# zhangxiaochen95/uav_bs_ctrl

Hardware: AMD Instinct MI355X
Metric: env-steps/sec (MADRQN, 8 UBS x 80 GT) (higher is better)
Workload: dtype f32

## Files before the change

include/uavgnn.h:

```cpp
#ifndef UAVGNN_H
#define UAVGNN_H

#include <stddef.h>
#include <stdint.h>

#ifdef __cplusplus
extern "C" {
#endif

#define UAVGNN_VERSION 100

#define UAVGNN_EINVAL (-1000)
#define UAVGNN_EUNSUPPORTED (-1001)
#define UAVGNN_EWORKSPACE (-1002)

typedef void* uavgnn_stream_t;

int uavgnn_version(void);

const char* uavgnn_strerror(int code);

int uavgnn_gatv2_fwd(const float* x_src, int E, int F_src, const float* x_dst, int F_dst, const int32_t* seg_off,
                     const int32_t* dst_order, int N, const float* W_s, const float* b_s, const float* W_d, const float* b_d, const float* attn,
                     const float* W_r, const float* b_r, int nh, int D, float slope, float* out, int ld_out,
// ... 40 lines not shown
                     const float* attn_save, float* dW_s, float* db_s, float* dW_d, float* db_d, float* dattn,
                     float* dW_r, float* db_r, void* workspace, size_t workspace_bytes, uavgnn_stream_t stream);
int uavgnn_gatv2_bwd_generic(const float* x_src, int E, int F_src, const float* x_dst, int F_dst, const int32_t* seg_off,
                     const int32_t* dst_order, int N, const float* W_s, const float* b_s, const float* W_d, const float* b_d, const float* attn,
                     int nh, int D, float slope, const float* out, const float* d_out, int ld_out,
                     const float* attn_save, float* dW_s, float* db_s, float* dW_d, float* db_d, float* dattn,
                     float* dW_r, float* db_r, void* workspace, size_t workspace_bytes, uavgnn_stream_t stream);

int uavgnn_talk_attn_fwd(const float* s, int ld_s, const float* q, int ld_q, const float* v, int ld_v, int K, int M,
                         const int32_t* talk_off, const int32_t* talk_src, int N, float scale, float* c, int ld_c,
                         float* a_save, const float* x_copy, int ld_x, int n_copy, uavgnn_stream_t stream);

int uavgnn_talk_attn_bwd(const float* s, int ld_s, const float* q, int ld_q, const float* v, int ld_v, int K, int M,
                         const int32_t* talk_off, const int32_t* talk_src, const int32_t* t_off, const int32_t* t_dst,
                         const int32_t* t_pos, int N, float scale, const float* a_save, const float* d_c, int ld_dc,
                         float* d_s, int ld_ds, float* d_q, int ld_dq, float* d_v, int ld_dv, float* de_tmp,
                         uavgnn_stream_t stream);

int uavgnn_gru_gates_fwd(const float* gi, const float* gh, const float* h, int N, int H, float* h_out,
                         uavgnn_stream_t stream);
int uavgnn_gru_gates_bwd(const float* gi, const float* gh, const float* h, const float* d_hout, int N, int H,
                         float* d_gi, float* d_gh, float* d_h, uavgnn_stream_t stream);

int uavgnn_disc_comm_fwd(const float* logits, int ld, const float* gumbel, const long long* rng, int msg,
                         const int32_t* talk_off, const int32_t* talk_src, int N, float inv_tau, float* c, int ld_c,
                         float* y0_save, int32_t* sel, uavgnn_stream_t stream);
int uavgnn_gumbel_noise(const long long* rng, long long E, int msg, float* out, uavgnn_stream_t stream);
int uavgnn_disc_comm_bwd(const float* d_c, int ld_dc, const float* y0_save, const int32_t* sel, int msg,
                         const int32_t* t_off, const int32_t* t_dst, const int32_t* t_pos, int N, float inv_tau,
                         float* d_logits, int ld_dl, uavgnn_stream_t stream);

int uavgnn_obs_degrees(const float* gt, int M, int Fg, const float* ubs, int U, int Fu, int N, int32_t* deg_seen,
                       int32_t* deg_near, uavgnn_stream_t stream);
int uavgnn_obs_compact(const float* gt, int M, int Fg, const float* ubs, int U, int Fu, int N, const int32_t* seen_off,
                       const int32_t* near_off, float* x_gt, float* x_ubs, uavgnn_stream_t stream);
int uavgnn_talk_degrees(const float* d_u2u, int n, int B, float r_comm, int32_t* deg_in, int32_t* env_edges,
                        uavgnn_stream_t stream);
int uavgnn_talk_compact(const float* d_u2u, int n, int B, float r_comm, const int32_t* talk_off,
                        const int32_t* env_base, int32_t* talk_src, int32_t* talk_eid, uavgnn_stream_t stream);
int uavgnn_offsets_scan4(const int32_t* d0, int n0, int32_t* o0, const int32_t* d1, int n1, int32_t* o1, const int32_t* d2,
                         int n2, int32_t* o2, const int32_t* d3, int n3, int32_t* o3, uavgnn_stream_t stream);

int uavgnn_eps_greedy(const float* q, int ld_q, int N, int A, int n_agents, const float* u_team, const float* u_agent,
                      float eps, long long* acts, uavgnn_stream_t stream);
int uavgnn_eps_greedy_dev(const float* q, int ld_q, int N, int A, int n_agents, const float* u_team, const float* u_agent,
                          const float* eps_dev, long long* acts, uavgnn_stream_t stream);

int uavgnn_colsum_acc(const float* x, long long ld, int N, int C, float* acc, int S, uavgnn_stream_t stream);
int uavgnn_gemm_h2_supported(int M, int N, int K);
long long uavgnn_split_h2_bytes(int n_out, int K);
int uavgnn_split_h2(const float* W, int ld, int R, int C, int transpose, void* planes, uavgnn_stream_t stream);
int uavgnn_gemm_nt_h2(const float* X, int ldx, int K1, const float* X2, int ldx2, int M, int K, const float* rowmax, const float* rowmax2,
                      const void* planes, int N, const float* bias, float* Y, int ldy, int epilogue, uavgnn_stream_t stream);
int uavgnn_gemm_nt_h2_rm2(const float* X, int ldx, int K1, const float* X2, int ldx2, int M, int K, const float* rowmax, float* rowmax2_out,
                          const void* planes, int N, const float* bias, float* Y, int ldy, int epilogue, uavgnn_stream_t stream);
int uavgnn_gemm_nt_h2_n64(const float* X, int ldx, int M, int K, const float* rowmax, const void* planes, int N, float* Y, int ldy,
                          uavgnn_stream_t stream);
int uavgnn_gru_gates_bwd_fused_sums_rowmax(const float* pre, const float* h, const float* d_hout, const float* dq, int n_out,
                                           const float* W_out, int N, int H, float* d_gi, float* d_gh, float* d_h, float* col_sums,
                                           float* row_absmax, uavgnn_stream_t stream);
int uavgnn_relu_bwd_colsum_rowmax(const float* dy, long long ld, const float* y, long long ldy, float* out, long long ldo, int N, int C,
                                  float* acc, int S, float* row_absmax, uavgnn_stream_t stream);
int uavgnn_relu_bwd_colsum(const float* dy, long long ld, const float* y, long long ldy, float* out, long long ldo, int N, int C,
                           float* acc, int S, uavgnn_stream_t stream);

int uavgnn_flat_obs_supported(int H_out, int F);
int uavgnn_flat_obs_fwd(const float* agent, long long ld_a, int F_a, const float* gt, long long ld_g, int K_g, const float* ubs,
                        long long ld_u, int K_u, int rows, const float* W, const float* b, int H_out, float* y, long long ld_y,
                        uavgnn_stream_t stream);
int uavgnn_flat_obs_wgrad_chunks(long long rows, int H_out, int F);
int uavgnn_flat_obs_wgrad(const float* dy, long long ld_dy, int H_out, const float* agent, long long ld_a, int F_a, const float* gt,
                          long long ld_g, int K_g, const float* ubs, long long ld_u, int K_u, int rows, float* partials, int S,
                          int accumulate, uavgnn_stream_t stream);

int uavgnn_talk_attn_env_supported(int n_max, int M, int K);
int uavgnn_talk_attn_env_fwd(const float* s, int ld_s, const float* q, int ld_q, const float* v, int ld_v, int K, int M,
                             const int32_t* talk_off, const int32_t* talk_src, const int32_t* graph_off, int B,
                             int n_max, float scale, float* c, int ld_c, float* a_save, const float* x_copy, int ld_x,
                             int n_copy, uavgnn_stream_t stream);
int uavgnn_talk_attn_env_bwd(const float* s, int ld_s, const float* q, int ld_q, const float* v, int ld_v, int K, int M,
                             const int32_t* talk_off, const int32_t* talk_src, const int32_t* graph_off, int B,
                             int n_max, float scale, const float* a_save, const float* d_c, int ld_dc, float* d_s,
                             int ld_ds, float* d_q, int ld_dq, float* d_v, int ld_dv, uavgnn_stream_t stream);

int uavgnn_tarmac_msg_supported(int H, int M, int K, int n_ag);
long long uavgnn_tarmac_msg_weight_bytes(int H, int M, int K);
long long uavgnn_tarmac_msg_planes_bytes(int N, int H, int M);
int uavgnn_tarmac_msg_prepare(const float* Wp, int ld, int H, int M, int K, void* tiles, uavgnn_stream_t stream);
int uavgnn_tarmac_msg_fwd(const float* x, int ld_x, const float* h, int ld_h, int N, int H, int n_ag, const void* tiles,
                          const float* bias, int M, int K, const int32_t* talk_off, const int32_t* talk_src, float scale,
                          float* c_out, int ld_c, float* a_save, float* proj_out, int ld_p, float* x_copy, int ld_xc,
                          void* planes_out, uavgnn_stream_t stream);
int uavgnn_tarmac_msg_rowmax_supported(int H, int M, int K, int n_ag);
int uavgnn_tarmac_msg_fwd_rowmax(const float* x, int ld_x, const float* h, int ld_h, int N, int H, int n_ag, const void* tiles,
                                 const float* bias, int M, int K, const int32_t* talk_off, const int32_t* talk_src, float scale,
                                 float* c_out, int ld_c, float* a_save, float* proj_out, int ld_p, float* x_copy, int ld_xc,
                                 float* row_absmax, uavgnn_stream_t stream);

size_t uavgnn_degree_order_workspace_bytes(int N);
int uavgnn_degree_order(const int32_t* seg_off, int N, int32_t* order, void* workspace, size_t workspace_bytes,
                        uavgnn_stream_t stream);
size_t uavgnn_csc_transpose_workspace_bytes(int N);
int uavgnn_csc_transpose(const int32_t* talk_off, const int32_t* talk_src, int N, int E, int32_t* t_off,
                         int32_t* t_dst, int32_t* t_pos, void* workspace, size_t workspace_bytes,
                         uavgnn_stream_t stream);
int uavgnn_csc_transpose_env(const int32_t* talk_off, const int32_t* talk_src, const int32_t* graph_off, int B, int N,
                             int32_t* t_off, int32_t* t_dst, int32_t* t_pos, uavgnn_stream_t stream);

int uavgnn_adamw_polyak(float* p, float* g, float* exp_avg, float* exp_avg_sq, float* p_targ, long long n,
                        long long n_clip, const float* hyper, double beta1, double beta2, float eps, float weight_decay,
                        float clip, float polyak, uavgnn_stream_t stream);

int uavgnn_env_state_dim(int n_ubs, int n_gts, int fair_service);
int uavgnn_env_step(const int32_t* int_consts, const double* f64_consts, int B, const long long* actions,
                    const double* avail_moves, double* pos_ubs, const float* pos_gts, int32_t* prior, float* avg_rate,
                    int32_t* t, float* run_f32, double* n_colls, float* d_u2g, float* d_u2u, int32_t* gt_ubs,
                    int32_t* gt_rb, float* rate_per_gt, double* rate_per_ubs, int32_t* mask_collision, double* reward,
                    float* done, float* obs_gt, float* obs_ubs, float* obs_agent, float* state, uavgnn_stream_t stream);

int uavgnn_build_graph_small_max_agents(void);
int uavgnn_build_graph_small(const float* gt, int M, int Fg, const float* ubs, int U, int Fu, const float* d_u2u, int n, int B,
                             float r_comm, int32_t* seen_off, int32_t* near_off, int32_t* talk_off, float* x_gt, float* x_ubs,
                             int32_t* talk_src, int32_t* talk_eid, int32_t* graph_off, uavgnn_stream_t stream);

int uavgnn_gru_cell_supported(int K_in, int H);
int uavgnn_gru_cell_fwd(const float* inp, int ld_inp, int K_in, const float* h, int N, int H, const float* W_ih,
                        const float* b_ih, const float* W_hh, const float* b_hh, float* h_out, float* pre_save,
                        uavgnn_stream_t stream);
int uavgnn_gru_cell_x3_supported(int K_in, int H);
long long uavgnn_gru_cell_x3_workspace_bytes(int K_in, int H);
int uavgnn_gru_split_weights(const float* W_ih, int K_in, const float* W_hh, int H, void* planes, uavgnn_stream_t stream);
int uavgnn_gru_cell_fwd_x3(const float* inp, int ld_inp, int K_in, const float* h, int N, int H, const void* planes,
                           const float* b_ih, const float* b_hh, float* h_out, float* pre_save, uavgnn_stream_t stream);
int uavgnn_gru_cell_fwd_x3_cat(const float* inp, int ld_inp, int K1, const float* inp2, int ld_inp2, int K2, const float* h,
                               int N, int H, const void* planes, const float* b_ih, const float* b_hh, float* h_out,
                               float* pre_save, uavgnn_stream_t stream);
#define UAVGNN_GRU_STAGING_BLOCKS 1
int uavgnn_gru_cell_fwd_x3_opts(const float* inp, int ld_inp, int K1, const float* inp2, int ld_inp2, int K2, const float* h,
                                int N, int H, const void* planes, const float* b_ih, const float* b_hh, float* h_out,
                                float* pre_save, int flags, uavgnn_stream_t stream);
int uavgnn_gru_cell_h2_supported(int K_in, int H);
long long uavgnn_gru_cell_h2_workspace_bytes(int K_in, int H);
int uavgnn_gru_split_weights_h2(const float* W_ih, int K_in, const float* W_hh, int H, void* planes, uavgnn_stream_t stream);
int uavgnn_gru_cell_fwd_h2(const float* inp, int ld_inp, int K1, const float* inp2, int ld_inp2, int K2, const float* h, int N, int H,
                           const float* row_absmax, const void* planes, const float* b_ih, const float* b_hh, float* h_out,
                           float* pre_save, uavgnn_stream_t stream);
int uavgnn_row_absmax(const float* a1, int ld1, int K1, const float* a2, int ld2, int K2, const float* a3, int ld3, int K3, int N,
                      float* out, uavgnn_stream_t stream);
int uavgnn_head_supported(int H, int A);
int uavgnn_head_fwd(const float* h, int ld_h, int N, int H, const float* W, int ld_w, const float* b, int A, float* q, int ld_q,
                    uavgnn_stream_t stream);
#define UAVGNN_GEMM_ACCUMULATE 1
#define UAVGNN_GEMM_RELU 2
#define UAVGNN_GEMM_STAGING_INTERLEAVED 4
#define UAVGNN_GEMM_TILE_128 8
#define UAVGNN_GEMM_TILE_64 16
int uavgnn_gemm_x3_supported(int M, int N, int K);
int uavgnn_split_bf16x3(const float* W, int ld, int R, int C, int transpose, void* planes, uavgnn_stream_t stream);
int uavgnn_gemm_nt_x3(const float* X, int ldx, int M, int K, const void* planes, int N, const float* bias, float* Y, int ldy,
                      int epilogue, uavgnn_stream_t stream);
int uavgnn_gemm_nt_x3_cat(const float* X, int ldx, int K1, const float* X2, int ldx2, int M, int K, const void* planes, int N,
                          const float* bias, float* Y, int ldy, int epilogue, uavgnn_stream_t stream);
int uavgnn_gemm_nt_x3_rowmax(const float* X, int ldx, int M, int K, const void* planes, int N, const float* bias, float* Y, int ldy,
                             int epilogue, float* rowmax_out, uavgnn_stream_t stream);

int uavgnn_gemm_tn_x3_chunks(long long n_rows, int Mo, int Ko);
int uavgnn_gemm_tn_x3(const float* dY, int ldy, int Mo, const float* X, int ldx, int Ko, long long n_rows, float* partials,
                      int S, int accumulate, uavgnn_stream_t stream);
int uavgnn_col_absmax(const float* x, long long ld, long long n, int C, float* out, uavgnn_stream_t stream);
int uavgnn_gemm_tn_h2_supported(long long n_rows, int Mo, int Ko);
int uavgnn_gemm_tn_h2_chunks(long long n_rows, int Mo, int Ko);
int uavgnn_gemm_tn_h2(const float* dY, long long ldy, int Mo, const float* X, long long ldx, int Ko, long long n_rows,
                      const float* colmax_y, const float* colmax_x, float* partials, int S, int accumulate, uavgnn_stream_t stream);
int uavgnn_gru_gates_bwd_fused(const float* pre, const float* h, const float* d_hout, int N, int H, float* d_gi, float* d_gh,
                               float* d_h, uavgnn_stream_t stream);
int uavgnn_gru_gates_bwd_fused_head(const float* pre, const float* h, const float* d_hout, const float* dq, int n_out,
                                    const float* W_out, int N, int H, float* d_gi, float* d_gh, float* d_h,
                                    uavgnn_stream_t stream);
int uavgnn_gru_gates_bwd_sum_rows(int N, int H);
int uavgnn_gru_gates_bwd_fused_sums(const float* pre, const float* h, const float* d_hout, const float* dq, int n_out,
                                    const float* W_out, int N, int H, float* d_gi, float* d_gh, float* d_h, float* col_sums,
                                    uavgnn_stream_t stream);

long long uavgnn_gru_cell_bwd_workspace_bytes(int K_in, int H);
int uavgnn_gru_split_weights_bwd(const float* W_ih, int K_in, const float* W_hh, int H, void* planes, uavgnn_stream_t stream);
int uavgnn_gru_cell_bwd(const float* pre, const float* h, const float* d_hout, int N, int K_in, int H, const void* planes_bwd,
                        float* d_gi, float* d_gh, float* d_inp, int ld_dinp, float* d_h, uavgnn_stream_t stream);

#define UAVGNN_WS_GATV2_BWD 1
#define UAVGNN_WS_DEGREE_ORDER 2
#define UAVGNN_WS_CSC_TRANSPOSE 3
#define UAVGNN_WS_GRU_PLANES 4
#define UAVGNN_WS_GRU_BWD_PLANES 5
#define UAVGNN_WS_GEMM_PLANES 6
#define UAVGNN_WS_GEMM_TN_PARTIALS 7
#define UAVGNN_WS_K1_IMAGE 8
long long uavgnn_workspace_bytes(int kind, long long a, long long b, long long c);

#ifdef __cplusplus
// ... 4 lines not shown
```

uav_bs_ctrl_amd/_lib.py:

```python
from __future__ import annotations

import ctypes
import os

import torch as th

_HERE = os.path.dirname(os.path.abspath(__file__))
LIB_PATH = os.environ.get("UAVGNN_LIB") or os.path.join(_HERE, "csrc", "libuavgnn.so")

_c_fp = ctypes.c_void_p
_c_ip = ctypes.c_void_p
_c_int = ctypes.c_int
_c_f32 = ctypes.c_float
_c_st = ctypes.c_void_p

SIGNATURES = {
    "uavgnn_version": (_c_int, []),
    "uavgnn_strerror": (ctypes.c_char_p, [_c_int]),
    "uavgnn_gatv2_fwd": (_c_int, [_c_fp, _c_int, _c_int, _c_fp, _c_int, _c_ip, _c_ip, _c_int, _c_fp, _c_fp, _c_fp, _c_fp, _c_fp,
                                  _c_fp, _c_fp, _c_int, _c_int, _c_f32, _c_fp, _c_int, _c_fp, _c_st]),
    "uavgnn_gatv2_fwd_valu": (_c_int, [_c_fp, _c_int, _c_int, _c_fp, _c_int, _c_ip, _c_ip, _c_int, _c_fp, _c_fp, _c_fp, _c_fp, _c_fp,
                                       _c_fp, _c_fp, _c_int, _c_int, _c_f32, _c_fp, _c_int, _c_fp, _c_st]),
    "uavgnn_gatv2_fwd_mfma": (_c_int, [_c_fp, _c_int, _c_int, _c_fp, _c_int, _c_ip, _c_ip, _c_int, _c_fp, _c_fp, _c_fp, _c_fp, _c_fp,
                                       _c_fp, _c_fp, _c_int, _c_int, _c_f32, _c_fp, _c_int, _c_fp, _c_st]),
# ... 38 lines not shown
    "uavgnn_talk_compact": (_c_int, [_c_fp, _c_int, _c_int, _c_f32, _c_ip, _c_ip, _c_ip, _c_ip, _c_st]),
    "uavgnn_build_graph_small_max_agents": (_c_int, []),
    "uavgnn_build_graph_small": (_c_int, [_c_fp, _c_int, _c_int, _c_fp, _c_int, _c_int, _c_fp, _c_int, _c_int, _c_f32, _c_ip, _c_ip,
                                          _c_ip, _c_fp, _c_fp, _c_ip, _c_ip, _c_ip, _c_st]),
    "uavgnn_degree_order_workspace_bytes": (ctypes.c_size_t, [_c_int]),
    "uavgnn_degree_order": (_c_int, [_c_ip, _c_int, _c_ip, ctypes.c_void_p, ctypes.c_size_t, _c_st]),
    "uavgnn_csc_transpose_workspace_bytes": (ctypes.c_size_t, [_c_int]),
    "uavgnn_csc_transpose": (_c_int, [_c_ip, _c_ip, _c_int, _c_int, _c_ip, _c_ip, _c_ip, ctypes.c_void_p,
                                      ctypes.c_size_t, _c_st]),
    "uavgnn_csc_transpose_env": (_c_int, [_c_ip, _c_ip, _c_ip, _c_int, _c_int, _c_ip, _c_ip, _c_ip, _c_st]),
    "uavgnn_talk_attn_env_supported": (_c_int, [_c_int, _c_int, _c_int]),
    "uavgnn_tarmac_msg_supported": (_c_int, [_c_int, _c_int, _c_int, _c_int]),
    "uavgnn_tarmac_msg_weight_bytes": (ctypes.c_longlong, [_c_int, _c_int, _c_int]),
    "uavgnn_tarmac_msg_planes_bytes": (ctypes.c_longlong, [_c_int, _c_int, _c_int]),
    "uavgnn_tarmac_msg_prepare": (_c_int, [_c_fp, _c_int, _c_int, _c_int, _c_int, ctypes.c_void_p, _c_st]),
    "uavgnn_tarmac_msg_fwd_dbg": (_c_int, [_c_fp, _c_int, _c_fp, _c_int, _c_int, _c_int, _c_int, ctypes.c_void_p, _c_fp, _c_int, _c_int,
                                           _c_ip, _c_ip, _c_f32, _c_fp, _c_int, _c_fp, _c_fp, _c_int, _c_fp, _c_int, ctypes.c_void_p,
                                           _c_int, _c_st]),
    "uavgnn_tarmac_msg_fwd": (_c_int, [_c_fp, _c_int, _c_fp, _c_int, _c_int, _c_int, _c_int, ctypes.c_void_p, _c_fp, _c_int, _c_int,
                                       _c_ip, _c_ip, _c_f32, _c_fp, _c_int, _c_fp, _c_fp, _c_int, _c_fp, _c_int, ctypes.c_void_p,
                                       _c_st]),
    "uavgnn_talk_attn_env_fwd": (_c_int, [_c_fp, _c_int, _c_fp, _c_int, _c_fp, _c_int, _c_int, _c_int, _c_ip, _c_ip,
                                          _c_ip, _c_int, _c_int, _c_f32, _c_fp, _c_int, _c_fp, _c_fp, _c_int, _c_int,
                                          _c_st]),
    "uavgnn_talk_attn_env_bwd": (_c_int, [_c_fp, _c_int, _c_fp, _c_int, _c_fp, _c_int, _c_int, _c_int, _c_ip, _c_ip,
                                          _c_ip, _c_int, _c_int, _c_f32, _c_fp, _c_fp, _c_int, _c_fp, _c_int, _c_fp,
                                          _c_int, _c_fp, _c_int, _c_st]),
    "uavgnn_eps_greedy": (_c_int, [_c_fp, _c_int, _c_int, _c_int, _c_int, _c_fp, _c_fp, _c_f32, ctypes.c_void_p, _c_st]),
    "uavgnn_eps_greedy_dev": (_c_int, [_c_fp, _c_int, _c_int, _c_int, _c_int, _c_fp, _c_fp, _c_fp, ctypes.c_void_p, _c_st]),
    "uavgnn_colsum_acc": (_c_int, [_c_fp, ctypes.c_longlong, _c_int, _c_int, _c_fp, _c_int, _c_st]),
    "uavgnn_relu_bwd_colsum": (_c_int, [_c_fp, ctypes.c_longlong, _c_fp, ctypes.c_longlong, _c_fp, ctypes.c_longlong, _c_int, _c_int, _c_fp,
                               _c_int, _c_st]),
    "uavgnn_relu_bwd_colsum_rowmax": (_c_int, [_c_fp, ctypes.c_longlong, _c_fp, ctypes.c_longlong, _c_fp, ctypes.c_longlong, _c_int, _c_int,
                                               _c_fp, _c_int, _c_fp, _c_st]),
    "uavgnn_flat_obs_supported": (_c_int, [_c_int, _c_int]),
    "uavgnn_flat_obs_fwd": (_c_int, [_c_fp, ctypes.c_longlong, _c_int, _c_fp, ctypes.c_longlong, _c_int, _c_fp, ctypes.c_longlong, _c_int,
                                     _c_int, _c_fp, _c_fp, _c_int, _c_fp, ctypes.c_longlong, _c_st]),
    "uavgnn_flat_obs_wgrad_chunks": (_c_int, [ctypes.c_longlong, _c_int, _c_int]),
    "uavgnn_flat_obs_wgrad": (_c_int, [_c_fp, ctypes.c_longlong, _c_int, _c_fp, ctypes.c_longlong, _c_int, _c_fp, ctypes.c_longlong, _c_int,
                                       _c_fp, ctypes.c_longlong, _c_int, _c_int, _c_fp, _c_int, _c_int, _c_st]),
    "uavgnn_gemm_nt_x3_rowmax": (_c_int, [_c_fp, _c_int, _c_int, _c_int, ctypes.c_void_p, _c_int, _c_fp, _c_fp, _c_int, _c_int, _c_fp, _c_st]),
    "uavgnn_col_absmax": (_c_int, [_c_fp, ctypes.c_longlong, ctypes.c_longlong, _c_int, _c_fp, _c_st]),
    "uavgnn_gemm_tn_h2_supported": (_c_int, [ctypes.c_longlong, _c_int, _c_int]),
    "uavgnn_gemm_tn_h2_chunks": (_c_int, [ctypes.c_longlong, _c_int, _c_int]),
    "uavgnn_gemm_tn_h2": (_c_int, [_c_fp, ctypes.c_longlong, _c_int, _c_fp, ctypes.c_longlong, _c_int, ctypes.c_longlong, _c_fp, _c_fp, _c_fp,
                                   _c_int, _c_int, _c_st]),
    "uavgnn_gemm_h2_supported": (_c_int, [_c_int, _c_int, _c_int]),
    "uavgnn_split_h2_bytes": (ctypes.c_longlong, [_c_int, _c_int]),
    "uavgnn_split_h2": (_c_int, [_c_fp, _c_int, _c_int, _c_int, _c_int, ctypes.c_void_p, _c_st]),
    "uavgnn_gemm_nt_h2": (_c_int, [_c_fp, _c_int, _c_int, _c_fp, _c_int, _c_int, _c_int, _c_fp, _c_fp, ctypes.c_void_p, _c_int, _c_fp, _c_fp,
                                   _c_int, _c_int, _c_st]),
    "uavgnn_gemm_nt_h2_rm2": (_c_int, [_c_fp, _c_int, _c_int, _c_fp, _c_int, _c_int, _c_int, _c_fp, _c_fp, ctypes.c_void_p, _c_int, _c_fp, _c_fp,
                                       _c_int, _c_int, _c_st]),
    "uavgnn_gemm_nt_h2_n64": (_c_int, [_c_fp, _c_int, _c_int, _c_int, _c_fp, ctypes.c_void_p, _c_int, _c_fp, _c_int, _c_st]),
    "uavgnn_env_state_dim": (_c_int, [_c_int, _c_int, _c_int]),
    "uavgnn_env_step": (_c_int, [ctypes.POINTER(ctypes.c_int32), ctypes.POINTER(ctypes.c_double), _c_int] + [_c_fp] * 22 + [_c_st]),
    "uavgnn_adamw_polyak": (_c_int, [_c_fp, _c_fp, _c_fp, _c_fp, _c_fp, ctypes.c_longlong, ctypes.c_longlong, _c_fp, ctypes.c_double,
                                     ctypes.c_double, _c_f32, _c_f32, _c_f32, _c_f32, _c_st]),
    "uavgnn_gru_cell_supported": (_c_int, [_c_int, _c_int]),
    "uavgnn_gru_cell_fwd": (_c_int, [_c_fp, _c_int, _c_int, _c_fp, _c_int, _c_int, _c_fp, _c_fp, _c_fp, _c_fp, _c_fp, _c_fp, _c_st]),
    "uavgnn_gru_cell_x3_supported": (_c_int, [_c_int, _c_int]),
    "uavgnn_gru_cell_x3_workspace_bytes": (ctypes.c_longlong, [_c_int, _c_int]),
    "uavgnn_gru_split_weights": (_c_int, [_c_fp, _c_int, _c_fp, _c_int, ctypes.c_void_p, _c_st]),
    "uavgnn_gru_cell_fwd_x3": (_c_int, [_c_fp, _c_int, _c_int, _c_fp, _c_int, _c_int, ctypes.c_void_p, _c_fp, _c_fp, _c_fp, _c_fp, _c_st]),
    "uavgnn_gru_cell_fwd_x3_cat": (_c_int, [_c_fp, _c_int, _c_int, _c_fp, _c_int, _c_int, _c_fp, _c_int, _c_int, ctypes.c_void_p, _c_fp, _c_fp,
                                            _c_fp, _c_fp, _c_st]),
    "uavgnn_gru_cell_fwd_x3_opts": (_c_int, [_c_fp, _c_int, _c_int, _c_fp, _c_int, _c_int, _c_fp, _c_int, _c_int, ctypes.c_void_p, _c_fp, _c_fp,
                                             _c_fp, _c_fp, _c_int, _c_st]),
    "uavgnn_gru_cell_h2_supported": (_c_int, [_c_int, _c_int]),
    "uavgnn_gru_cell_h2_workspace_bytes": (ctypes.c_longlong, [_c_int, _c_int]),
    "uavgnn_gru_split_weights_h2": (_c_int, [_c_fp, _c_int, _c_fp, _c_int, ctypes.c_void_p, _c_st]),
    "uavgnn_gru_cell_fwd_h2": (_c_int, [_c_fp, _c_int, _c_int, _c_fp, _c_int, _c_int, _c_fp, _c_int, _c_int, _c_fp, ctypes.c_void_p, _c_fp,
                                        _c_fp, _c_fp, _c_fp, _c_st]),
    "uavgnn_row_absmax": (_c_int, [_c_fp, _c_int, _c_int, _c_fp, _c_int, _c_int, _c_fp, _c_int, _c_int, _c_int, _c_fp, _c_st]),
    "uavgnn_tarmac_msg_rowmax_supported": (_c_int, [_c_int, _c_int, _c_int, _c_int]),
    "uavgnn_tarmac_msg_fwd_rowmax": (_c_int, [_c_fp, _c_int, _c_fp, _c_int, _c_int, _c_int, _c_int, ctypes.c_void_p, _c_fp, _c_int, _c_int,
                                              _c_ip, _c_ip, _c_f32, _c_fp, _c_int, _c_fp, _c_fp, _c_int, _c_fp, _c_int, _c_fp, _c_st]),
    "uavgnn_gru_weight_tiles_bytes": (ctypes.c_longlong, [_c_int, _c_int]),
    "uavgnn_gru_split_weight_tiles": (_c_int, [_c_fp, _c_int, _c_fp, _c_int, ctypes.c_void_p, _c_st]),
    "uavgnn_gru_cell_fwd_planes": (_c_int, [ctypes.c_void_p, _c_int, _c_fp, _c_int, _c_int, ctypes.c_void_p, _c_fp, _c_fp, _c_fp, _c_fp,
                                            _c_st]),
    "uavgnn_gru_cell_fwd_planes_opts": (_c_int, [ctypes.c_void_p, _c_int, _c_fp, _c_int, _c_int, ctypes.c_void_p, _c_fp, _c_fp, _c_fp,
                                                 _c_fp, _c_int, _c_st]),
    "uavgnn_gru_cell_bwd_workspace_bytes": (ctypes.c_longlong, [_c_int, _c_int]),
    "uavgnn_gru_split_weights_bwd": (_c_int, [_c_fp, _c_int, _c_fp, _c_int, ctypes.c_void_p, _c_st]),
    "uavgnn_gru_cell_bwd": (_c_int, [_c_fp, _c_fp, _c_fp, _c_int, _c_int, _c_int, ctypes.c_void_p, _c_fp, _c_fp, _c_fp, _c_int, _c_fp,
                                     _c_st]),
    "uavgnn_workspace_bytes": (ctypes.c_longlong, [_c_int, ctypes.c_longlong, ctypes.c_longlong, ctypes.c_longlong]),
    "uavgnn_gemm_tn_x3_chunks": (_c_int, [ctypes.c_longlong, _c_int, _c_int]),
    "uavgnn_gemm_tn_x3": (_c_int, [_c_fp, _c_int, _c_int, _c_fp, _c_int, _c_int, ctypes.c_longlong, _c_fp, _c_int, _c_int, _c_st]),
    "uavgnn_gemm_x3_supported": (_c_int, [_c_int, _c_int, _c_int]),
    "uavgnn_head_supported": (_c_int, [_c_int, _c_int]),
    "uavgnn_head_fwd": (_c_int, [_c_fp, _c_int, _c_int, _c_int, _c_fp, _c_int, _c_fp, _c_int, _c_fp, _c_int, _c_st]),
    "uavgnn_split_bf16x3": (_c_int, [_c_fp, _c_int, _c_int, _c_int, _c_int, ctypes.c_void_p, _c_st]),
    "uavgnn_gemm_nt_x3": (_c_int, [_c_fp, _c_int, _c_int, _c_int, ctypes.c_void_p, _c_int, _c_fp, _c_fp, _c_int, _c_int, _c_st]),
    "uavgnn_gemm_nt_x3_cat": (_c_int, [_c_fp, _c_int, _c_int, _c_fp, _c_int, _c_int, _c_int, ctypes.c_void_p, _c_int, _c_fp, _c_fp, _c_int,
                              _c_int, _c_st]),
    "uavgnn_gru_gates_bwd_fused": (_c_int, [_c_fp, _c_fp, _c_fp, _c_int, _c_int, _c_fp, _c_fp, _c_fp, _c_st]),
    "uavgnn_gru_gates_bwd_fused_head": (_c_int, [_c_fp, _c_fp, _c_fp, _c_fp, _c_int, _c_fp, _c_int, _c_int, _c_fp, _c_fp, _c_fp,
                                                 _c_st]),
    "uavgnn_gru_gates_bwd_sum_rows": (_c_int, [_c_int, _c_int]),
    "uavgnn_gru_gates_bwd_fused_sums": (_c_int, [_c_fp, _c_fp, _c_fp, _c_fp, _c_int, _c_fp, _c_int, _c_int, _c_fp, _c_fp, _c_fp, _c_fp,
                                                 _c_st]),
    "uavgnn_gru_gates_bwd_fused_sums_rowmax": (_c_int, [_c_fp, _c_fp, _c_fp, _c_fp, _c_int, _c_fp, _c_int, _c_int, _c_fp, _c_fp, _c_fp, _c_fp,
                                                        _c_fp, _c_st]),
    "uavgnn_gru_gates_fwd": (_c_int, [_c_fp, _c_fp, _c_fp, _c_int, _c_int, _c_fp, _c_st]),
    "uavgnn_gru_gates_bwd": (_c_int, [_c_fp, _c_fp, _c_fp, _c_fp, _c_int, _c_int, _c_fp, _c_fp, _c_fp, _c_st]),
}

_LIB = None
UAVGNN_EINVAL = -1000
UAVGNN_EUNSUPPORTED = -1001


class UavGnnError(RuntimeError):
    pass


def lib() -> ctypes.CDLL:
    global _LIB
    if _LIB is None:
        if not os.path.exists(LIB_PATH):
            raise UavGnnError(f"{LIB_PATH} is missing - build it with `python -c 'import __graft_entry__ as g; "
                              f"g.build()'`.  uav_bs_ctrl_amd has no CPU / eager fallback.")
        handle = ctypes.CDLL(LIB_PATH)
        for name, (res, args) in SIGNATURES.items():
            fn = getattr(handle, name)
            fn.restype, fn.argtypes = res, args
        _LIB = handle
        if os.environ.get("UAVGNN_TUNED_GEMM", "0") == "1":
# ... 42 lines not shown
```

uav_bs_ctrl_amd/csrc/gemm_h2.hip:

```cpp
#include "common.h"
#include "f16x2.h"

namespace uavgnn {
namespace {

using namespace h2;

constexpr int BN = 128, BK = 32, BM8 = 256, NT = 512;
constexpr int PA = BM8 * 4, PB = BN * 4;
constexpr int BUF = 2 * PA + 2 * PB;

__global__ __launch_bounds__(256) void split_h2_kernel(const float* __restrict__ W, int ld, int R, int C, int transpose,
                                                       unsigned short* __restrict__ planes, float* __restrict__ winv) {
  __shared__ float red[4];
  const int orow = blockIdx.x, tid = threadIdx.x;
  const int ocol_n = transpose ? R : C;
  const size_t n = static_cast<size_t>(transpose ? C : R) * ocol_n;
  auto at = [&](int j) { return transpose ? W[static_cast<size_t>(j) * ld + orow] : W[static_cast<size_t>(orow) * ld + j]; };
  float m = 0.f;
  for (int j = tid; j < ocol_n; j += 256) m = fmaxf(m, fabsf(at(j)));
  m = wave_max(m);
  if ((tid & 63) == 0) red[tid >> 6] = m;
  __syncthreads();
  m = fmaxf(fmaxf(red[0], red[1]), fmaxf(red[2], red[3]));
  const int se = scale_exp(m);
  const float s = pow2f(se);
  for (int j = 2 * tid; j < ocol_n; j += 512) {
    const Split2 sp = split_pair(at(j) * s, at(j + 1) * s);
    *reinterpret_cast<unsigned*>(planes + static_cast<size_t>(orow) * ocol_n + j) = sp.hi;
    *reinterpret_cast<unsigned*>(planes + n + static_cast<size_t>(orow) * ocol_n + j) = sp.lo;
  }
  if (tid == 0) winv[orow] = pow2f(-se);
}

template <bool ACC, bool RELU, bool IL>
__global__ __launch_bounds__(NT) void gemm_nt_h2w8_kernel(const float* __restrict__ X, int ldx, int M, int K,
                                                          const unsigned short* __restrict__ Bp, int N, const float* __restrict__ winv,
                                                          const float* __restrict__ bias, float* __restrict__ Y, int ldy,
                                                          int row_blocks, int col_blocks, const float* __restrict__ X2, int ldx2,
                                                          int ns1, const float* __restrict__ rm1, const float* __restrict__ rm2,
                                                          float* __restrict__ rm2_out) {
  constexpr int kTileChunks = BM8 * (BN + 4) / 4;
#ifndef UAVGNN_GEMM_H2_TILE_STORE
#define UAVGNN_GEMM_H2_TILE_STORE 1
#endif
  constexpr bool kTileStore = ACC || UAVGNN_GEMM_H2_TILE_STORE;
  __shared__ u32x4 smem[(kTileStore && kTileChunks > 2 * BUF) ? kTileChunks : 2 * BUF];
  __shared__ float sInv[BM8];
  __shared__ float sRow2[BM8];
  const int tid = threadIdx.x, lane = tid & 63, wave = tid >> 6;
  const int l32 = lane & 31, lh = lane >> 5, sw = swz32(l32);
  const int wm = (wave >> 1) * 64, wn = (wave & 1) * 64;
  const int xcd = blockIdx.x & 7, slot = blockIdx.x >> 3;
  const int rb = (slot / col_blocks) * 8 + xcd, cb = slot - (slot / col_blocks) * col_blocks;
  if (rb >= row_blocks) return;
  const int m0 = rb * BM8, n0 = cb * BN;

  f32x16 acc[2][2];
#pragma unroll
  for (int a = 0; a < 2; ++a)
#pragma unroll
    for (int b = 0; b < 2; ++b)
#pragma unroll
      for (int i = 0; i < 16; ++i) acc[a][b][i] = 0.f;

  const int lr = tid >> 3, c4 = tid & 7;
  unsigned xo[4], xo2[4];
  float sca[4];
  auto bound = [&](int row) {
    const float a = rm1[row];
    return rm2 != nullptr ? fmaxf(a, rm2[row]) : a;
  };
  const bool own2 = rm2_out != nullptr;
  float m2[4] = {0.f, 0.f, 0.f, 0.f};
#pragma unroll
  for (int i = 0; i < 4; ++i) {
    const int row = min(m0 + lr + 64 * i, M - 1);
    xo[i] = static_cast<unsigned>(row) * ldx + 4 * c4;
    xo2[i] = static_cast<unsigned>(row) * ldx2 + 4 * c4;
  }
  if (own2) {
    const int nq = (K - ns1 * BK) / 4;
    bool bad[4] = {false, false, false, false};
#pragma unroll
    for (int i = 0; i < 4; ++i)
      for (int q = c4; q < nq; q += 8) {
        const float4 v = *reinterpret_cast<const float4*>(X2 + xo2[i] + 4 * (q - c4));
        const float a0 = fabsf(v.x), a1 = fabsf(v.y), a2 = fabsf(v.z), a3 = fabsf(v.w);
        bad[i] |= !(a0 <= 3.4028234663852886e38f) | !(a1 <= 3.4028234663852886e38f) | !(a2 <= 3.4028234663852886e38f) |
                  !(a3 <= 3.4028234663852886e38f);
        m2[i] = fmaxf(fmaxf(m2[i], fmaxf(a0, a1)), fmaxf(a2, a3));
      }
#pragma unroll
    for (int i = 0; i < 4; ++i) {
// ... 133 lines not shown
      }
      __builtin_amdgcn_sched_barrier(0);
      UAVGNN_H2_MFMA(f0)
      __builtin_amdgcn_sched_barrier(0);
      if (!early) {
        lstore((t + 1) & 1);
        gload(min(t + 2, ns - 1));
      }
      __syncthreads();
      UAVGNN_H2_READ(f0, (t + 1) & 1, 0)
      __builtin_amdgcn_sched_barrier(0);
      UAVGNN_H2_MFMA(f1)
      __builtin_amdgcn_sched_barrier(0);
    }
  }
#undef UAVGNN_H2_MFMA
#undef UAVGNN_H2_TERM
#undef UAVGNN_H2_READ
  if constexpr (kTileStore) {
  if ((ldy & 3) == 0 && (reinterpret_cast<uintptr_t>(Y) & 15) == 0 && n0 + BN <= N) {
    constexpr int LDT = BN + 4;
    float* sT = reinterpret_cast<float*>(smem);
    static_assert(BM8 * LDT * 4 <= static_cast<int>(sizeof(smem)), "the output tile fits the LDS array");
    __syncthreads();
#pragma unroll
    for (int a = 0; a < 2; ++a)
#pragma unroll
      for (int b = 0; b < 2; ++b) {
        const int col = n0 + wn + b * 32 + l32;
        const float bv = bias != nullptr ? bias[col] : 0.f, ci = winv[col];
#pragma unroll
        for (int i = 0; i < 16; ++i) {
          const int lrow = wm + a * 32 + 8 * (i >> 2) + 4 * lh + (i & 3);
          sT[lrow * LDT + wn + b * 32 + l32] = acc[a][b][i] * ci * sInv[lrow] + bv;
        }
      }
    float4 yv[16];
    if constexpr (ACC) {
#pragma unroll
      for (int q = 0; q < 16; ++q) {
        const int idx = tid + NT * q, row = idx >> 5, cc = idx & 31;
        yv[q] = *reinterpret_cast<const float4*>(Y + static_cast<size_t>(min(m0 + row, M - 1)) * ldy + n0 + 4 * cc);
      }
    }
    __syncthreads();
#pragma unroll
    for (int q = 0; q < 16; ++q) {
      const int idx = tid + NT * q, row = idx >> 5, cc = idx & 31;
      const float4 t = *reinterpret_cast<const float4*>(sT + row * LDT + 4 * cc);
      float4 o = t;
      if constexpr (ACC) o = {yv[q].x + t.x, yv[q].y + t.y, yv[q].z + t.z, yv[q].w + t.w};
      if (RELU) o = {fmaxf(o.x, 0.f), fmaxf(o.y, 0.f), fmaxf(o.z, 0.f), fmaxf(o.w, 0.f)};
      if (m0 + row < M) *reinterpret_cast<float4*>(Y + static_cast<size_t>(m0 + row) * ldy + n0 + 4 * cc) = o;
    }
    return;
  }
  }
#pragma unroll
  for (int b = 0; b < 2; ++b) {
    const int col = n0 + wn + b * 32 + l32;
    if (col >= N) continue;
    const float bv = bias != nullptr ? bias[col] : 0.f, ci = winv[col];
#pragma unroll
    for (int a = 0; a < 2; ++a)
#pragma unroll
      for (int i = 0; i < 16; ++i) {
        const int lrow = wm + a * 32 + 8 * (i >> 2) + 4 * lh + (i & 3);
        const int row = m0 + lrow;
        if (row < M) {
          float* p = Y + static_cast<size_t>(row) * ldy + col;
          float v = acc[a][b][i] * ci * sInv[lrow] + bv;
          if (ACC) v += *p;
          if (RELU) v = fmaxf(v, 0.f);
          *p = v;
        }
      }
  }
}

constexpr int BM6 = 128, BN6 = 64;
constexpr int PA6 = BM6 * 4, PB6 = BN6 * 4;
constexpr int SUB6 = 2 * PA6 + 2 * PB6;
constexpr int BUF6 = 2 * SUB6;

__global__ __launch_bounds__(NT) void gemm_nt_h2n64_kernel(const float* __restrict__ X, int ldx, int M, int K,
                                                           const unsigned short* __restrict__ Bp, int N, const float* __restrict__ winv,
                                                           float* __restrict__ Y, int ldy, int col_blocks, const float* __restrict__ rm1) {
  constexpr int LDT = BN6 + 4;
  static_assert(BM6 * LDT * 4 <= 2 * BUF6 * 16, "the output tile fits the staging buffers");
  __shared__ u32x4 smem[2 * BUF6];
  __shared__ float sInv[BM6];
  const int tid = threadIdx.x, lane = tid & 63, wave = tid >> 6;
  const int l32 = lane & 31, lh = lane >> 5, sw = swz32(l32);
  const int wm = (wave >> 1) * 32, wn = (wave & 1) * 32;
  const int rb = blockIdx.x / col_blocks, cb = blockIdx.x - rb * col_blocks;
  const int m0 = rb * BM6, n0 = cb * BN6;

  f32x16 acc;
#pragma unroll
  for (int i = 0; i < 16; ++i) acc[i] = 0.f;

  const int lr = tid >> 3, c4 = tid & 7;
  unsigned xo[2];
  float sca[2];
#pragma unroll
  for (int i = 0; i < 2; ++i) {
// ... 68 lines not shown
    __builtin_amdgcn_sched_barrier(0);
    UAVGNN_N64_MFMA(f3)
    __builtin_amdgcn_sched_barrier(0);
  }
#undef UAVGNN_N64_MFMA
#undef UAVGNN_N64_READ
  float* sT = reinterpret_cast<float*>(smem);
  __syncthreads();
  {
    const float ci = winv[n0 + wn + l32];
#pragma unroll
    for (int i = 0; i < 16; ++i) {
      const int lrow = wm + 8 * (i >> 2) + 4 * lh + (i & 3);
      sT[lrow * LDT + wn + l32] = acc[i] * ci * sInv[lrow];
    }
  }
  __syncthreads();
#pragma unroll
  for (int q = 0; q < 4; ++q) {
    const int idx = tid + NT * q, row = idx >> 4, cc = idx & 15;
    if (m0 + row < M)
      *reinterpret_cast<float4*>(Y + static_cast<size_t>(m0 + row) * ldy + n0 + 4 * cc) =
          *reinterpret_cast<const float4*>(sT + row * LDT + 4 * cc);
  }
}

}
}

using namespace uavgnn;

extern "C" int uavgnn_gemm_h2_supported(int M, int N, int K) {
  return (M > 0 && N > 0 && K >= BK && K % BK == 0 && static_cast<long long>(M) * K < (1LL << 31) &&
          2LL * N * K < (1LL << 31)) ? 1 : 0;
}

extern "C" long long uavgnn_split_h2_bytes(int n_out, int K) {
  if (n_out <= 0 || K <= 0) return 0;
  return 4LL * n_out * K + 4LL * n_out;
}

extern "C" int uavgnn_split_h2(const float* W, int ld, int R, int C, int transpose, void* planes, uavgnn_stream_t stream) {
  if (!W || !planes || R <= 0 || C <= 0 || ld < C) return UAVGNN_EINVAL;
  const int n_out = transpose ? C : R, K = transpose ? R : C;
  if ((K & 1) || (reinterpret_cast<uintptr_t>(planes) & 15)) return UAVGNN_EUNSUPPORTED;
  unsigned short* p = static_cast<unsigned short*>(planes);
  float* winv = reinterpret_cast<float*>(p + 2LL * n_out * K);
  hipLaunchKernelGGL(split_h2_kernel, dim3(n_out), dim3(256), 0, static_cast<hipStream_t>(stream), W, ld, R, C, transpose, p, winv);
  return launch_status();
}

static int gemm_nt_h2_launch(const float* X, int ldx, int K1, const float* X2, int ldx2, int M, int K, const float* rowmax,
                             const float* rowmax2, float* rowmax2_out, const void* planes, int N, const float* bias, float* Y, int ldy,
                             int epilogue, uavgnn_stream_t stream) {
  if (M < 0 || !X || !planes || !Y || !rowmax || ldx < K1 || ldy < N || K1 <= 0 || K1 > K || (X2 == nullptr) != (K1 == K) ||
      (X2 != nullptr && ldx2 < K - K1) || (rowmax2_out != nullptr && (X2 == nullptr || rowmax2 != nullptr)))
    return UAVGNN_EINVAL;
  if (M == 0) return 0;
  if (!uavgnn_gemm_h2_supported(M, N, K) || (ldx & 3) || static_cast<long long>(M) * ldx >= (1LL << 31) ||
      ((reinterpret_cast<uintptr_t>(X) | reinterpret_cast<uintptr_t>(planes)) & 15) ||
      (epilogue & (UAVGNN_GEMM_TILE_128 | UAVGNN_GEMM_TILE_64)))
    return UAVGNN_EUNSUPPORTED;
  if (X2 != nullptr && ((K1 % BK) || (ldx2 & 3) || static_cast<long long>(M) * ldx2 >= (1LL << 31) || (reinterpret_cast<uintptr_t>(X2) & 15)))
    return UAVGNN_EUNSUPPORTED;
  const int ns1 = K1 / BK;
  hipStream_t st = static_cast<hipStream_t>(stream);
  const unsigned short* bp = static_cast<const unsigned short*>(planes);
  const float* winv = reinterpret_cast<const float*>(bp + 2LL * N * K);
  const bool acc = (epilogue & UAVGNN_GEMM_ACCUMULATE) != 0, relu = (epilogue & UAVGNN_GEMM_RELU) != 0;
  const int col_blocks = (N + BN - 1) / BN, row_blocks = (M + BM8 - 1) / BM8;
  const dim3 grid(((row_blocks + 7) / 8) * 8 * col_blocks), block(NT);
#define UAVGNN_H2_GEMM(ACC, RELU, IL)                                                                                              \
  hipLaunchKernelGGL((gemm_nt_h2w8_kernel<ACC, RELU, IL>), grid, block, 0, st, X, ldx, M, K, bp, N, winv, bias, Y, ldy, row_blocks, \
                     col_blocks, X2, ldx2, ns1, rowmax, rowmax2, rowmax2_out)
#define UAVGNN_H2_GEMM_IL(IL)                         \
  if (acc && relu) UAVGNN_H2_GEMM(true, true, IL);    \
  else if (acc) UAVGNN_H2_GEMM(true, false, IL);      \
  else if (relu) UAVGNN_H2_GEMM(false, true, IL);     \
  else UAVGNN_H2_GEMM(false, false, IL);
  if (epilogue & UAVGNN_GEMM_STAGING_INTERLEAVED) { UAVGNN_H2_GEMM_IL(true) }
  else { UAVGNN_H2_GEMM_IL(false) }
#undef UAVGNN_H2_GEMM_IL
#undef UAVGNN_H2_GEMM
  return launch_status();
}

extern "C" int uavgnn_gemm_nt_h2(const float* X, int ldx, int K1, const float* X2, int ldx2, int M, int K, const float* rowmax,
                                 const float* rowmax2, const void* planes, int N, const float* bias, float* Y, int ldy, int epilogue,
                                 uavgnn_stream_t stream) {
  return gemm_nt_h2_launch(X, ldx, K1, X2, ldx2, M, K, rowmax, rowmax2, nullptr, planes, N, bias, Y, ldy, epilogue, stream);
}

extern "C" int uavgnn_gemm_nt_h2_rm2(const float* X, int ldx, int K1, const float* X2, int ldx2, int M, int K, const float* rowmax,
                                     float* rowmax2_out, const void* planes, int N, const float* bias, float* Y, int ldy, int epilogue,
                                     uavgnn_stream_t stream) {
  if (!rowmax2_out) return UAVGNN_EINVAL;
  return gemm_nt_h2_launch(X, ldx, K1, X2, ldx2, M, K, rowmax, nullptr, rowmax2_out, planes, N, bias, Y, ldy, epilogue, stream);
}

extern "C" int uavgnn_gemm_nt_h2_n64(const float* X, int ldx, int M, int K, const float* rowmax, const void* planes, int N, float* Y,
                                     int ldy, uavgnn_stream_t stream) {
  if (M < 0 || !X || !planes || !Y || !rowmax || K <= 0 || N <= 0 || ldx < K || ldy < N) return UAVGNN_EINVAL;
  if (M == 0) return 0;
  if (!uavgnn_gemm_h2_supported(M, N, K) || (N % BN6) || (K % (2 * BK)) || (ldx & 3) || (ldy & 3) || static_cast<long long>(M) * ldx >= (1LL << 31) ||
      ((reinterpret_cast<uintptr_t>(X) | reinterpret_cast<uintptr_t>(planes) | reinterpret_cast<uintptr_t>(Y)) & 15))
    return UAVGNN_EUNSUPPORTED;
  const unsigned short* bp = static_cast<const unsigned short*>(planes);
  const float* winv = reinterpret_cast<const float*>(bp + 2LL * N * K);
  const int col_blocks = N / BN6, row_blocks = (M + BM6 - 1) / BM6;
  hipLaunchKernelGGL(gemm_nt_h2n64_kernel, dim3(row_blocks * col_blocks), dim3(NT), 0, static_cast<hipStream_t>(stream), X, ldx, M, K, bp,
                     N, winv, Y, ldy, col_blocks, rowmax);
  return launch_status();
}
```

uav_bs_ctrl_amd/csrc/gru_h2.hip:

```cpp
#include <type_traits>

#include "common.h"
#include "f16x2.h"
#include "gru_gates.h"

namespace uavgnn {
namespace {

using namespace h2;

constexpr int BM = 128, BK = 32, BJ = 64, NT = 512, ST = 68;
constexpr int PA = BM * 4, PB = 3 * BJ * 4;
constexpr int BUF = 2 * PA + 2 * PB;

__global__ __launch_bounds__(256) void split_planes_h2_kernel(const float* __restrict__ W_ih, int K_in, const float* __restrict__ W_hh,
                                                              int H, unsigned short* __restrict__ p_ih,
                                                              unsigned short* __restrict__ p_hh, float* __restrict__ winv) {
  __shared__ float red[4];
  const int row = blockIdx.x, tid = threadIdx.x;
  const float* a = W_ih + static_cast<size_t>(row) * K_in;
  const float* b = W_hh + static_cast<size_t>(row) * H;
  float m = 0.f;
  for (int i = tid; i < K_in; i += 256) m = fmaxf(m, fabsf(a[i]));
  for (int i = tid; i < H; i += 256) m = fmaxf(m, fabsf(b[i]));
  m = wave_max(m);
  if ((tid & 63) == 0) red[tid >> 6] = m;
  __syncthreads();
  m = fmaxf(fmaxf(red[0], red[1]), fmaxf(red[2], red[3]));
  const int se = scale_exp(m);
  const float s = pow2f(se);
  const size_t n_ih = static_cast<size_t>(3) * H * K_in, n_hh = static_cast<size_t>(3) * H * H;
  for (int i = 2 * tid; i < K_in; i += 512) {
    const Split2 sp = split_pair(a[i] * s, a[i + 1] * s);
    *reinterpret_cast<unsigned*>(p_ih + static_cast<size_t>(row) * K_in + i) = sp.hi;
    *reinterpret_cast<unsigned*>(p_ih + n_ih + static_cast<size_t>(row) * K_in + i) = sp.lo;
  }
  for (int i = 2 * tid; i < H; i += 512) {
    const Split2 sp = split_pair(b[i] * s, b[i + 1] * s);
    *reinterpret_cast<unsigned*>(p_hh + static_cast<size_t>(row) * H + i) = sp.hi;
    *reinterpret_cast<unsigned*>(p_hh + n_hh + static_cast<size_t>(row) * H + i) = sp.lo;
  }
  if (tid == 0) winv[row] = pow2f(-se);
}

template <bool SAVE>
__global__ __launch_bounds__(NT) void gru_cell_fwd_h2_kernel(
    const float* __restrict__ inp, int ld_inp, int K1, const float* __restrict__ inp2, int ld_inp2, int K2,
    const float* __restrict__ h, int N, int H, const float* __restrict__ row_absmax,
    const unsigned short* __restrict__ Wih_p, const float* __restrict__ b_ih, const unsigned short* __restrict__ Whh_p,
    const float* __restrict__ b_hh, const float* __restrict__ winv, float* __restrict__ h_out, float* __restrict__ pre, int row_blocks) {
  __shared__ u32x4 smem[2 * BUF];
  __shared__ float sInv[BM];
  const int tid = threadIdx.x, lane = tid & 63, wave = tid >> 6;
  const int wm = (wave >> 1) * 32, wc = (wave & 1) * 32;
  const int CB = H / BJ;
  const int xcd = blockIdx.x & 7, slot = blockIdx.x >> 3;
  const int rb = (slot / CB) * 8 + xcd, cb = slot - (slot / CB) * CB;
  if (rb >= row_blocks) return;
  const int m0 = rb * BM, j0 = cb * BJ;

  f32x16 acc[4];
#pragma unroll
  for (int s = 0; s < 4; ++s)
#pragma unroll
    for (int i = 0; i < 16; ++i) acc[s][i] = 0.f;
  const int l32 = lane & 31, lh = lane >> 5, sw = swz32(l32);
  const int lr = tid >> 3, c4 = tid & 7;
  const int sa_w = lr * 32 + (((c4 >> 1) ^ swz32(lr)) * 8) + (c4 & 1) * 4;
  unsigned rowa[2], wrow[3];
  float sca[2];
  int sbw[3];
#pragma unroll
  for (int i = 0; i < 2; ++i) {
    rowa[i] = static_cast<unsigned>(min(m0 + lr + 64 * i, N - 1));
    sca[i] = pow2f(scale_exp(row_absmax[rowa[i]]));
  }
  if (tid < BM) sInv[tid] = pow2f(-scale_exp(row_absmax[min(m0 + tid, N - 1)]));
#pragma unroll
  for (int i = 0; i < 3; ++i) {
    const int q = tid + NT * i, pl = q / PB, rem = q - pl * PB, row = rem >> 2, c = rem & 3;
    wrow[i] = static_cast<unsigned>(pl * 3 * H + (row >> 6) * H + j0 + (row & 63));
    sbw[i] = 2 * PA + pl * PB + row * 4 + (c ^ swz32(row));
  }
  const unsigned wc8 = 16u * (tid & 3);
  const int n1 = K1 / BK, n12 = n1 + K2 / BK, ns = n12 + H / BK;
  float4 ra[2][2];
  u32x4 rw[2][3];
  unsigned oa[2], ow[3];
  const char* __restrict__ Ab = reinterpret_cast<const char*>(inp);
  const char* __restrict__ Wb = reinterpret_cast<const char*>(Wih_p);
  int lt = 0;
  auto set_a = [&](const float* base, int ld) {
    Ab = reinterpret_cast<const char*>(base);
#pragma unroll
    for (int i = 0; i < 2; ++i) oa[i] = 4u * (rowa[i] * static_cast<unsigned>(ld) + 4u * c4);
  };
  auto set_w = [&](const unsigned short* base, int K) {
    Wb = reinterpret_cast<const char*>(base);
#pragma unroll
    for (int i = 0; i < 3; ++i) ow[i] = 2u * wrow[i] * static_cast<unsigned>(K) + wc8;
  };
  set_a(inp, ld_inp);
  set_w(Wih_p, K1 + K2);
// ... 128 lines not shown
    UAVGNN_H2_STEP(2, Set1)
    ++t;
    UAVGNN_H2_STEP(3, Set0)
    ++t;
  }
  for (; t + 1 < ns; ++t) {
    UAVGNN_H2_STEP(3, Set1)
    ++t;
    UAVGNN_H2_STEP(3, Set0)
  }
  if (t < ns) {
    UAVGNN_H2_STEP(3, Set1)
    ++t;
  }
#undef UAVGNN_H2_STEP
#undef UAVGNN_H2_MFMA
#undef UAVGNN_H2_READ
#undef UAVGNN_H2_TERM
  __syncthreads();
  float* sH = reinterpret_cast<float*>(smem);
#pragma unroll
  for (int q = 0; q < 4; ++q) {
    const int idx = tid + NT * q, row = idx >> 4, cc = idx & 15;
    *reinterpret_cast<float4*>(sH + row * ST + 4 * cc) =
        *reinterpret_cast<const float4*>(h + static_cast<size_t>(min(m0 + row, N - 1)) * H + j0 + 4 * cc);
  }
  __syncthreads();
  const int c = j0 + wc + l32;
  const float b_r = b_ih[c] + b_hh[c], b_z = b_ih[H + c] + b_hh[H + c], b_in = b_ih[2 * H + c], b_hn = b_hh[2 * H + c];
  const float ci_r = winv[c], ci_z = winv[H + c], ci_n = winv[2 * H + c];
#pragma unroll
  for (int i = 0; i < 16; ++i) {
    const int lrow = wm + 8 * (i >> 2) + 4 * lh + (i & 3);
    const int row = m0 + lrow;
    const float ri = sInv[lrow];
    const float pr = acc[0][i] * ri * ci_r + b_r, pz = acc[1][i] * ri * ci_z + b_z;
    const float gin = acc[2][i] * ri * ci_n + b_in, ghn = acc[3][i] * ri * ci_n + b_hn;
    const float rr = fast_sigmoid(pr), zz = fast_sigmoid(pz);
    const float nn = fast_tanh(fmaf(rr, ghn, gin));
    float* hp = sH + lrow * ST + wc + l32;
    *hp = fmaf(zz, *hp - nn, nn);
    if (SAVE && row < N) {
      float* p = pre + static_cast<size_t>(row) * 4 * H + c;
      p[0] = pr;
      p[H] = pz;
      p[2 * H] = gin;
      p[3 * H] = ghn;
    }
  }
  __syncthreads();
#pragma unroll
  for (int q = 0; q < 4; ++q) {
    const int idx = tid + NT * q, row = idx >> 4, cc = idx & 15;
    if (m0 + row < N)
      *reinterpret_cast<float4*>(h_out + static_cast<size_t>(m0 + row) * H + j0 + 4 * cc) =
          *reinterpret_cast<const float4*>(sH + row * ST + 4 * cc);
  }
}

}
}

using namespace uavgnn;

extern "C" int uavgnn_gru_cell_h2_supported(int K_in, int H) {
  return (K_in >= BK && K_in % BK == 0 && H >= BJ && H % BJ == 0) ? 1 : 0;
}

extern "C" long long uavgnn_gru_cell_h2_workspace_bytes(int K_in, int H) {
  if (K_in <= 0 || H <= 0) return 0;
  return 2LL * 3 * H * (static_cast<long long>(K_in) + H) * 2 + 4LL * 3 * H;
}

extern "C" int uavgnn_gru_split_weights_h2(const float* W_ih, int K_in, const float* W_hh, int H, void* planes,
                                           uavgnn_stream_t stream) {
  if (!W_ih || !W_hh || !planes || K_in <= 0 || H <= 0) return UAVGNN_EINVAL;
  if ((K_in & 1) || (H & 1) || ((reinterpret_cast<uintptr_t>(W_ih) | reinterpret_cast<uintptr_t>(W_hh)) & 7) ||
      (reinterpret_cast<uintptr_t>(planes) & 15))
    return UAVGNN_EUNSUPPORTED;
  unsigned short* p0 = static_cast<unsigned short*>(planes);
  unsigned short* p1 = p0 + 6LL * H * K_in;
  float* winv = reinterpret_cast<float*>(p1 + 6LL * H * H);
  hipLaunchKernelGGL(split_planes_h2_kernel, dim3(3 * H), dim3(256), 0, static_cast<hipStream_t>(stream), W_ih, K_in, W_hh, H, p0, p1,
                     winv);
  return launch_status();
}

extern "C" int uavgnn_gru_cell_fwd_h2(const float* inp, int ld_inp, int K1, const float* inp2, int ld_inp2, int K2, const float* h,
                                      int N, int H, const float* row_absmax, const void* planes, const float* b_ih,
                                      const float* b_hh, float* h_out, float* pre_save, uavgnn_stream_t stream) {
  const int K_in = K1 + K2;
  if (N < 0 || !inp || !h || !planes || !b_ih || !b_hh || !h_out || !row_absmax || ld_inp < K1 || K2 < 0 ||
      (K2 > 0 && (!inp2 || ld_inp2 < K2)))
    return UAVGNN_EINVAL;
  if (K2 == 0) {
    inp2 = inp;
    ld_inp2 = ld_inp;
  }
  if (!uavgnn_gru_cell_h2_supported(K_in, H) || K1 < BK || (K1 % BK) || (K2 % BK) || (ld_inp & 3) || (ld_inp2 & 3) ||
      ((reinterpret_cast<uintptr_t>(inp) | reinterpret_cast<uintptr_t>(inp2) | reinterpret_cast<uintptr_t>(h) |
        reinterpret_cast<uintptr_t>(planes) | reinterpret_cast<uintptr_t>(h_out)) & 15))
    return UAVGNN_EUNSUPPORTED;
  const long long ld_max = ld_inp > ld_inp2 ? (ld_inp > H ? ld_inp : H) : (ld_inp2 > H ? ld_inp2 : H);
  if (4LL * N * ld_max >= (1LL << 32) || 12LL * H * (K_in > H ? K_in : H) >= (1LL << 32)) return UAVGNN_EUNSUPPORTED;
  if (N == 0) return 0;
  const unsigned short* p0 = static_cast<const unsigned short*>(planes);
  const unsigned short* p1 = p0 + 6LL * H * K_in;
  const float* winv = reinterpret_cast<const float*>(p1 + 6LL * H * H);
  const int row_blocks = (N + BM - 1) / BM, rb8 = ((row_blocks + 7) / 8) * 8;
  hipStream_t st = static_cast<hipStream_t>(stream);
  const dim3 grid(rb8 * (H / BJ)), block(NT);
  if (pre_save != nullptr)
    hipLaunchKernelGGL(gru_cell_fwd_h2_kernel<true>, grid, block, 0, st, inp, ld_inp, K1, inp2, ld_inp2, K2, h, N, H, row_absmax, p0, b_ih,
                       p1, b_hh, winv, h_out, pre_save, row_blocks);
  else
    hipLaunchKernelGGL(gru_cell_fwd_h2_kernel<false>, grid, block, 0, st, inp, ld_inp, K1, inp2, ld_inp2, K2, h, N, H, row_absmax, p0, b_ih,
                       p1, b_hh, winv, h_out, pre_save, row_blocks);
  return launch_status();
}

namespace uavgnn {
namespace {
__global__ __launch_bounds__(256) void row_absmax_kernel(const float* __restrict__ a1, int ld1, int K1, const float* __restrict__ a2,
                                                         int ld2, int K2, const float* __restrict__ a3, int ld3, int K3, int N,
                                                         float* __restrict__ out) {
  const int row = blockIdx.x * 4 + (threadIdx.x >> 6), lane = threadIdx.x & 63;
  if (row >= N) return;
  float m = 0.f;
  bool bad = false;
  auto piece = [&](const float* a, int ld, int K) {
    if (a == nullptr) return;
    const float* r = a + static_cast<size_t>(row) * ld;
    for (int i = lane; i < K; i += 64) {
      const float v = fabsf(r[i]);
      bad |= !(v <= 3.4028234663852886e38f);
      m = fmaxf(m, v);
    }
  };
  piece(a1, ld1, K1);
  piece(a2, ld2, K2);
  piece(a3, ld3, K3);
  m = wave_max(m);
  if (__any(bad)) m = INFINITY;
  if (lane == 0) out[row] = m;
}
}
}

extern "C" int uavgnn_row_absmax(const float* a1, int ld1, int K1, const float* a2, int ld2, int K2, const float* a3, int ld3, int K3,
                                 int N, float* out, uavgnn_stream_t stream) {
  if (N < 0 || !a1 || !out || K1 <= 0 || ld1 < K1 || (a2 && (K2 <= 0 || ld2 < K2)) || (a3 && (K3 <= 0 || ld3 < K3))) return UAVGNN_EINVAL;
  if (N == 0) return 0;
  hipLaunchKernelGGL(row_absmax_kernel, dim3((N + 3) / 4), dim3(256), 0, static_cast<hipStream_t>(stream), a1, ld1, K1, a2, ld2, K2, a3,
                     ld3, K3, N, out);
  return launch_status();
}
```

uav_bs_ctrl_amd/csrc/tarmac_msg.hip:

```cpp
#include <math.h>

#include "bf16x3.h"
#include "common.h"
#include "uavgnn_probe.h"

namespace uavgnn {
namespace {

using namespace x3;

constexpr int kMsgWaves = 4;
constexpr int kMsgRows = 16 * kMsgWaves;
constexpr int kMsgThreads = kWave * kMsgWaves;
constexpr int kMaxCols = 128;

__device__ __forceinline__ bf16x8 frag_of(unsigned a, unsigned b, unsigned c, unsigned d) {
  return __builtin_bit_cast(bf16x8, u32x4{a, b, c, d});
}

__device__ __forceinline__ void lds_barrier() {
  __builtin_amdgcn_fence(__ATOMIC_RELEASE, "workgroup", "local");
  __builtin_amdgcn_s_barrier();
  __builtin_amdgcn_fence(__ATOMIC_ACQUIRE, "workgroup", "local");
}

struct Planes8 {
  u32x4 p[3];
};

__device__ __forceinline__ Planes8 split8(const float4 lo, const float4 hi) {
  const Split3 a = split_pair(lo.x, lo.y), b = split_pair(lo.z, lo.w), c = split_pair(hi.x, hi.y), d = split_pair(hi.z, hi.w);
  Planes8 r;
  r.p[0] = u32x4{a.h1, b.h1, c.h1, d.h1};
  r.p[1] = u32x4{a.h2, b.h2, c.h2, d.h2};
  r.p[2] = u32x4{a.h3, b.h3, c.h3, d.h3};
  return r;
}

__global__ __launch_bounds__(256) void tarmac_msg_prepare_kernel(const float* __restrict__ W, int ld, int R, int RP, int KK,
                                                                 u32x4* __restrict__ tiles) {
  const int idx = blockIdx.x * 256 + threadIdx.x;
  const int per_slice = RP * 4, nsl = KK / 32;
  if (idx >= nsl * per_slice) return;
  const int s = idx / per_slice, rem = idx - s * per_slice, r = rem >> 2, c = rem & 3;
  Planes8 pl;
  if (r < R) {
    const float* src = W + static_cast<size_t>(r) * ld + 32 * s + 4 * c;
    pl = split8(*reinterpret_cast<const float4*>(src), *reinterpret_cast<const float4*>(src + 16));
  } else {
    pl.p[0] = pl.p[1] = pl.p[2] = u32x4{0u, 0u, 0u, 0u};
  }
  u32x4* dst = tiles + static_cast<size_t>(s) * 3 * per_slice + r * 4 + (c ^ swz(r));
#pragma unroll
  for (int p = 0; p < 3; ++p) dst[p * per_slice] = pl.p[p];
}

__device__ __forceinline__ void msg_scatter(float* __restrict__ Mx, int nmax, const float* __restrict__ VAL,
                                            const int* __restrict__ SRC, const int* __restrict__ DST,
                                            const int* __restrict__ OFF, int E, int lane) {
  for (int e = lane; e < E; e += kWave) {
    const int d = DST[e], sidx = SRC[e];
    const int j0 = OFF[d], j1 = OFF[d + 1];
    bool first = true;
    for (int jx = j0; jx < e; ++jx) first = first && (SRC[jx] != sidx);
    if (first) {
      float acc = VAL[e];
      for (int jx = e + 1; jx < j1; ++jx)
        if (SRC[jx] == sidx) acc += VAL[jx];
      Mx[d * nmax + sidx] = acc;
    }
  }
}

template <int CT, bool TRAIN, bool PLANES>
__global__ __launch_bounds__(kMsgThreads, CT == 8 ? 2 : 3) void tarmac_msg_fwd_kernel(
    const float* __restrict__ x, int ld_x, const float* __restrict__ h, int ld_h, int N, int H, int n_ag,
    const u32x4* __restrict__ Wt, const float* __restrict__ bias, int M, int K, const int32_t* __restrict__ talk_off,
    const int32_t* __restrict__ talk_src, float scale, float* __restrict__ c_out, int ld_c, float* __restrict__ a_save,
    float* __restrict__ proj_out, int ld_p, float* __restrict__ x_copy, int ld_xc, u32x4* __restrict__ planes_out, int dbg) {
  constexpr int RP = 16 * CT;
  constexpr int BCH = 3 * RP * 4;
  constexpr int BPT = (BCH + kMsgThreads - 1) / kMsgThreads;
  constexpr int LDP = RP + 1;
  constexpr int NA = 16, EMAX = NA * NA;
  constexpr int kScratch = (NA + 4) + 5 * EMAX;
  constexpr int kLoopBytes = 2 * BCH * 16, kTailBytes = kMsgWaves * (16 * LDP + kScratch) * 4;
  __shared__ __attribute__((aligned(16))) unsigned char smem_raw[kLoopBytes > kTailBytes ? kLoopBytes : kTailBytes];
  u32x4(*sB)[BCH] = reinterpret_cast<u32x4(*)[BCH]>(smem_raw);

  const int tid = threadIdx.x, lane = tid & 63;
  const int wave = __builtin_amdgcn_readfirstlane(tid >> 6);
  const int j = lane & 15, g = lane >> 4;
  const int row0 = blockIdx.x * kMsgRows + wave * 16;
  const int row = row0 + j, rowc = min(row, N - 1);
  const int nsx = H / 32, ns = 2 * nsx;
  const float* __restrict__ xr = x + static_cast<size_t>(rowc) * ld_x + 4 * g;
  const float* __restrict__ hr = h + static_cast<size_t>(rowc) * ld_h + 4 * g;

  f32x4 acc[CT];
#pragma unroll
  for (int ct = 0; ct < CT; ++ct) acc[ct] = f32x4{0.f, 0.f, 0.f, 0.f};

  auto a_src = [&](int s) {
    s = min(s, ns - 1);
    return s < nsx ? xr + 32 * s : hr + 32 * (s - nsx);
  };
  u32x4 rb[BPT];
  auto load_b = [&](int s) {
    const u32x4* src = Wt + static_cast<size_t>(min(s, ns - 1)) * BCH;
#pragma unroll
    for (int i = 0; i < BPT; ++i) rb[i] = src[min(tid + kMsgThreads * i, BCH - 1)];
  };
  auto store_b = [&](int buf) {
#pragma unroll
    for (int i = 0; i < BPT; ++i) sB[buf][min(tid + kMsgThreads * i, BCH - 1)] = rb[i];
  };
  const int nsl_cell = nsx + (M + 31) / 32 + nsx;
  const int r128 = row & 127;
  u32x2* const pl_base = PLANES ? reinterpret_cast<u32x2*>(planes_out + (static_cast<size_t>(row >> 7) * nsl_cell * 3) * 512 + r128 * 4) +
                                      (g & 1)
                                : nullptr;
  const int pl_q0 = 2 * ((g >> 1) ^ swz32(r128)), pl_q1 = 2 * ((2 + (g >> 1)) ^ swz32(r128));
  auto store_planes = [&](int cell_slice, const Planes8& pl) {
    if (PLANES && row < N) {
// ... 270 lines not shown
      amax = fmaxf(fmaxf(amax, fabsf(HI.z)), fabsf(HI.w));                                           \
    }                                                                                                \
    if (TRAIN && half == 0 && x_copy != nullptr && row < N) {           \
      float* d = x_copy + static_cast<size_t>(row) * ld_xc + 32 * t_ + 4 * g;                        \
      *reinterpret_cast<float4*>(d) = LO;                                                            \
      *reinterpret_cast<float4*>(d + 16) = HI;                                                       \
    }                                                                                                \
    UAVGNN_MSG_LOAD_A(LO, HI, t_ + 2)                                                                \
    const bf16x8 fa0 = as_frag(pa.p[0]), fa1 = as_frag(pa.p[1]), fa2 = as_frag(pa.p[2]);            \
    const u32x4* sb = sB[t_ & 1] + half * BCH;                                                       \
    _Pragma("unroll") for (int cp = 0; cp < CT; cp += 2) {                                           \
      UAVGNN_MSG_TERM(fa0, 2) UAVGNN_MSG_TERM(fa2, 0) UAVGNN_MSG_TERM(fa1, 1) UAVGNN_MSG_TERM(fa0, 1) \
      UAVGNN_MSG_TERM(fa1, 0) UAVGNN_MSG_TERM(fa0, 0)                                                \
    }                                                                                                \
    store_b((t_ + 1) & 1);                    \
    load_b(t_ + 2);                                                                                  \
    lds_barrier();                                                                                   \
  }
  for (int t = 0; t < nsx; t += 2) {
    UAVGNN_MSG_STEP(a0_lo, a0_hi, t)
    UAVGNN_MSG_STEP(a1_lo, a1_hi, t + 1)
  }
#undef UAVGNN_MSG_STEP
#undef UAVGNN_MSG_TERM
#undef UAVGNN_MSG_LOAD_A

  float* __restrict__ P = reinterpret_cast<float*>(smem_raw) + tile * (16 * LDP + kScratch);
  const int ncol = M + 2 * K;
  if (RM) load_fsrc();
  if (RM) {
    amax = fmaxf(amax, __shfl_xor(amax, 16));
    amax = fmaxf(amax, __shfl_xor(amax, 32));
    if (g == 0) sRowMax[tile][half][j] = amax;
  }
  if (half == 0) {
#pragma unroll
    for (int ct = 0; ct < CT; ++ct) {
      const int col = ct * 16 + j;
      const float b = col < ncol ? bias[col] : 0.f;
#pragma unroll
      for (int i = 0; i < 4; ++i) P[(4 * g + i) * LDP + col] = acc[ct][i] + b;
    }
  }
  lds_barrier();
  if (half == 1) {
#pragma unroll
    for (int ct = 0; ct < CT; ++ct) {
      const int col = ct * 16 + j;
#pragma unroll
      for (int i = 0; i < 4; ++i) P[(4 * g + i) * LDP + col] += acc[ct][i];
    }
  }
  lds_barrier();
  int* __restrict__ OFF = reinterpret_cast<int*>(P + 16 * LDP);
  float* __restrict__ SC = reinterpret_cast<float*>(OFF + NA + 4);
  float* __restrict__ AD = SC + EMAX;
  int* __restrict__ SRC = reinterpret_cast<int*>(AD + EMAX);
  int* __restrict__ DST = SRC + EMAX;
  float* __restrict__ AV = reinterpret_cast<float*>(DST + EMAX);
  if (half == 1) {
    if (TRAIN && proj_out != nullptr) {
      for (int r = 0; r < 16; ++r) {
        if (row0 + r >= N) break;
        float* d = proj_out + static_cast<size_t>(row0 + r) * ld_p;
        for (int col = lane; col < ncol; col += kWave) d[col] = P[r * LDP + col];
      }
    }
    lds_barrier();
    return;
  }
  bool poison = !ok;
  if (ok) {
    for (int i = lane; i < EMAX; i += kWave) AD[i] = 0.f;
    if (lane <= 16) OFF[lane] = toff - e_lo;
    wave_sync_lds();
    bool bad = false;
#pragma unroll
    for (int i = 0; i < 4; ++i) {
      const int e = lane + kWave * i;
      if (e < E) {
        const int u = fsrc[i] - row0;
        bad |= (u < 0) | (u >= 16);
        SRC[e] = u < 0 ? 0 : (u >= 16 ? 15 : u);
        int d = 0;
#pragma unroll
        for (int jj = 1; jj < 16; ++jj) d += e >= OFF[jj];
        DST[e] = d;
      }
    }
    poison = __any(bad);
    wave_sync_lds();
    if (!poison) {
      for (int e = lane; e < E; e += kWave) {
        const float* __restrict__ sr = P + SRC[e] * LDP + M;
        const float* __restrict__ qr = P + DST[e] * LDP + M + K;
        float a = 0.f;
#pragma unroll 4
        for (int k = 0; k < K; ++k) a = fmaf(sr[k], qr[k], a);
        SC[e] = a * scale;
      }
      wave_sync_lds();
      for (int e = lane; e < E; e += kWave) {
        const int d = DST[e];
        const int j0 = OFF[d], j1 = OFF[d + 1];
        float m = -INFINITY;
#pragma unroll 2
        for (int jj = j0; jj < j1; ++jj) m = fmaxf(m, SC[jj]);
        float den = 0.f;
#pragma unroll 2
        for (int jj = j0; jj < j1; ++jj) den += expf(SC[jj] - m);
        const float a = expf(SC[e] - m) / den;
        if (TRAIN && a_save != nullptr) a_save[e_lo + e] = a;
        AV[e] = a;
      }
      wave_sync_lds();
      msg_scatter(AD, NA, AV, SRC, DST, OFF, E, lane);
      wave_sync_lds();
    }
  }
  lds_barrier();
  if (poison) {
    for (int i = 0; i < 16; ++i)
      for (int ch = lane; ch < M; ch += kWave) P[i * LDP + ch] = NAN;
  } else {
    for (int c0 = 0; c0 < M; c0 += kWave) {
      const int ch = c0 + lane, chc = ch < M ? ch : M - 1;
      float v[NA];
#pragma unroll
      for (int t = 0; t < NA; ++t) v[t] = P[t * LDP + chc];
#pragma unroll 4
      for (int r = 0; r < NA; ++r) {
        float a = 0.f;
#pragma unroll
        for (int t = 0; t < NA; t += 4) {
          const float4 q = *reinterpret_cast<const float4*>(AD + r * NA + t);
          a = fmaf(q.x, v[t], a);
          a = fmaf(q.y, v[t + 1], a);
          a = fmaf(q.z, v[t + 2], a);
          a = fmaf(q.w, v[t + 3], a);
        }
        if (ch < M) P[r * LDP + ch] = a;
      }
    }
  }
  wave_sync_lds();
  for (int r = 0; r < 16; ++r) {
    if (row0 + r >= N) break;
    float* d = c_out + static_cast<size_t>(row0 + r) * ld_c;
    for (int ch = lane; ch < M; ch += kWave) d[ch] = P[r * LDP + ch];
  }
  if (RM) {
    float cm = 0.f;
    for (int ch = g; ch < M; ch += 4) cm = fmaxf(cm, fabsf(P[j * LDP + ch]));
    cm = fmaxf(cm, __shfl_xor(cm, 16));
    cm = fmaxf(cm, __shfl_xor(cm, 32));
    if (g == 0 && row < N) row_absmax[row] = fmaxf(cm, fmaxf(sRowMax[tile][0][j], sRowMax[tile][1][j]));
  }
}

}
}

using namespace uavgnn;

extern "C" int uavgnn_tarmac_msg_supported(int H, int M, int K, int n_ag) {
  if (H < 32 || (H % 32) || M < 1 || K < 1 || K > 64 || M + 2 * K > kMaxCols) return 0;
  if (n_ag < 1 || n_ag > 16 || (16 % n_ag)) return 0;
  return 1;
}

static int msg_rows_padded(int M, int K) {
  const int ct = (M + 2 * K + 15) / 16;
  return 16 * (ct <= 4 ? 4 : ct <= 6 ? 6 : 8);
}

extern "C" long long uavgnn_tarmac_msg_weight_bytes(int H, int M, int K) {
  if (H <= 0 || M <= 0 || K <= 0 || M + 2 * K > kMaxCols) return 0;
  return static_cast<long long>(2 * H / 32) * 3 * msg_rows_padded(M, K) * 64;
}

extern "C" long long uavgnn_tarmac_msg_planes_bytes(int N, int H, int M) {
  if (N <= 0 || H <= 0 || M <= 0) return 0;
  const long long nsl = 2 * (H / 32) + (M + 31) / 32;
  return ((static_cast<long long>(N) + 127) / 128) * nsl * 3 * 8192;
}

extern "C" int uavgnn_tarmac_msg_prepare(const float* Wp, int ld, int H, int M, int K, void* tiles, uavgnn_stream_t stream) {
  if (!Wp || !tiles || H <= 0 || M <= 0 || K <= 0 || ld < 2 * H) return UAVGNN_EINVAL;
  if ((H % 32) || (ld & 3) || (reinterpret_cast<uintptr_t>(Wp) & 15) || (reinterpret_cast<uintptr_t>(tiles) & 15) || M + 2 * K > kMaxCols)
    return UAVGNN_EUNSUPPORTED;
  const int R = M + 2 * K, RP = msg_rows_padded(M, K), KK = 2 * H;
  const int total = (KK / 32) * RP * 4;
  hipLaunchKernelGGL(tarmac_msg_prepare_kernel, dim3((total + 255) / 256), dim3(256), 0, static_cast<hipStream_t>(stream), Wp, ld,
                     R, RP, KK, static_cast<u32x4*>(tiles));
  return launch_status();
}

static int msg_launch(const float* x, int ld_x, const float* h, int ld_h, int N, int H, int n_ag, const void* tiles, const float* bias, int M,
                      int K, const int32_t* talk_off, const int32_t* talk_src, float scale, float* c_out, int ld_c, float* a_save,
                      float* proj_out, int ld_p, float* x_copy, int ld_xc, void* planes_out, float* row_absmax, int dbg,
                      uavgnn_stream_t stream);

extern "C" int uavgnn_tarmac_msg_fwd_dbg(const float* x, int ld_x, const float* h, int ld_h, int N, int H, int n_ag, const void* tiles,
                                         const float* bias, int M, int K, const int32_t* talk_off, const int32_t* talk_src,
                                         float scale, float* c_out, int ld_c, float* a_save, float* proj_out, int ld_p,
                                         float* x_copy, int ld_xc, void* planes_out, int dbg, uavgnn_stream_t stream) {
  return msg_launch(x, ld_x, h, ld_h, N, H, n_ag, tiles, bias, M, K, talk_off, talk_src, scale, c_out, ld_c, a_save, proj_out, ld_p, x_copy,
                    ld_xc, planes_out, nullptr, dbg, stream);
}

// ... 85 lines not shown
```

uav_bs_ctrl_amd/ops.py:

```python
from __future__ import annotations

import os
import torch as th

from . import _lib as L

NEG_SLOPE = 0.2
K1_IMAGE = os.environ.get("UAVGNN_K1_IMAGE", "1") != "0"
HETERO_FUSED = True
K1_BF16Z = os.environ.get("UAVGNN_K1_BF16Z", "1") != "0"
K1_ROWMAX = os.environ.get("UAVGNN_K1_ROWMAX", "1") != "0"
K1_ROWMAX_MIN_ROWS = 1 << 17
K1_ROWMAX_DENSE_DEG = int(os.environ.get("UAVGNN_K1_ROWMAX_DENSE_DEG", "16"))
K1_ROWMAX_DENSE_MIN_ROWS = 16384


class _KernelTimer:

    def __init__(self):
        self.enabled = False
        self.only = None
        self._spans = {}

    def reset(self, enabled=True, only=None):
        self._spans = {}
        self.enabled = enabled
        self.only = None if only is None else frozenset(only)

    class _Span:
        def __init__(self, timer, name, work=None):
            self.t, self.name, self.work = timer, name, work

        def __enter__(self):
            self.on = self.t.enabled and (self.t.only is None or self.name in self.t.only)
            if self.on:
                self.e0 = th.cuda.Event(enable_timing=True)
                self.e1 = th.cuda.Event(enable_timing=True)
                self.e0.record()
            return self

        def __exit__(self, *exc):
            if self.on:
                self.e1.record()
                self.t._spans.setdefault(self.name, []).append((self.e0, self.e1, self.work))
            return False

    def span(self, name, work=None):
        return _KernelTimer._Span(self, name, work)

    def summary(self):
        th.cuda.synchronize()
        out = {}
        for name, pairs in self._spans.items():
            ms = [a.elapsed_time(b) for a, b, _ in pairs]
            out[name] = dict(count=len(ms), avg_ms=sum(ms) / len(ms), total_ms=sum(ms), ms=ms,
# ... 79 lines not shown
            has_order.append(order is not None)
            meta.append((FS, need, has_br, has_order[-1]))
        ctx.nh, ctx.meta, ctx.H = nh, meta, H
        ctx.save_for_backward(*saved, out)
        return out

    @staticmethod
    def backward(ctx, d_out):
        saved = ctx.saved_tensors
        x_dst, out = saved[0], saved[-1]
        nh, H = ctx.nh, ctx.H
        R = len(ctx.meta)
        N, dev = x_dst.shape[0], x_dst.device
        d_out = L.f32c(d_out)
        grads = [None, None, None]
        for i, (FS, need, has_br, has_ord) in enumerate(ctx.meta):
            x_src, seg_off, order, W_s, b_s, W_d, b_d, attn, W_r, a_save = saved[1 + i * 10: 1 + (i + 1) * 10]
            if not need or N == 0:
                grads += [None] * 10
                continue
            g = [th.empty_like(W_s), th.empty_like(b_s), th.empty_like(W_d), th.empty_like(b_d),
                 th.empty_like(attn), th.empty_like(W_r), th.empty(H, dtype=th.float32, device=dev)]
            ws_bytes = L.lib().uavgnn_gatv2_bwd_workspace_bytes(FS, H)
            ws = th.empty(ws_bytes // 4, dtype=th.float32, device=dev)
            with KERNEL_TIMER.span(f"gatv2_bwd[F={FS}]"):
                rc = L.lib().uavgnn_gatv2_bwd(L.ptr(x_src), x_src.shape[0], FS, L.ptr(x_dst), x_dst.shape[1], L.ptr(seg_off),
                                              L.ptr(order) if has_ord else None, N, L.ptr(W_s), L.ptr(b_s), L.ptr(W_d), L.ptr(b_d), L.ptr(attn), nh, H // nh,
                                              NEG_SLOPE, out.data_ptr() + 4 * i * H, d_out.data_ptr() + 4 * i * H,
                                              R * H, L.ptr(a_save), *[L.ptr(t) for t in g], ws.data_ptr(), ws_bytes,
                                              L.stream())
            L.check(rc, "uavgnn_gatv2_bwd")
            dW_s, db_s, dW_d, db_d, dattn, dW_r, db_r = g
            grads += [None, None, None, dattn, dW_s, db_s, dW_d, db_d, dW_r, db_r if has_br else None]
        return tuple(grads)


def hetero_gatv2(x_dst, nh, relations):
    flat = []
    for x_src, seg_off, order, conv in relations:
        flat += [x_src, seg_off, order, conv.attn, conv.fc_src.weight, conv.fc_src.bias, conv.fc_dst.weight,
                 conv.fc_dst.bias, conv.res_fc.weight, conv.res_fc.bias]
    _HeteroGATv2.last_rowmax = None
    out = _HeteroGATv2.apply(x_dst, nh, th.is_grad_enabled(), *flat)
    rm, _HeteroGATv2.last_rowmax = _HeteroGATv2.last_rowmax, None
    if rm is not None and rm[0] == out.data_ptr():
        out._uavgnn_rowmax = (rm[1], rm[2], _version_of(out))
    return out


def _version_of(t):
    return None if t.is_inference() else t._version


def _talk_transpose_if_needed(g, *tensors):
    if th.is_grad_enabled() and any(t is not None and t.requires_grad for t in tensors):
        return g.talk_transpose()
    return None, None, None


def _talk_env(g, M, K):
    go, n_max = g.graph_off, g.hints.get("max_graph_agents")
    if go is None or not go.is_cuda or n_max is None or n_max < 1:
        return None
    if not L.lib().uavgnn_talk_attn_env_supported(int(n_max), int(M), int(K)):
        return None
    return go, go.numel() - 1, int(n_max)


def _launch_talk_fwd(env, s, ld_s, q, ld_q, v, ld_v, K, M, talk_off, talk_src, N, scale, c, ld_c, a_save, x_copy, ld_x,
                     n_copy):
    with KERNEL_TIMER.span("talk_attn_fwd"):
        if env is not None:
            go, B, n_max = env
            rc = L.lib().uavgnn_talk_attn_env_fwd(s, ld_s, q, ld_q, v, ld_v, K, M, L.ptr(talk_off), L.ptr(talk_src),
                                                  go.data_ptr(), B, n_max, scale, c, ld_c, a_save, x_copy, ld_x, n_copy,
                                                  L.stream())
        else:
            rc = L.lib().uavgnn_talk_attn_fwd(s, ld_s, q, ld_q, v, ld_v, K, M, L.ptr(talk_off), L.ptr(talk_src), N,
                                              scale, c, ld_c, a_save, x_copy, ld_x, n_copy, L.stream())
    L.check(rc, "uavgnn_talk_attn_fwd")


def _launch_talk_bwd(env, s, ld_s, q, ld_q, v, ld_v, K, M, talk_off, talk_src, transpose, N, scale, a_save, d_c, ld_dc,
                     d_s, ld_ds, d_q, ld_dq, d_v, ld_dv):
    with KERNEL_TIMER.span("talk_attn_bwd"):
        if env is not None:
            go, B, n_max = env
            rc = L.lib().uavgnn_talk_attn_env_bwd(s, ld_s, q, ld_q, v, ld_v, K, M, L.ptr(talk_off), L.ptr(talk_src),
                                                  go.data_ptr(), B, n_max, scale, a_save.data_ptr(), d_c, ld_dc, d_s,
                                                  ld_ds, d_q, ld_dq, d_v, ld_dv, L.stream())
        else:
            t_off, t_dst, t_pos = transpose
            de = th.empty_like(a_save) if s is not None else None
            rc = L.lib().uavgnn_talk_attn_bwd(s, ld_s, q, ld_q, v, ld_v, K, M, L.ptr(talk_off), L.ptr(talk_src),
                                              L.ptr(t_off), L.ptr(t_dst), L.ptr(t_pos), N, scale, a_save.data_ptr(),
                                              d_c, ld_dc, d_s, ld_ds, d_q, ld_dq, d_v, ld_dv, L.ptr(de), L.stream())
    L.check(rc, "uavgnn_talk_attn_bwd")


class _TalkAttention(th.autograd.Function):

    @staticmethod
    def forward(ctx, s, q, v, talk_off, talk_src, t_off, t_dst, t_pos, scale, env=None):
        L.require_gpu(v, talk_off, talk_src, s, q)
        N, M = v.shape
        K = 0 if s is None else s.shape[1]
# ... 92 lines not shown
_PLANES_MAX = 128


class frozen_weights:

    def __init__(self, store=None):
        self.store = store

    def __enter__(self):
        global _PLANES
        self.prev = _PLANES
        if self.store is not None:
            _PLANES = self.store
        elif _PLANES is None:
            _PLANES = {}
        return self

    def __exit__(self, *exc):
        global _PLANES
        _PLANES = self.prev
        return False


def _cached_planes(key, nbytes, device, build, keep=()):
    if _PLANES is not None:
        hit = _PLANES.pop(key, None)
        if hit is not None:
            _PLANES[key] = hit
            return hit[0]
    planes = th.empty(nbytes, dtype=th.uint8, device=device)
    build(planes)
    if _PLANES is not None:
        while len(_PLANES) >= _PLANES_MAX:
            victim = next((k for k in _PLANES if k[0] != "k1img"), None)
            if victim is None:
                break
            del _PLANES[victim]
        _PLANES[key] = (planes, tuple(keep))
    return planes


def gru_cell_two_piece_supported(x, c, h) -> bool:
    K1, K2, H = x.shape[1], c.shape[1], h.shape[1]
    return bool(GRU_X3 and K1 >= 32 and K1 % 32 == 0 and K2 % 32 == 0 and _mc_operand(x) and _mc_operand(c)
                and L.lib().uavgnn_gru_cell_x3_supported(K1 + K2, H)
                and 4 * x.shape[0] * max(x.stride(0), c.stride(0), H) < 2 ** 32)


def gru_cell_h2_supported(K_in, H, N, ld_max) -> bool:
    return bool(GRU_H2 and GRU_X3 and N >= GRU_FUSED_MIN_ROWS and L.lib().uavgnn_gru_cell_h2_supported(K_in, H)
                and 4 * N * max(ld_max, H) < 2 ** 32)


def _gru_cell_launch(inp, h, W_ih, b_ih, W_hh, b_hh, save, inp2=None, h2_out=None, rowmax=None):
    N, H = h.shape
    h2 = th.empty_like(h) if h2_out is None else h2_out
    pre = th.empty((N, 4 * H), dtype=th.float32, device=h.device) if save else None
    if rowmax is not None:
        lib, K1, K2 = L.lib(), inp.shape[1], (0 if inp2 is None else inp2.shape[1])
        K_in = K1 + K2
        with KERNEL_TIMER.span("gru_cell_fwd", (N, K_in, H, "f16x2")):
            planes = _cached_planes(("gruh2", W_ih.data_ptr(), W_hh.data_ptr(), W_ih._version, W_hh._version, K_in, H),
                                    lib.uavgnn_gru_cell_h2_workspace_bytes(K_in, H), h.device,
                                    lambda p: L.check(lib.uavgnn_gru_split_weights_h2(W_ih.data_ptr(), K_in, W_hh.data_ptr(), H,
                                                                                      p.data_ptr(), L.stream()),
                                                      "uavgnn_gru_split_weights_h2"), keep=(W_ih, W_hh))
            rc = lib.uavgnn_gru_cell_fwd_h2(inp.data_ptr(), inp.stride(0), K1, L.ptr(inp2), 0 if inp2 is None else inp2.stride(0), K2,
                                            h.data_ptr(), N, H, rowmax.data_ptr(), planes.data_ptr(), b_ih.data_ptr(), b_hh.data_ptr(),
                                            h2.data_ptr(), L.ptr(pre), L.stream())
        L.check(rc, "uavgnn_gru_cell_fwd_h2")
        return h2, pre
    if inp2 is not None or (GRU_X3 and L.lib().uavgnn_gru_cell_x3_supported(inp.shape[1], H)
                            and 4 * N * max(inp.stride(0), H) < 2 ** 32):
        lib, K1, K2 = L.lib(), inp.shape[1], (0 if inp2 is None else inp2.shape[1])
        K_in = K1 + K2
        with KERNEL_TIMER.span("gru_cell_fwd", (N, K_in, H, "bf16x3")):
            planes = _cached_planes(("gru", W_ih.data_ptr(), W_hh.data_ptr(), W_ih._version, W_hh._version, K_in, H),
                                    lib.uavgnn_gru_cell_x3_workspace_bytes(K_in, H), h.device,
                                    lambda p: L.check(lib.uavgnn_gru_split_weights(W_ih.data_ptr(), K_in, W_hh.data_ptr(), H,
                                                                                   p.data_ptr(), L.stream()),
                                                      "uavgnn_gru_split_weights"), keep=(W_ih, W_hh))
            rc = lib.uavgnn_gru_cell_fwd_x3_opts(inp.data_ptr(), inp.stride(0), K1, L.ptr(inp2),
                                                 0 if inp2 is None else inp2.stride(0), K2, h.data_ptr(), N, H, planes.data_ptr(),
                                                 b_ih.data_ptr(), b_hh.data_ptr(), h2.data_ptr(), L.ptr(pre), GRU_X3_FLAGS,
                                                 L.stream())
        L.check(rc, "uavgnn_gru_cell_fwd_x3_opts")
        return h2, pre
    with KERNEL_TIMER.span("gru_cell_fwd", (N, inp.shape[1], H, "f32")):
        rc = L.lib().uavgnn_gru_cell_fwd(inp.data_ptr(), inp.stride(0), inp.shape[1], h.data_ptr(), N, H, W_ih.data_ptr(),
                                         b_ih.data_ptr(), W_hh.data_ptr(), b_hh.data_ptr(), h2.data_ptr(), L.ptr(pre),
                                         L.stream())
    L.check(rc, "uavgnn_gru_cell_fwd")
    return h2, pre


def _gru_gates_bwd_from_pre(pre, h, d_hout, d_gi=None, d_gh=None, head=None, sums=None, rowmax=None):
    N, H = h.shape
    if d_gi is None:
        d_gi = th.empty((N, 3 * H), dtype=th.float32, device=h.device)
    if d_gh is None:
        d_gh = th.empty_like(d_gi)
    dh = th.empty_like(h)
    with KERNEL_TIMER.span("gru_gates_bwd"):
        if sums is not None and rowmax is not None:
            dq, W_out = head if head is not None else (None, None)
            rc = L.lib().uavgnn_gru_gates_bwd_fused_sums_rowmax(pre.data_ptr(), h.data_ptr(), L.ptr(d_hout), L.ptr(dq),
                                                                0 if dq is None else dq.shape[1], L.ptr(W_out), N, H, d_gi.data_ptr(),
                                                                d_gh.data_ptr(), dh.data_ptr(), sums.data_ptr(), rowmax.data_ptr(),
                                                                L.stream())
        elif sums is not None:
            dq, W_out = head if head is not None else (None, None)
            rc = L.lib().uavgnn_gru_gates_bwd_fused_sums(pre.data_ptr(), h.data_ptr(), L.ptr(d_hout), L.ptr(dq),
                                                         0 if dq is None else dq.shape[1], L.ptr(W_out), N, H, d_gi.data_ptr(),
                                                         d_gh.data_ptr(), dh.data_ptr(), sums.data_ptr(), L.stream())
        elif head is not None:
            dq, W_out = head
            rc = L.lib().uavgnn_gru_gates_bwd_fused_head(pre.data_ptr(), h.data_ptr(), L.ptr(d_hout), dq.data_ptr(), dq.shape[1],
                                                         W_out.data_ptr(), N, H, d_gi.data_ptr(), d_gh.data_ptr(), dh.data_ptr(),
                                                         L.stream())
        else:
            rc = L.lib().uavgnn_gru_gates_bwd_fused(pre.data_ptr(), h.data_ptr(), d_hout.data_ptr(), N, H, d_gi.data_ptr(),
                                                    d_gh.data_ptr(), dh.data_ptr(), L.stream())
# ... 126 lines not shown
    if relu:
        return th._addmm_activation(b, x, W.t())
    return th.addmm(b, x, W.t()) if b is not None else th.mm(x, W.t())


def _mm_nn(dy, W, out=None, accumulate=False, rowmax=None):
    if rowmax is not None and gemm_h2_supported(dy, W.shape[1], W.shape[0]) and W.stride(1) == 1 and \
            (out is None or (out.stride(1) == 1 and out.dtype == th.float32)):
        return gemm_h2(dy, W, rowmax, True, out=out, accumulate=accumulate)
    if gemm_x3_supported(dy, W.shape[1], W.shape[0]) and W.stride(1) == 1 and \
            (out is None or (out.stride(1) == 1 and out.dtype == th.float32)):
        return gemm_x3(dy, W, True, out=out, accumulate=accumulate)
    if out is None:
        return th.mm(dy, W)
    return out.addmm_(dy, W) if accumulate else th.mm(dy, W, out=out)


def gemm_x3_cat_supported(a1, a2, n_out) -> bool:
    K1, K2 = a1.shape[1], a2.shape[1]
    return bool(a2.is_cuda and a2.dtype == th.float32 and a2.dim() == 2 and a2.shape[0] == a1.shape[0] and K1 % 32 == 0
                and K2 % 32 == 0 and _mc_operand(a2)
                and a2.shape[0] * a2.stride(0) < 2 ** 31 and gemm_x3_supported(a1, n_out, K1 + K2)
                and ((a1.shape[0] + 255) // 256) * ((n_out + 127) // 128) >= GEMM_X3_SMALL_GRID and not (GEMM_X3_FLAGS & 8))


def gemm_x3_cat(a1, a2, W1, W2, out):
    lib = L.lib()
    M, K1 = a1.shape
    K2, n_out = a2.shape[1], W1.shape[1]
    K = K1 + K2
    assert W1.shape[0] == K1 and W2.shape == (K2, n_out) and W1.stride(1) == 1 and W2.stride(1) == 1

    def build(p):
        Wc = th.cat((W1, W2), 0)
        L.check(lib.uavgnn_split_bf16x3(Wc.data_ptr(), n_out, K, n_out, 1, p.data_ptr(), L.stream()), "uavgnn_split_bf16x3")
    with KERNEL_TIMER.span("gemm_x3", (M, n_out, K)):
        planes = _cached_planes(("matcat", W1.data_ptr(), W1._version, W1.stride(0), W2.data_ptr(), W2._version, W2.stride(0), K1, K2,
                                 n_out), 6 * K * n_out, a1.device, build, keep=(W1, W2))
        rc = lib.uavgnn_gemm_nt_x3_cat(a1.data_ptr(), a1.stride(0), K1, a2.data_ptr(), a2.stride(0), M, K, planes.data_ptr(), n_out,
                                       None, out.data_ptr(), out.stride(0), GEMM_X3_FLAGS & 4, L.stream())
    L.check(rc, "uavgnn_gemm_nt_x3_cat")
    return out


GEMM_H2 = os.environ.get("UAVGNN_GEMM_H2", "1") != "0"


def gemm_h2_supported(a, n_out, k) -> bool:
    return bool(GEMM_H2 and gemm_x3_supported(a, n_out, k) and L.lib().uavgnn_gemm_h2_supported(a.shape[0], n_out, k)
                and ((a.shape[0] + 255) // 256) * ((n_out + 127) // 128) >= GEMM_X3_SMALL_GRID)


def gemm_h2(a, W, rowmax, transpose_w=False, bias=None, out=None, accumulate=False, relu=False, a2=None, W2=None, rowmax2=None,
            rowmax2_out=None):
    lib = L.lib()
    M, K1 = a.shape
    if a2 is not None:
        assert transpose_w and W2 is not None and W.stride(1) == 1 and W2.stride(1) == 1
        K2, n_out = a2.shape[1], W.shape[1]
        K = K1 + K2
        key = ("h2cat", W.data_ptr(), W._version, W.stride(0), W2.data_ptr(), W2._version, W2.stride(0), K1, K2, n_out)

        def build(p):
            Wc = th.cat((W, W2), 0)
            L.check(lib.uavgnn_split_h2(Wc.data_ptr(), n_out, K, n_out, 1, p.data_ptr(), L.stream()), "uavgnn_split_h2")
        keep = (W, W2)
    else:
        R, C = W.shape
        n_out, K = (C, R) if transpose_w else (R, C)
        assert K == K1 and W.stride(1) == 1
        key = ("h2mat", W.data_ptr(), W._version, W.stride(0), R, C, bool(transpose_w))

        def build(p):
            L.check(lib.uavgnn_split_h2(W.data_ptr(), W.stride(0), R, C, int(transpose_w), p.data_ptr(), L.stream()), "uavgnn_split_h2")
        keep = (W,)
    if out is None:
        out = th.empty((M, n_out), dtype=th.float32, device=a.device)
    with KERNEL_TIMER.span("gemm_h2", (M, n_out, K)):
        planes = _cached_planes(key, lib.uavgnn_split_h2_bytes(n_out, K), a.device, build, keep=keep)
        fn, rm2 = (lib.uavgnn_gemm_nt_h2, rowmax2) if rowmax2_out is None else (lib.uavgnn_gemm_nt_h2_rm2, rowmax2_out)
        rc = fn(a.data_ptr(), a.stride(0), K1, L.ptr(a2), 0 if a2 is None else a2.stride(0), M, K, rowmax.data_ptr(),
                L.ptr(rm2), planes.data_ptr(), n_out, L.ptr(bias), out.data_ptr(), out.stride(0),
                (1 if accumulate else 0) | (2 if relu else 0) | (GEMM_X3_FLAGS & 4), L.stream())
    L.check(rc, "uavgnn_gemm_nt_h2")
    return out


G4 = os.environ.get("UAVGNN_G4", "1") != "0"
DC_H2 = os.environ.get("UAVGNN_DC_H2", "1") != "0"
GEMM_H2_N64_MIN_GRID = 128


def gemm_h2_n64_supported(a, n_out, k) -> bool:
    return bool(DC_H2 and GEMM_H2 and a.is_cuda and a.dtype == th.float32 and a.dim() == 2 and _mc_operand(a) and a.shape[1] == k
                and n_out % 64 == 0 and k % 64 == 0 and a.shape[0] * a.stride(0) < 2 ** 31
                and L.lib().uavgnn_gemm_h2_supported(a.shape[0], n_out, k)
                and ((a.shape[0] + 127) // 128) * (n_out // 64) >= GEMM_H2_N64_MIN_GRID)


def gemm_h2_n64(a, W, rowmax, out=None):
    lib = L.lib()
    M, K = a.shape
    R, n_out = W.shape
    assert R == K and W.stride(1) == 1
    if out is None:
        out = th.empty((M, n_out), dtype=th.float32, device=a.device)
    with KERNEL_TIMER.span("gemm_h2_n64", (M, n_out, K)):
        planes = _cached_planes(("h2mat", W.data_ptr(), W._version, W.stride(0), R, n_out, True), lib.uavgnn_split_h2_bytes(n_out, K),
                                a.device, lambda p: L.check(lib.uavgnn_split_h2(W.data_ptr(), W.stride(0), R, n_out, 1, p.data_ptr(),
                                                                                 L.stream()), "uavgnn_split_h2"), keep=(W,))
        rc = lib.uavgnn_gemm_nt_h2_n64(a.data_ptr(), a.stride(0), M, K, rowmax.data_ptr(), planes.data_ptr(), n_out, out.data_ptr(),
                                       out.stride(0), L.stream())
    L.check(rc, "uavgnn_gemm_nt_h2_n64")
    return out


GEMM_TN_MIN_ROWS = 1 << 18
GEMM_TN_H2 = os.environ.get("UAVGNN_GEMM_TN_H2", "1") != "0"


def _max_two_stage(t):
    n = t.numel()
    S = 1
    while S < 1024 and n % (2 * S) == 0 and n // (2 * S) >= 256:
        S *= 2
    return t.reshape(S, n // S).max(1).values.max()


def gemm_tn_h2_supported(dy, x, min_in=128) -> bool:
    return bool(GEMM_X3 and GEMM_H2 and GEMM_TN_H2 and dy.is_cuda and dy.dtype == th.float32 and x.dtype == th.float32 and dy.dim() == 2
                and x.dim() == 2 and dy.shape[0] == x.shape[0] and dy.shape[0] >= GEMM_TN_MIN_ROWS and _mc_operand(dy) and _mc_operand(x)
                and dy.shape[1] >= 256 and x.shape[1] >= min_in
                and L.lib().uavgnn_gemm_tn_h2_supported(dy.shape[0], dy.shape[1], x.shape[1]))


def gemm_tn_x3_supported(dy, x) -> bool:
# ... 19 lines not shown

    @staticmethod
    def forward(ctx, x, W, b):
        ctx.save_for_backward(x, W)
        ctx.has_bias = b is not None
        return _mm_nt(x, W, b)

    @staticmethod
    def backward(ctx, dy):
        x, W = ctx.saved_tensors
        return _LinearSplitK._grads(ctx, x, W, dy, ctx.has_bias)

    @staticmethod
    def _grads(ctx, x, W, dy, has_bias, rowmax=None, x_rowmax=None):
        dy = dy.contiguous()
        dx = dW = db = None
        if ctx.needs_input_grad[0]:
            dx = _mm_nn(dy, W, rowmax=rowmax)
        if ctx.needs_input_grad[1] and rowmax is not None and x_rowmax is not None and gemm_tn_h2_supported(dy, x):
            lib = L.lib()
            n, Mo, Ko = dy.shape[0], dy.shape[1], x.shape[1]
            S = lib.uavgnn_gemm_tn_h2_chunks(n, Mo, Ko)
            part = th.empty((S, Mo, Ko), dtype=th.float32, device=x.device)
            cy, cx = _max_two_stage(rowmax).expand(Mo).contiguous(), _max_two_stage(x_rowmax).expand(Ko).contiguous()
            with KERNEL_TIMER.span("gemm_tn_h2", (n, Mo, Ko)):
                rc = lib.uavgnn_gemm_tn_h2(dy.data_ptr(), dy.stride(0), Mo, x.data_ptr(), x.stride(0), Ko, n, cy.data_ptr(), cx.data_ptr(),
                                           part.data_ptr(), S, 0, L.stream())
            L.check(rc, "uavgnn_gemm_tn_h2")
            dW = part.sum(0)
        elif ctx.needs_input_grad[1] and gemm_tn_x3_supported(dy, x):
            dW = gemm_tn_x3(dy, x).sum(0)
        elif ctx.needs_input_grad[1]:
            n, S = x.shape[0], WeightGradSink._chunks(x.shape[0])
            if S > 1:
                xc = x if x.is_contiguous() else x.contiguous()
                part = th.bmm(dy.view(S, n // S, -1).transpose(1, 2), xc.view(S, n // S, -1))
                dW = part.sum(0)
            else:
                dW = th.mm(dy.t(), x)
        if has_bias and ctx.needs_input_grad[2]:
            db = _colsum(dy)
        return dx, dW, db


def linear(x, W, b=None):
    return _LinearSplitK.apply(x, W, b)


RELU_BWD_FUSED = os.environ.get("UAVGNN_RELU_BWD_FUSED", "1") != "0"


class _LinearReLU(th.autograd.Function):

    @staticmethod
    def forward(ctx, x, W, b, rm_a=None, rm_b=None, train=True):
        ctx.x_rowmax = None
        ctx.n_extra = 0 if rm_a is None else 3
        n_out = W.shape[0]
        rm = None if rm_a is None else (rm_a, rm_b)
        if (rm is not None and b is not None and b.is_contiguous() and W.stride(1) == 1 and gemm_h2_supported(x, n_out, W.shape[1])):
            y = gemm_h2(x, W, rm[0], False, bias=b, relu=True, rowmax2=rm[1])
            if ctx.needs_input_grad[1] and train:
                ctx.x_rowmax = th.maximum(rm[0], rm[1])
            ctx.save_for_backward(x, W, y)
            return y
        if (ctx.needs_input_grad[1] and n_out % 4 == 0 and gemm_x3_supported(x, n_out, W.shape[1]) and W.stride(1) == 1 and b is not None
                and b.is_contiguous() and x.shape[0] >= GEMM_TN_MIN_ROWS and GEMM_TN_H2 and GEMM_H2 and n_out >= 256 and x.shape[1] >= 128
                and L.lib().uavgnn_gemm_tn_h2_supported(x.shape[0], n_out, x.shape[1])):
            ctx.x_rowmax = th.empty(x.shape[0], dtype=th.float32, device=x.device)
            y = gemm_x3(x, W, False, bias=b, relu=True, rowmax_out=ctx.x_rowmax)
        else:
            y = _mm_nt(x, W, b, relu=True)
        ctx.save_for_backward(x, W, y)
        return y

    @staticmethod
    def backward(ctx, dy):
        x, W, y = ctx.saved_tensors
        n, C = dy.shape
        if (RELU_BWD_FUSED and ctx.needs_input_grad[2] and dy.is_cuda and dy.dtype == th.float32 and y.dtype == th.float32 and n > 0
                and C % 4 == 0 and _mc_operand(dy) and _mc_operand(y)
                and dy.stride(0) >= C and y.stride(0) >= C):
            S = _row_blocks(n)
            dym = th.empty((n, C), dtype=th.float32, device=dy.device)
            part = th.zeros((S, C), dtype=th.float32, device=dy.device)
            rowmax = None
            if C == 256 and ctx.needs_input_grad[0] and gemm_h2_supported(dym, W.shape[1], C) and W.stride(1) == 1:
                rowmax = th.empty(n, dtype=th.float32, device=dy.device)
                L.check(L.lib().uavgnn_relu_bwd_colsum_rowmax(dy.data_ptr(), dy.stride(0), y.data_ptr(), y.stride(0), dym.data_ptr(), C, n,
                                                              C, part.data_ptr(), S, rowmax.data_ptr(), L.stream()),
                        "uavgnn_relu_bwd_colsum_rowmax")
            else:
                L.check(L.lib().uavgnn_relu_bwd_colsum(dy.data_ptr(), dy.stride(0), y.data_ptr(), y.stride(0), dym.data_ptr(), C, n, C,
                                                       part.data_ptr(), S, L.stream()), "uavgnn_relu_bwd_colsum")
            dx, dW, _ = _LinearSplitK._grads(ctx, x, W, dym, False, rowmax=rowmax, x_rowmax=ctx.x_rowmax)
            return (dx, dW, part.sum(0)) + (None,) * ctx.n_extra
        dy = th.ops.aten.threshold_backward(dy, y, 0.0)
        return tuple(_LinearSplitK._grads(ctx, x, W, dy, True)) + (None,) * ctx.n_extra


def linear_relu(x, W, b):
    rm = getattr(x, "_uavgnn_rowmax", None)
    if rm is not None and rm[2] == _version_of(x):
        return _LinearReLU.apply(x, W, b, rm[0], rm[1], th.is_grad_enabled())
    return _LinearReLU.apply(x, W, b)


FLAT_OBS_FUSED = os.environ.get("UAVGNN_FLAT_OBS_FUSED", "auto")
FLAT_OBS_AUTO_MAX_ROWS = 1 << 15
FLAT_OBS_AUTO_MAX_F = 64


def flat_obs_supported(parts, W, needs_grad=False) -> bool:
    F = sum(p.shape[1] for p in parts)
    rows = parts[0].shape[0]
    mode = str(FLAT_OBS_FUSED)
    if mode == "0" or (mode != "1" and (needs_grad or rows > FLAT_OBS_AUTO_MAX_ROWS or F > FLAT_OBS_AUTO_MAX_F)):
        return False
    return bool(W.is_cuda and W.dtype == th.float32 and W.is_contiguous() and W.shape[1] == F
                and all(p.is_cuda and p.dtype == th.float32 and p.dim() == 2 and p.shape[0] == rows
                        and (p.stride(1) == 1 or p.shape[1] <= 1) and (rows <= 1 or p.stride(0) >= p.shape[1]) for p in parts)
                and rows < 2 ** 31 and L.lib().uavgnn_flat_obs_supported(W.shape[0], F))


def _flat_src(parts):
    out = []
    for p in parts:
        out += [p.data_ptr() if p.shape[1] else None, p.stride(0) if p.shape[0] > 1 else p.shape[1], p.shape[1]]
    return out


class _FlatLinearReLU(th.autograd.Function):

    @staticmethod
    def forward(ctx, W, b, agent, gt, ubs):
        parts = (agent, gt, ubs)
        rows, H = agent.shape[0], W.shape[0]
        y = th.empty((rows, H), dtype=th.float32, device=W.device)
        with KERNEL_TIMER.span("flat_obs_fwd", (rows, H, W.shape[1])):
            rc = L.lib().uavgnn_flat_obs_fwd(*_flat_src(parts), rows, W.data_ptr(), L.ptr(b), H, y.data_ptr(), y.stride(0), L.stream())
        L.check(rc, "uavgnn_flat_obs_fwd")
        ctx.has_bias = b is not None
        ctx.save_for_backward(y, agent, gt, ubs)
        return y

    @staticmethod
    def backward(ctx, dy):
        y, agent, gt, ubs = ctx.saved_tensors
        parts = (agent, gt, ubs)
        n, H = dy.shape
        F = sum(p.shape[1] for p in parts)
        lib = L.lib()
        if dy.stride(1) != 1 or dy.stride(0) < H or dy.stride(0) % 4 or dy.data_ptr() % 16:
            dy = dy.contiguous()
        S = _row_blocks(n)
        dym = th.empty((n, H), dtype=th.float32, device=dy.device)
        db_part = th.zeros((S, H), dtype=th.float32, device=dy.device)
# ... 195 lines not shown
    n, S = x.shape[0], WeightGradSink._chunks(x.shape[0])
    if S == 1:
        return th.mm(dy.t(), x)
    return th.bmm(dy.view(S, n // S, -1).transpose(1, 2), x.view(S, n // S, -1)).sum(0)


GRAD_SINK = None
SEQ_STAGING = os.environ.get("UAVGNN_SEQ_STAGING", "1") != "0"


def _add_grad(p, g):
    if p.grad is None:
        p.grad = g.clone()
    else:
        p.grad.add_(g)


def _add_grad_cols(p, g, start):
    if p.grad is None:
        p.grad = th.zeros_like(p)
    p.grad[start:start + g.shape[0]].add_(g)


class _TimeSplit(th.autograd.Function):

    @staticmethod
    def forward(ctx, x_all, T1, holder):
        N = x_all.shape[0] // T1
        buf = th.empty((T1, N, x_all.shape[1]), dtype=x_all.dtype, device=x_all.device)
        holder.append(buf)
        ctx.buf = buf
        return tuple(x_all.detach().view(T1, N, -1).unbind(0))

    @staticmethod
    def backward(ctx, *grads):
        buf = ctx.buf
        for t, g in enumerate(grads):
            if g is None:
                buf[t].zero_()
            elif g.data_ptr() != buf[t].data_ptr() or g.stride() != buf[t].stride():
                buf[t].copy_(g)
        return buf.view(-1, buf.shape[2]), None, None


def time_split(x_all, T1):
    if not (th.is_grad_enabled() and x_all.requires_grad):
        return x_all.view(T1, x_all.shape[0] // T1, -1).unbind(0), [None] * T1
    holder = []
    xs = _TimeSplit.apply(x_all, T1, holder)
    return xs, list(holder[0].unbind(0))


MSG_FUSED = os.environ.get("UAVGNN_MSG_FUSED", "1") != "0"


def _tarmac_msg_plan(x, h, Wp, bp, M, K, env, N, H):
    if not MSG_FUSED or env is None or N == 0:
        return None
    _, B, n_ag = env
    if N != B * n_ag or (H + M) % 4 or not L.lib().uavgnn_tarmac_msg_supported(H, M, K, n_ag):
        return None
    if (Wp.shape != (M + 2 * K, 2 * H) or not Wp.is_contiguous() or Wp.data_ptr() % 16 or not bp.is_contiguous()
            or x.data_ptr() % 16 or h.data_ptr() % 16 or x.dtype != th.float32 or Wp.dtype != th.float32):
        return None
    lib = L.lib()
    tiles = _cached_planes(("msgw", Wp.data_ptr(), Wp._version, H, M, K), lib.uavgnn_tarmac_msg_weight_bytes(H, M, K), x.device,
                           lambda buf: L.check(lib.uavgnn_tarmac_msg_prepare(Wp.data_ptr(), Wp.stride(0), H, M, K, buf.data_ptr(),
                                                                            L.stream()), "uavgnn_tarmac_msg_prepare"),
                           keep=(Wp,))
    return tiles, n_ag


def _launch_tarmac_msg(msg, x, h, bp, M, K, talk_off, talk_src, N, H, c_ptr, ld_c, a_save, proj, ld_p, x_copy, ld_xc, planes=None,
                       rowmax=None):
    tiles, n_ag = msg
    if rowmax is not None:
        with KERNEL_TIMER.span("tarmac_msg_fwd", (N, H, M, K, int(proj is not None), int(x_copy is not None))):
            rc = L.lib().uavgnn_tarmac_msg_fwd_rowmax(x.data_ptr(), x.stride(0), h.data_ptr(), h.stride(0), N, H, n_ag, tiles.data_ptr(),
                                                      bp.data_ptr(), M, K, L.ptr(talk_off), L.ptr(talk_src), 1.0 / K, c_ptr, ld_c, a_save,
                                                      proj, ld_p, x_copy, ld_xc, rowmax.data_ptr(), L.stream())
        L.check(rc, "uavgnn_tarmac_msg_fwd_rowmax")
        return
    with KERNEL_TIMER.span("tarmac_msg_fwd", (N, H, M, K, int(proj is not None), int(x_copy is not None))):
        rc = L.lib().uavgnn_tarmac_msg_fwd(x.data_ptr(), x.stride(0), h.data_ptr(), h.stride(0), N, H, n_ag, tiles.data_ptr(),
                                           bp.data_ptr(), M, K, L.ptr(talk_off), L.ptr(talk_src), 1.0 / K, c_ptr, ld_c, a_save, proj,
                                           ld_p, x_copy, ld_xc, L.ptr(planes), L.stream())
    L.check(rc, "uavgnn_tarmac_msg_fwd")


def head_fwd(h, W_out, b_out):
    N, H = h.shape
    A = W_out.shape[0]
    if (h.is_cuda and h.dtype == th.float32 and N > 0 and _mc_operand(h) and _mc_operand(W_out)
            and b_out.is_contiguous() and L.lib().uavgnn_head_supported(H, A)):
        q = th.empty((N, A), dtype=th.float32, device=h.device)
        with KERNEL_TIMER.span("head_fwd", (N, H, A)):
            rc = L.lib().uavgnn_head_fwd(h.data_ptr(), h.stride(0), N, H, W_out.data_ptr(), W_out.stride(0), b_out.data_ptr(), A,
                                         q.data_ptr(), A, L.stream())
        L.check(rc, "uavgnn_head_fwd")
        return q
    return th.addmm(b_out, h, W_out.t())


class _TarmacStep(th.autograd.Function):

    @staticmethod
    def forward(ctx, x, h, Wp, bp, W_ih, b_ih, W_hh, b_hh, W_out, b_out, M, K, talk_off, talk_src, t_off, t_dst, t_pos,
                split, env=None, dx_out=None, train=True):
        L.require_gpu(x, h, Wp, W_ih, talk_off)
        N, H = x.shape
        x, h = L.f32c(x), L.f32c(h)
        msg = _tarmac_msg_plan(x, h, Wp, bp, M, K, env, N, H)
        if msg is not None:
            proj = None
        elif gemm_x3_supported(x, Wp.shape[0], H) and gemm_x3_supported(h, Wp.shape[0], H) and bp.is_contiguous():
            proj = gemm_x3(x, Wp[:, :H], bias=bp)
            gemm_x3(h, Wp[:, H:], out=proj, accumulate=True)
        else:
            proj = th.addmm(bp, x, Wp[:, :H].t())
            proj.addmm_(h, Wp[:, H:].t())
        E = talk_src.shape[0]
        a_save = th.empty(max(E, 1), dtype=th.float32, device=x.device)
        ld = M + 2 * K
        ctx.seq = ctx.seq_t = None
        aligned = all(t.is_contiguous() and t.data_ptr() % 16 == 0 for t in (W_ih, W_hh))
        rowmax = None
        if (msg is not None and aligned and GRU_FUSED and gru_cell_h2_supported(H + M, H, N, max(x.stride(0), H + M))
                and H % 32 == 0 and M % 32 == 0 and L.lib().uavgnn_tarmac_msg_rowmax_supported(H, M, K, msg[1])):
            rowmax = th.empty(N, dtype=th.float32, device=x.device)
        c_only = None
        if not train and aligned and h.shape[0] >= GRU_FUSED_MIN_ROWS and GRU_FUSED:
            c_only = th.empty((N, M), dtype=th.float32, device=x.device)
            if not gru_cell_two_piece_supported(x, c_only, h):
                c_only = None
        if c_only is not None:
            if msg is not None:
                _launch_tarmac_msg(msg, x, h, bp, M, K, talk_off, talk_src, N, H, c_only.data_ptr(), M, None, None, 0, None, 0,
                                   rowmax=rowmax)
            else:
                _launch_talk_fwd(env, proj.data_ptr() + 4 * M, ld, proj.data_ptr() + 4 * (M + K), ld, proj.data_ptr(), ld, K, M,
                                 talk_off, talk_src, N, 1.0 / K, c_only.data_ptr(), M, a_save.data_ptr(), None, 0, 0)
            h2, _ = _gru_cell_launch(x, h, W_ih, b_ih, W_hh, b_hh, save=False, inp2=c_only, rowmax=rowmax)
            inp, fused = c_only, True
            gi = gh = h2
        else:
            seq = GRAD_SINK.seq if (train and GRAD_SINK is not None) else None
            if seq is not None and (seq.t_fwd >= seq.T1 or N != seq.N or seq.x_all.shape[1] != H or
                                    x.data_ptr() != seq.x_all.data_ptr() + 4 * H * N * seq.t_fwd):
                seq = None
            if seq is not None and seq.t_fwd > 0 and h.data_ptr() != seq.slot("h", seq.t_fwd, H, extra=1).data_ptr():
                seq = None
            if seq is not None:
                seq_t = seq.t_fwd
                seq.t_fwd += 1
                seq.steps[seq_t] = _StepRecord()
                inp = seq.slot("inp", seq_t, H + M)
                if seq_t == 0:
                    seq.slot("h", 0, H, extra=1).copy_(h)
            else:
                inp = th.empty((N, H + M), dtype=th.float32, device=x.device)
            if seq is not None and rowmax is not None:
                rowmax = seq.slot("rowmax", seq_t, 1).view(N)
                seq.steps[seq_t].rowmax = True
            if msg is not None:
                proj = th.empty((N, ld), dtype=th.float32, device=x.device)
                _launch_tarmac_msg(msg, x, h, bp, M, K, talk_off, talk_src, N, H, inp.data_ptr() + 4 * H, H + M, a_save.data_ptr(),
                                   proj.data_ptr(), ld, inp.data_ptr(), H + M, rowmax=rowmax)
            else:
                _launch_talk_fwd(env, proj.data_ptr() + 4 * M, ld, proj.data_ptr() + 4 * (M + K), ld, proj.data_ptr(), ld, K, M,
                                 talk_off, talk_src, N, 1.0 / K, inp.data_ptr() + 4 * H, H + M, a_save.data_ptr(), x.data_ptr(),
                                 x.stride(0), H)
            fused = gru_cell_supported(inp, h) and aligned
            if fused:
                h2, pre = _gru_cell_launch(inp, h, W_ih, b_ih, W_hh, b_hh, save=bool(train),
                                           h2_out=None if seq is None else seq.slot("h", seq_t + 1, H, extra=1), rowmax=rowmax)
                if seq is not None and pre is not None:
                    ctx.seq, ctx.seq_t = seq, seq_t
                gi = gh = pre if pre is not None else h2
            else:
                gi = th.addmm(b_ih, inp, W_ih.t())
                gh = th.addmm(b_hh, h, W_hh.t())
                h2 = th.empty_like(h)
                with KERNEL_TIMER.span("gru_gates_fwd"):
                    rc = L.lib().uavgnn_gru_gates_fwd(gi.data_ptr(), gh.data_ptr(), h.data_ptr(), N, H, h2.data_ptr(), L.stream())
                L.check(rc, "uavgnn_gru_gates_fwd")
        q = head_fwd(h2, W_out, b_out)
        if proj is None:
            proj = h2
        ctx.dims = (M, K)
        ctx.split, ctx.env, ctx.dx_out, ctx.fused_gru = split, env, dx_out, fused
        ctx.have_pre = bool(train) or not fused
        ctx.save_for_backward(x, h, proj, inp, gi, gh, h2, a_save, Wp, W_ih, W_hh, W_out, talk_off, talk_src, t_off,
                              t_dst, t_pos)
        return q, h2

    @staticmethod
    def backward(ctx, dq, dh2):
        (x, h, proj, inp, gi, gh, h2, a_save, Wp, W_ih, W_hh, W_out, talk_off, talk_src, t_off, t_dst,
         t_pos) = ctx.saved_tensors
        N, H = x.shape
        if not ctx.have_pre:
            raise L.UavGnnError("tarmac_step: backward through a forward that saved no pre-activations (train=False)")
        sink = GRAD_SINK
        dq = L.f32c(dq) if dq is not None else th.zeros((N, W_out.shape[0]), dtype=th.float32, device=x.device)
        seq = ctx.seq if (sink is not None and ctx.seq is not None and sink.seq is ctx.seq) else None
        head, dh2_tot = _step_dh2(ctx.fused_gru, sink, dq, dh2, W_out, N, H)
        d_gi, d_gh, dh, rm_g, g4 = _step_gate_grads(seq, ctx.seq_t, ctx.fused_gru, gi, gh, h, dh2_tot, head, W_hh)
        dx, d_proj = _step_input_grads(seq, ctx.seq_t, sink, ctx.dims, ctx.env, ctx.dx_out, proj, a_save, Wp, W_ih, W_hh,
                                       (talk_off, talk_src, (t_off, t_dst, t_pos)), d_gi, d_gh, dh, rm_g, g4)
        gWp = gbp = gWih = gbih = gWhh = gbhh = gWo = gbo = None
        ids = {"Wp": id(Wp), "W_ih": id(W_ih), "W_hh": id(W_hh), "W_out": id(W_out)}
        if seq is not None:
            seq.steps[ctx.seq_t].dq = dq
            seq.bwd_steps.append(ctx.seq_t)
            seq.split, seq.H, seq.ids = ctx.split, H, ids
        elif sink is not None:
            sink.step_grads(ctx.split, ids, H, x, h, h2, inp, d_proj, d_gi, d_gh, dq)
        else:
            gWp = th.cat((_wgrad(d_proj, x), _wgrad(d_proj, h)), 1)
            gbp = _colsum(d_proj)
            gWih, gbih = _wgrad(d_gi, inp), _colsum(d_gi)
            gWhh, gbhh = _wgrad(d_gh, h), th.cat((gbih[:2 * H], _colsum(d_gh[:, 2 * H:])))
            gWo, gbo = _wgrad(dq, h2), _colsum(dq)
        return (dx, dh, gWp, gbp, gWih, gbih, gWhh, gbhh, gWo, gbo) + (None,) * 11


def _step_dh2(fused_gru, sink, dq, dh2, W_out, N, H):
    if (fused_gru and H % 4 == 0 and W_out.shape[0] <= 64 and W_out.is_contiguous()
            and W_out.dtype == th.float32 and W_out.data_ptr() % 16 == 0
            and (dh2 is None or (dh2.is_contiguous() and dh2.dtype == th.float32 and dh2.shape == (N, H)))):
        if sink is not None:
            sink.owned.clear()
        return (dq, W_out.detach()), dh2
    if dh2 is None:
        return None, th.mm(dq, W_out)
    if (sink is not None and dh2.is_contiguous() and dh2.dtype == th.float32 and dh2.shape == (N, H)
            and sink.owned.get(dh2.data_ptr()) is not None):
        sink.owned.clear()
# ... 68 lines not shown
            rm_p = seq.slot("rm_p", t, 1).view(N)
            seq.steps[t].rm_p = True
        else:
            rm_p = th.empty(N, dtype=th.float32, device=d_gi.device)
        gemm_h2(d_gi, W_ih[:, :H], rm_g, True, out=dx, a2=d_proj, W2=Wp[:, :H], rowmax2_out=rm_p)
    elif dx_cat:
        gemm_x3_cat(d_gi, d_proj, W_ih[:, :H], Wp[:, :H], dx)
    elif split_dinp:
        dx.addmm_(d_proj, Wp[:, :H])
    elif dx_out is not None:
        dx = th.addmm(d_inp[:, :H], d_proj, Wp[:, :H], out=dx_out)
    else:
        dx = th.addmm(d_inp[:, :H], d_proj, Wp[:, :H])
    return dx, d_proj


def tarmac_step(x, h, g, comm, f_out, stacked=None, dx_out=None):
    M, K = comm._msg_size, comm._key_size
    Wp, bp = stacked if stacked is not None else comm.fused_projection()
    off, src = g.talk_csc()
    cell = comm.f_udt
    env = _talk_env(g, M, K)
    t_off, t_dst, t_pos = ((None, None, None) if env is not None else
                           _talk_transpose_if_needed(g, x, h, Wp, cell.weight_ih, f_out.weight))
    H = cell.weight_hh.shape[1]
    params = {"W_ih": cell.weight_ih, "b_ih": cell.bias_ih, "W_hh": cell.weight_hh, "b_hh": cell.bias_hh,
              "W_out": f_out.weight, "b_out": f_out.bias}

    def split(name, grad, col0):
        if name == "Wp":
            r = 0
            for lin in (comm.f_val, comm.f_sign, comm.f_que):
                rows = lin.weight.shape[0]
                if lin.weight.grad is None:
                    lin.weight.grad = th.zeros_like(lin.weight)
                lin.weight.grad[:, col0:col0 + grad.shape[1]].add_(grad[r:r + rows])
                r += rows
        elif name == "bp":
            r = 0
            for lin in (comm.f_val, comm.f_sign, comm.f_que):
                rows = lin.bias.shape[0]
                _add_grad(lin.bias, grad[r:r + rows])
                r += rows
        elif name == "b_ih":
            _add_grad(params["b_ih"], grad)
            _add_grad_cols(params["b_hh"], grad[:2 * H], 0)
        elif name == "b_hh":
            _add_grad_cols(params["b_hh"], grad, col0)
        else:
            _add_grad(params[name], grad)

    train = th.is_grad_enabled() and any(t.requires_grad for t in (x, h, Wp, bp, cell.weight_ih, cell.bias_ih,
                                                                   cell.weight_hh, cell.bias_hh, f_out.weight, f_out.bias))
    return _TarmacStep.apply(x, h, Wp, bp, cell.weight_ih, cell.bias_ih, cell.weight_hh, cell.bias_hh, f_out.weight,
                             f_out.bias, M, K, off, src, t_off, t_dst, t_pos, split, env, dx_out, train)


class _DiscComm(th.autograd.Function):

    @staticmethod
    def forward(ctx, logits, gumbel, talk_off, talk_src, t_off, t_dst, t_pos, inv_tau, rng=None):
        L.require_gpu(logits, gumbel, talk_off, talk_src, rng)
        logits = L.f32c(logits)
        N, M2 = logits.shape
        M = M2 // 2
        E = talk_src.shape[0]
        if gumbel is not None:
            gumbel = L.f32c(gumbel)
            if gumbel.numel() != E * M2:
                raise L.UavGnnError(f"disc_comm: gumbel noise must be [E={E}, msg={M}, 2]")
        elif rng is None or rng.dtype != th.int64 or rng.numel() != 2:
            raise L.UavGnnError("disc_comm: either the Gumbel noise or a device int64 {seed, step} pair is required")
        c = th.empty((N, M2), dtype=th.float32, device=logits.device)
        y0 = th.empty((max(E, 1), M), dtype=th.float32, device=logits.device)
        sel = th.empty((N, M2), dtype=th.int32, device=logits.device)
        with KERNEL_TIMER.span("disc_comm_fwd"):
            rc = L.lib().uavgnn_disc_comm_fwd(logits.data_ptr(), M2, L.ptr(gumbel), L.ptr(rng), M, L.ptr(talk_off),
                                              L.ptr(talk_src), N, float(inv_tau), c.data_ptr(), M2, y0.data_ptr(),
                                              sel.data_ptr(), L.stream())
        L.check(rc, "uavgnn_disc_comm_fwd")
        ctx.inv_tau, ctx.M = float(inv_tau), M
        ctx.save_for_backward(y0, sel, t_off, t_dst, t_pos)
        return c

    @staticmethod
    def backward(ctx, d_c):
        y0, sel, t_off, t_dst, t_pos = ctx.saved_tensors
        d_c = L.f32c(d_c)
        N = d_c.shape[0]
        d_logits = th.empty_like(d_c)
        with KERNEL_TIMER.span("disc_comm_bwd"):
            rc = L.lib().uavgnn_disc_comm_bwd(d_c.data_ptr(), d_c.stride(0), y0.data_ptr(), sel.data_ptr(), ctx.M,
                                              L.ptr(t_off), L.ptr(t_dst), L.ptr(t_pos), N, ctx.inv_tau,
                                              d_logits.data_ptr(), d_logits.stride(0), L.stream())
        L.check(rc, "uavgnn_disc_comm_bwd")
        return d_logits, None, None, None, None, None, None, None, None


def disc_comm_aggregate(logits, gumbel, g, tau=0.5, rng=None):
    off, src = g.talk_csc()
    t_off, t_dst, t_pos = _talk_transpose_if_needed(g, logits)
    return _DiscComm.apply(logits, gumbel, off, src, t_off, t_dst, t_pos, 1.0 / tau, rng)


def gumbel_noise(rng, E, msg):
    out = th.empty((E, msg, 2), dtype=th.float32, device=rng.device)
    L.check(L.lib().uavgnn_gumbel_noise(rng.data_ptr(), E, msg, out.data_ptr(), L.stream()), "uavgnn_gumbel_noise")
    return out
# ... 1 lines not shown
```

Measured before the change: 2.647 million.

## Propagate per-row abs-max bounds from GEMM/GRU epilogues into an h2 TarMAC message kernel

Adds epilogue variants of the h2 GEMM and the GRU cell kernel that emit per-row, per-column-block abs-max values alongside their outputs. It also adds an h2 TarMAC message kernel that takes these precomputed bounds for x and h. The goal is to skip separate row-absmax passes over the activations before the split-precision message projection. The cost is extra shuffle reductions and stores in the epilogues, plus Python-side bookkeeping (a last_hmax handoff and row-bound caching) that could go stale if pointers are reused.

```diff
diff --git a/include/uavgnn.h b/include/uavgnn.h
--- a/include/uavgnn.h
+++ b/include/uavgnn.h
@@ -116,6 +116,9 @@
 int uavgnn_split_h2(const float* W, int ld, int R, int C, int transpose, void* planes, uavgnn_stream_t stream);
 int uavgnn_gemm_nt_h2(const float* X, int ldx, int K1, const float* X2, int ldx2, int M, int K, const float* rowmax, const float* rowmax2,
                       const void* planes, int N, const float* bias, float* Y, int ldy, int epilogue, uavgnn_stream_t stream);
+int uavgnn_gemm_nt_h2_ymax(const float* X, int ldx, int K1, const float* X2, int ldx2, int M, int K, const float* rowmax, const float* rowmax2,
+                           const void* planes, int N, const float* bias, float* Y, int ldy, int epilogue, float* ymax,
+                           uavgnn_stream_t stream);
 int uavgnn_gemm_nt_h2_rm2(const float* X, int ldx, int K1, const float* X2, int ldx2, int M, int K, const float* rowmax, float* rowmax2_out,
                           const void* planes, int N, const float* bias, float* Y, int ldy, int epilogue, uavgnn_stream_t stream);
 int uavgnn_gemm_nt_h2_n64(const float* X, int ldx, int M, int K, const float* rowmax, const void* planes, int N, float* Y, int ldy,
@@ -160,6 +163,13 @@
                                  const float* bias, int M, int K, const int32_t* talk_off, const int32_t* talk_src, float scale,
                                  float* c_out, int ld_c, float* a_save, float* proj_out, int ld_p, float* x_copy, int ld_xc,
                                  float* row_absmax, uavgnn_stream_t stream);
+int uavgnn_tarmac_msg_h2_supported(int H, int M, int K, int n_ag);
+long long uavgnn_tarmac_msg_weight_bytes_h2(int H, int M, int K);
+int uavgnn_tarmac_msg_prepare_h2(const float* Wp, int ld, int H, int M, int K, void* tiles, uavgnn_stream_t stream);
+int uavgnn_tarmac_msg_fwd_h2(const float* x, int ld_x, const float* h, int ld_h, int N, int H, int n_ag, const float* x_bound, int ld_xb,
+                             int n_xb, const float* h_bound, int ld_hb, int n_hb, const void* tiles, const float* bias, int M, int K,
+                             const int32_t* talk_off, const int32_t* talk_src, float scale, float* c_out, int ld_c, float* a_save,
+                             float* proj_out, int ld_p, float* x_copy, int ld_xc, float* row_absmax, uavgnn_stream_t stream);
 
 size_t uavgnn_degree_order_workspace_bytes(int N);
 int uavgnn_degree_order(const int32_t* seg_off, int N, int32_t* order, void* workspace, size_t workspace_bytes,
@@ -209,6 +219,9 @@
 int uavgnn_gru_cell_fwd_h2(const float* inp, int ld_inp, int K1, const float* inp2, int ld_inp2, int K2, const float* h, int N, int H,
                            const float* row_absmax, const void* planes, const float* b_ih, const float* b_hh, float* h_out,
                            float* pre_save, uavgnn_stream_t stream);
+int uavgnn_gru_cell_fwd_h2_hmax(const float* inp, int ld_inp, int K1, const float* inp2, int ld_inp2, int K2, const float* h, int N, int H,
+                                const float* row_absmax, const void* planes, const float* b_ih, const float* b_hh, float* h_out,
+                                float* pre_save, float* hmax, uavgnn_stream_t stream);
 int uavgnn_row_absmax(const float* a1, int ld1, int K1, const float* a2, int ld2, int K2, const float* a3, int ld3, int K3, int N,
                       float* out, uavgnn_stream_t stream);
 int uavgnn_head_supported(int H, int A);
diff --git a/uav_bs_ctrl_amd/_lib.py b/uav_bs_ctrl_amd/_lib.py
--- a/uav_bs_ctrl_amd/_lib.py
+++ b/uav_bs_ctrl_amd/_lib.py
@@ -114,6 +114,8 @@
                                    _c_int, _c_int, _c_st]),
     "uavgnn_gemm_nt_h2_rm2": (_c_int, [_c_fp, _c_int, _c_int, _c_fp, _c_int, _c_int, _c_int, _c_fp, _c_fp, ctypes.c_void_p, _c_int, _c_fp, _c_fp,
                                        _c_int, _c_int, _c_st]),
+    "uavgnn_gemm_nt_h2_ymax": (_c_int, [_c_fp, _c_int, _c_int, _c_fp, _c_int, _c_int, _c_int, _c_fp, _c_fp, ctypes.c_void_p, _c_int, _c_fp, _c_fp,
+                                        _c_int, _c_int, _c_fp, _c_st]),
     "uavgnn_gemm_nt_h2_n64": (_c_int, [_c_fp, _c_int, _c_int, _c_int, _c_fp, ctypes.c_void_p, _c_int, _c_fp, _c_int, _c_st]),
     "uavgnn_env_state_dim": (_c_int, [_c_int, _c_int, _c_int]),
     "uavgnn_env_step": (_c_int, [ctypes.POINTER(ctypes.c_int32), ctypes.POINTER(ctypes.c_double), _c_int] + [_c_fp] * 22 + [_c_st]),
@@ -134,10 +136,18 @@
     "uavgnn_gru_split_weights_h2": (_c_int, [_c_fp, _c_int, _c_fp, _c_int, ctypes.c_void_p, _c_st]),
     "uavgnn_gru_cell_fwd_h2": (_c_int, [_c_fp, _c_int, _c_int, _c_fp, _c_int, _c_int, _c_fp, _c_int, _c_int, _c_fp, ctypes.c_void_p, _c_fp,
                                         _c_fp, _c_fp, _c_fp, _c_st]),
+    "uavgnn_gru_cell_fwd_h2_hmax": (_c_int, [_c_fp, _c_int, _c_int, _c_fp, _c_int, _c_int, _c_fp, _c_int, _c_int, _c_fp, ctypes.c_void_p, _c_fp,
+                                             _c_fp, _c_fp, _c_fp, _c_fp, _c_st]),
     "uavgnn_row_absmax": (_c_int, [_c_fp, _c_int, _c_int, _c_fp, _c_int, _c_int, _c_fp, _c_int, _c_int, _c_int, _c_fp, _c_st]),
     "uavgnn_tarmac_msg_rowmax_supported": (_c_int, [_c_int, _c_int, _c_int, _c_int]),
     "uavgnn_tarmac_msg_fwd_rowmax": (_c_int, [_c_fp, _c_int, _c_fp, _c_int, _c_int, _c_int, _c_int, ctypes.c_void_p, _c_fp, _c_int, _c_int,
                                               _c_ip, _c_ip, _c_f32, _c_fp, _c_int, _c_fp, _c_fp, _c_int, _c_fp, _c_int, _c_fp, _c_st]),
+    "uavgnn_tarmac_msg_h2_supported": (_c_int, [_c_int, _c_int, _c_int, _c_int]),
+    "uavgnn_tarmac_msg_weight_bytes_h2": (ctypes.c_longlong, [_c_int, _c_int, _c_int]),
+    "uavgnn_tarmac_msg_prepare_h2": (_c_int, [_c_fp, _c_int, _c_int, _c_int, _c_int, ctypes.c_void_p, _c_st]),
+    "uavgnn_tarmac_msg_fwd_h2": (_c_int, [_c_fp, _c_int, _c_fp, _c_int, _c_int, _c_int, _c_int, _c_fp, _c_int, _c_int, _c_fp, _c_int, _c_int,
+                                          ctypes.c_void_p, _c_fp, _c_int, _c_int, _c_ip, _c_ip, _c_f32, _c_fp, _c_int, _c_fp, _c_fp, _c_int,
+                                          _c_fp, _c_int, _c_fp, _c_st]),
     "uavgnn_gru_weight_tiles_bytes": (ctypes.c_longlong, [_c_int, _c_int]),
     "uavgnn_gru_split_weight_tiles": (_c_int, [_c_fp, _c_int, _c_fp, _c_int, ctypes.c_void_p, _c_st]),
     "uavgnn_gru_cell_fwd_planes": (_c_int, [ctypes.c_void_p, _c_int, _c_fp, _c_int, _c_int, ctypes.c_void_p, _c_fp, _c_fp, _c_fp, _c_fp,
diff --git a/uav_bs_ctrl_amd/csrc/gemm_h2.hip b/uav_bs_ctrl_amd/csrc/gemm_h2.hip
--- a/uav_bs_ctrl_amd/csrc/gemm_h2.hip
+++ b/uav_bs_ctrl_amd/csrc/gemm_h2.hip
@@ -39,7 +39,7 @@
                                                           const float* __restrict__ bias, float* __restrict__ Y, int ldy,
                                                           int row_blocks, int col_blocks, const float* __restrict__ X2, int ldx2,
                                                           int ns1, const float* __restrict__ rm1, const float* __restrict__ rm2,
-                                                          float* __restrict__ rm2_out) {
+                                                          float* __restrict__ rm2_out, float* __restrict__ ymax) {
   constexpr int kTileChunks = BM8 * (BN + 4) / 4;
 #ifndef UAVGNN_GEMM_H2_TILE_STORE
 #define UAVGNN_GEMM_H2_TILE_STORE 1
@@ -279,6 +279,17 @@
       if constexpr (ACC) o = {yv[q].x + t.x, yv[q].y + t.y, yv[q].z + t.z, yv[q].w + t.w};
       if (RELU) o = {fmaxf(o.x, 0.f), fmaxf(o.y, 0.f), fmaxf(o.z, 0.f), fmaxf(o.w, 0.f)};
       if (m0 + row < M) *reinterpret_cast<float4*>(Y + static_cast<size_t>(m0 + row) * ldy + n0 + 4 * cc) = o;
+      if (ymax != nullptr) {
+        const float a0 = fabsf(o.x), a1 = fabsf(o.y), a2 = fabsf(o.z), a3 = fabsf(o.w);
+        float m = fmaxf(fmaxf(a0, a1), fmaxf(a2, a3));
+        if (!(fabsf(t.x) <= 3.4028234663852886e38f) || !(fabsf(t.y) <= 3.4028234663852886e38f) || !(fabsf(t.z) <= 3.4028234663852886e38f) ||
+            !(fabsf(t.w) <= 3.4028234663852886e38f) || !(a0 <= 3.4028234663852886e38f) || !(a1 <= 3.4028234663852886e38f) ||
+            !(a2 <= 3.4028234663852886e38f) || !(a3 <= 3.4028234663852886e38f))
+          m = INFINITY;
+#pragma unroll
+        for (int off = 1; off < 32; off <<= 1) m = fmaxf(m, __shfl_xor(m, off));
+        if (cc == 0 && m0 + row < M) ymax[static_cast<size_t>(m0 + row) * col_blocks + cb] = m;
+      }
     }
     return;
   }
@@ -453,7 +464,7 @@
 
 static int gemm_nt_h2_launch(const float* X, int ldx, int K1, const float* X2, int ldx2, int M, int K, const float* rowmax,
                              const float* rowmax2, float* rowmax2_out, const void* planes, int N, const float* bias, float* Y, int ldy,
-                             int epilogue, uavgnn_stream_t stream) {
+                             int epilogue, uavgnn_stream_t stream, float* ymax = nullptr) {
   if (M < 0 || !X || !planes || !Y || !rowmax || ldx < K1 || ldy < N || K1 <= 0 || K1 > K || (X2 == nullptr) != (K1 == K) ||
       (X2 != nullptr && ldx2 < K - K1) || (rowmax2_out != nullptr && (X2 == nullptr || rowmax2 != nullptr)))
     return UAVGNN_EINVAL;
@@ -464,6 +475,7 @@
     return UAVGNN_EUNSUPPORTED;
   if (X2 != nullptr && ((K1 % BK) || (ldx2 & 3) || static_cast<long long>(M) * ldx2 >= (1LL << 31) || (reinterpret_cast<uintptr_t>(X2) & 15)))
     return UAVGNN_EUNSUPPORTED;
+  if (ymax != nullptr && ((N % BN) || (ldy & 3) || (reinterpret_cast<uintptr_t>(Y) & 15) || !UAVGNN_GEMM_H2_TILE_STORE)) return UAVGNN_EUNSUPPORTED;
   const int ns1 = K1 / BK;
   hipStream_t st = static_cast<hipStream_t>(stream);
   const unsigned short* bp = static_cast<const unsigned short*>(planes);
@@ -473,7 +485,7 @@
   const dim3 grid(((row_blocks + 7) / 8) * 8 * col_blocks), block(NT);
 #define UAVGNN_H2_GEMM(ACC, RELU, IL)                                                                                              \
   hipLaunchKernelGGL((gemm_nt_h2w8_kernel<ACC, RELU, IL>), grid, block, 0, st, X, ldx, M, K, bp, N, winv, bias, Y, ldy, row_blocks, \
-                     col_blocks, X2, ldx2, ns1, rowmax, rowmax2, rowmax2_out)
+                     col_blocks, X2, ldx2, ns1, rowmax, rowmax2, rowmax2_out, ymax)
 #define UAVGNN_H2_GEMM_IL(IL)                         \
   if (acc && relu) UAVGNN_H2_GEMM(true, true, IL);    \
   else if (acc) UAVGNN_H2_GEMM(true, false, IL);      \
@@ -490,6 +502,13 @@
                                  const float* rowmax2, const void* planes, int N, const float* bias, float* Y, int ldy, int epilogue,
                                  uavgnn_stream_t stream) {
   return gemm_nt_h2_launch(X, ldx, K1, X2, ldx2, M, K, rowmax, rowmax2, nullptr, planes, N, bias, Y, ldy, epilogue, stream);
+}
+
+extern "C" int uavgnn_gemm_nt_h2_ymax(const float* X, int ldx, int K1, const float* X2, int ldx2, int M, int K, const float* rowmax,
+                                      const float* rowmax2, const void* planes, int N, const float* bias, float* Y, int ldy, int epilogue,
+                                      float* ymax, uavgnn_stream_t stream) {
+  if (!ymax) return UAVGNN_EINVAL;
+  return gemm_nt_h2_launch(X, ldx, K1, X2, ldx2, M, K, rowmax, rowmax2, nullptr, planes, N, bias, Y, ldy, epilogue, stream, ymax);
 }
 
 extern "C" int uavgnn_gemm_nt_h2_rm2(const float* X, int ldx, int K1, const float* X2, int ldx2, int M, int K, const float* rowmax,
diff --git a/uav_bs_ctrl_amd/csrc/gru_h2.hip b/uav_bs_ctrl_amd/csrc/gru_h2.hip
--- a/uav_bs_ctrl_amd/csrc/gru_h2.hip
+++ b/uav_bs_ctrl_amd/csrc/gru_h2.hip
@@ -48,7 +48,8 @@
     const float* __restrict__ inp, int ld_inp, int K1, const float* __restrict__ inp2, int ld_inp2, int K2,
     const float* __restrict__ h, int N, int H, const float* __restrict__ row_absmax,
     const unsigned short* __restrict__ Wih_p, const float* __restrict__ b_ih, const unsigned short* __restrict__ Whh_p,
-    const float* __restrict__ b_hh, const float* __restrict__ winv, float* __restrict__ h_out, float* __restrict__ pre, int row_blocks) {
+    const float* __restrict__ b_hh, const float* __restrict__ winv, float* __restrict__ h_out, float* __restrict__ pre, int row_blocks,
+    float* __restrict__ hmax) {
   __shared__ u32x4 smem[2 * BUF];
   __shared__ float sInv[BM];
   const int tid = threadIdx.x, lane = tid & 63, wave = tid >> 6;
@@ -283,9 +284,18 @@
 #pragma unroll
   for (int q = 0; q < 4; ++q) {
     const int idx = tid + NT * q, row = idx >> 4, cc = idx & 15;
-    if (m0 + row < N)
-      *reinterpret_cast<float4*>(h_out + static_cast<size_t>(m0 + row) * H + j0 + 4 * cc) =
-          *reinterpret_cast<const float4*>(sH + row * ST + 4 * cc);
+    const float4 v = *reinterpret_cast<const float4*>(sH + row * ST + 4 * cc);
+    if (m0 + row < N) *reinterpret_cast<float4*>(h_out + static_cast<size_t>(m0 + row) * H + j0 + 4 * cc) = v;
+    if (hmax != nullptr) {
+      const float a0 = fabsf(v.x), a1 = fabsf(v.y), a2 = fabsf(v.z), a3 = fabsf(v.w);
+      float m = fmaxf(fmaxf(a0, a1), fmaxf(a2, a3));
+      if (!(a0 <= 3.4028234663852886e38f) || !(a1 <= 3.4028234663852886e38f) || !(a2 <= 3.4028234663852886e38f) ||
+          !(a3 <= 3.4028234663852886e38f))
+        m = INFINITY;
+#pragma unroll
+      for (int o = 1; o < 16; o <<= 1) m = fmaxf(m, __shfl_xor(m, o));
+      if (cc == 0 && m0 + row < N) hmax[static_cast<size_t>(m0 + row) * CB + cb] = m;
+    }
   }
 }
 
@@ -317,9 +327,9 @@
   return launch_status();
 }
 
-extern "C" int uavgnn_gru_cell_fwd_h2(const float* inp, int ld_inp, int K1, const float* inp2, int ld_inp2, int K2, const float* h,
-                                      int N, int H, const float* row_absmax, const void* planes, const float* b_ih,
-                                      const float* b_hh, float* h_out, float* pre_save, uavgnn_stream_t stream) {
+static int gru_cell_h2_launch(const float* inp, int ld_inp, int K1, const float* inp2, int ld_inp2, int K2, const float* h, int N, int H,
+                              const float* row_absmax, const void* planes, const float* b_ih, const float* b_hh, float* h_out,
+                              float* pre_save, float* hmax, uavgnn_stream_t stream) {
   const int K_in = K1 + K2;
   if (N < 0 || !inp || !h || !planes || !b_ih || !b_hh || !h_out || !row_absmax || ld_inp < K1 || K2 < 0 ||
       (K2 > 0 && (!inp2 || ld_inp2 < K2)))
@@ -343,11 +353,24 @@
   const dim3 grid(rb8 * (H / BJ)), block(NT);
   if (pre_save != nullptr)
     hipLaunchKernelGGL(gru_cell_fwd_h2_kernel<true>, grid, block, 0, st, inp, ld_inp, K1, inp2, ld_inp2, K2, h, N, H, row_absmax, p0, b_ih,
-                       p1, b_hh, winv, h_out, pre_save, row_blocks);
+                       p1, b_hh, winv, h_out, pre_save, row_blocks, hmax);
   else
     hipLaunchKernelGGL(gru_cell_fwd_h2_kernel<false>, grid, block, 0, st, inp, ld_inp, K1, inp2, ld_inp2, K2, h, N, H, row_absmax, p0, b_ih,
-                       p1, b_hh, winv, h_out, pre_save, row_blocks);
+                       p1, b_hh, winv, h_out, pre_save, row_blocks, hmax);
   return launch_status();
+}
+
+extern "C" int uavgnn_gru_cell_fwd_h2(const float* inp, int ld_inp, int K1, const float* inp2, int ld_inp2, int K2, const float* h,
+                                      int N, int H, const float* row_absmax, const void* planes, const float* b_ih,
+                                      const float* b_hh, float* h_out, float* pre_save, uavgnn_stream_t stream) {
+  return gru_cell_h2_launch(inp, ld_inp, K1, inp2, ld_inp2, K2, h, N, H, row_absmax, planes, b_ih, b_hh, h_out, pre_save, nullptr, stream);
+}
+
+extern "C" int uavgnn_gru_cell_fwd_h2_hmax(const float* inp, int ld_inp, int K1, const float* inp2, int ld_inp2, int K2, const float* h,
+                                           int N, int H, const float* row_absmax, const void* planes, const float* b_ih,
+                                           const float* b_hh, float* h_out, float* pre_save, float* hmax, uavgnn_stream_t stream) {
+  if (!hmax) return UAVGNN_EINVAL;
+  return gru_cell_h2_launch(inp, ld_inp, K1, inp2, ld_inp2, K2, h, N, H, row_absmax, planes, b_ih, b_hh, h_out, pre_save, hmax, stream);
 }
 
 namespace uavgnn {
diff --git a/uav_bs_ctrl_amd/csrc/tarmac_msg.hip b/uav_bs_ctrl_amd/csrc/tarmac_msg.hip
--- a/uav_bs_ctrl_amd/csrc/tarmac_msg.hip
+++ b/uav_bs_ctrl_amd/csrc/tarmac_msg.hip
@@ -2,26 +2,19 @@
 
 #include "bf16x3.h"
 #include "common.h"
+#include "tarmac_msg_pair.h"
 #include "uavgnn_probe.h"
 
 namespace uavgnn {
 namespace {
 
 using namespace x3;
-
-constexpr int kMsgWaves = 4;
-constexpr int kMsgRows = 16 * kMsgWaves;
-constexpr int kMsgThreads = kWave * kMsgWaves;
+using namespace msg;
+
 constexpr int kMaxCols = 128;
 
 __device__ __forceinline__ bf16x8 frag_of(unsigned a, unsigned b, unsigned c, unsigned d) {
   return __builtin_bit_cast(bf16x8, u32x4{a, b, c, d});
-}
-
-__device__ __forceinline__ void lds_barrier() {
-  __builtin_amdgcn_fence(__ATOMIC_RELEASE, "workgroup", "local");
-  __builtin_amdgcn_s_barrier();
-  __builtin_amdgcn_fence(__ATOMIC_ACQUIRE, "workgroup", "local");
 }
 
 struct Planes8 {
@@ -53,23 +46,6 @@
   u32x4* dst = tiles + static_cast<size_t>(s) * 3 * per_slice + r * 4 + (c ^ swz(r));
 #pragma unroll
   for (int p = 0; p < 3; ++p) dst[p * per_slice] = pl.p[p];
-}
-
-__device__ __forceinline__ void msg_scatter(float* __restrict__ Mx, int nmax, const float* __restrict__ VAL,
-                                            const int* __restrict__ SRC, const int* __restrict__ DST,
-                                            const int* __restrict__ OFF, int E, int lane) {
-  for (int e = lane; e < E; e += kWave) {
-    const int d = DST[e], sidx = SRC[e];
-    const int j0 = OFF[d], j1 = OFF[d + 1];
-    bool first = true;
-    for (int jx = j0; jx < e; ++jx) first = first && (SRC[jx] != sidx);
-    if (first) {
-      float acc = VAL[e];
-      for (int jx = e + 1; jx < j1; ++jx)
-        if (SRC[jx] == sidx) acc += VAL[jx];
-      Mx[d * nmax + sidx] = acc;
-    }
-  }
 }
 
 template <int CT, bool TRAIN, bool PLANES>
@@ -446,110 +422,8 @@
     }
   }
   lds_barrier();
-  int* __restrict__ OFF = reinterpret_cast<int*>(P + 16 * LDP);
-  float* __restrict__ SC = reinterpret_cast<float*>(OFF + NA + 4);
-  float* __restrict__ AD = SC + EMAX;
-  int* __restrict__ SRC = reinterpret_cast<int*>(AD + EMAX);
-  int* __restrict__ DST = SRC + EMAX;
-  float* __restrict__ AV = reinterpret_cast<float*>(DST + EMAX);
-  if (half == 1) {
-    if (TRAIN && proj_out != nullptr) {
-      for (int r = 0; r < 16; ++r) {
-        if (row0 + r >= N) break;
-        float* d = proj_out + static_cast<size_t>(row0 + r) * ld_p;
-        for (int col = lane; col < ncol; col += kWave) d[col] = P[r * LDP + col];
-      }
-    }
-    lds_barrier();
-    return;
-  }
-  bool poison = !ok;
-  if (ok) {
-    for (int i = lane; i < EMAX; i += kWave) AD[i] = 0.f;
-    if (lane <= 16) OFF[lane] = toff - e_lo;
-    wave_sync_lds();
-    bool bad = false;
-#pragma unroll
-    for (int i = 0; i < 4; ++i) {
-      const int e = lane + kWave * i;
-      if (e < E) {
-        const int u = fsrc[i] - row0;
-        bad |= (u < 0) | (u >= 16);
-        SRC[e] = u < 0 ? 0 : (u >= 16 ? 15 : u);
-        int d = 0;
-#pragma unroll
-        for (int jj = 1; jj < 16; ++jj) d += e >= OFF[jj];
-        DST[e] = d;
-      }
-    }
-    poison = __any(bad);
-    wave_sync_lds();
-    if (!poison) {
-      for (int e = lane; e < E; e += kWave) {
-        const float* __restrict__ sr = P + SRC[e] * LDP + M;
-        const float* __restrict__ qr = P + DST[e] * LDP + M + K;
-        float a = 0.f;
-#pragma unroll 4
-        for (int k = 0; k < K; ++k) a = fmaf(sr[k], qr[k], a);
-        SC[e] = a * scale;
-      }
-      wave_sync_lds();
-      for (int e = lane; e < E; e += kWave) {
-        const int d = DST[e];
-        const int j0 = OFF[d], j1 = OFF[d + 1];
-        float m = -INFINITY;
-#pragma unroll 2
-        for (int jj = j0; jj < j1; ++jj) m = fmaxf(m, SC[jj]);
-        float den = 0.f;
-#pragma unroll 2
-        for (int jj = j0; jj < j1; ++jj) den += expf(SC[jj] - m);
-        const float a = expf(SC[e] - m) / den;
-        if (TRAIN && a_save != nullptr) a_save[e_lo + e] = a;
-        AV[e] = a;
-      }
-      wave_sync_lds();
-      msg_scatter(AD, NA, AV, SRC, DST, OFF, E, lane);
-      wave_sync_lds();
-    }
-  }
-  lds_barrier();
-  if (poison) {
-    for (int i = 0; i < 16; ++i)
-      for (int ch = lane; ch < M; ch += kWave) P[i * LDP + ch] = NAN;
-  } else {
-    for (int c0 = 0; c0 < M; c0 += kWave) {
-      const int ch = c0 + lane, chc = ch < M ? ch : M - 1;
-      float v[NA];
-#pragma unroll
-      for (int t = 0; t < NA; ++t) v[t] = P[t * LDP + chc];
-#pragma unroll 4
-      for (int r = 0; r < NA; ++r) {
-        float a = 0.f;
-#pragma unroll
-        for (int t = 0; t < NA; t += 4) {
-          const float4 q = *reinterpret_cast<const float4*>(AD + r * NA + t);
-          a = fmaf(q.x, v[t], a);
-          a = fmaf(q.y, v[t + 1], a);
-          a = fmaf(q.z, v[t + 2], a);
-          a = fmaf(q.w, v[t + 3], a);
-        }
-        if (ch < M) P[r * LDP + ch] = a;
-      }
-    }
-  }
-  wave_sync_lds();
-  for (int r = 0; r < 16; ++r) {
-    if (row0 + r >= N) break;
-    float* d = c_out + static_cast<size_t>(row0 + r) * ld_c;
-    for (int ch = lane; ch < M; ch += kWave) d[ch] = P[r * LDP + ch];
-  }
-  if (RM) {
-    float cm = 0.f;
-    for (int ch = g; ch < M; ch += 4) cm = fmaxf(cm, fabsf(P[j * LDP + ch]));
-    cm = fmaxf(cm, __shfl_xor(cm, 16));
-    cm = fmaxf(cm, __shfl_xor(cm, 32));
-    if (g == 0 && row < N) row_absmax[row] = fmaxf(cm, fmaxf(sRowMax[tile][0][j], sRowMax[tile][1][j]));
-  }
+  pair_tail<LDP, TRAIN, RM>(P, half, lane, row0, N, M, K, ok, toff, e_lo, E, fsrc, scale, c_out, ld_c, a_save, proj_out, ld_p, row_absmax,
+                            &sRowMax[tile][0][0]);
 }
 
 }
diff --git a/uav_bs_ctrl_amd/csrc/tarmac_msg_h2.hip b/uav_bs_ctrl_amd/csrc/tarmac_msg_h2.hip
--- /dev/null
+++ b/uav_bs_ctrl_amd/csrc/tarmac_msg_h2.hip
@@ -0,0 +1,283 @@
+#include <math.h>
+
+#include "common.h"
+#include "f16x2.h"
+#include "tarmac_msg_pair.h"
+
+namespace uavgnn {
+namespace {
+
+using namespace h2;
+using namespace msg;
+
+typedef float f32x4 __attribute__((ext_vector_type(4)));
+
+__device__ __forceinline__ int swz16(int row) { return (row & 8) ? 3 : 0; }
+__device__ __forceinline__ f32x4 mfma16(f16x8 a, f16x8 b, f32x4 c) { return __builtin_amdgcn_mfma_f32_16x16x32_f16(a, b, c, 0, 0, 0); }
+
+constexpr float kFltMax = 3.4028234663852886e38f;
+
+__global__ __launch_bounds__(256) void tarmac_msg_prepare_h2_kernel(const float* __restrict__ W, int ld, int R, int RP, int H,
+                                                                    u32x4* __restrict__ tiles, float* __restrict__ winv) {
+  __shared__ float red[2][4];
+  const int r = blockIdx.x, tid = threadIdx.x;
+  const int nsx = H / 32, per_plane = RP * 4;
+  float s[2] = {1.f, 1.f};
+  if (r < R) {
+    const float* w = W + static_cast<size_t>(r) * ld;
+    float m[2] = {0.f, 0.f};
+    for (int i = tid; i < H; i += 256) {
+      m[0] = fmaxf(m[0], fabsf(w[i]));
+      m[1] = fmaxf(m[1], fabsf(w[H + i]));
+    }
+#pragma unroll
+    for (int p = 0; p < 2; ++p) {
+      m[p] = wave_max(m[p]);
+      if ((tid & 63) == 0) red[p][tid >> 6] = m[p];
+    }
+    __syncthreads();
+#pragma unroll
+    for (int p = 0; p < 2; ++p) {
+      const int se = scale_exp(fmaxf(fmaxf(red[p][0], red[p][1]), fmaxf(red[p][2], red[p][3])));
+      s[p] = pow2f(se);
+      if (tid == 0) winv[p * RP + r] = pow2f(-se);
+    }
+  } else if (tid < 2) {
+    winv[tid * RP + r] = 1.f;
+  }
+  for (int idx = tid; idx < 2 * nsx * 4; idx += 256) {
+    const int sl = idx >> 2, c = idx & 3;
+    u32x4 hi = {0u, 0u, 0u, 0u}, lo = {0u, 0u, 0u, 0u};
+    if (r < R) {
+      const float* src = W + static_cast<size_t>(r) * ld + 32 * sl + 4 * c;
+      const float4 a = *reinterpret_cast<const float4*>(src), b = *reinterpret_cast<const float4*>(src + 16);
+      const float sc = s[sl >= nsx];
+      const Split2 p0 = split_pair(a.x * sc, a.y * sc), p1 = split_pair(a.z * sc, a.w * sc), p2 = split_pair(b.x * sc, b.y * sc),
+                   p3 = split_pair(b.z * sc, b.w * sc);
+      hi = u32x4{p0.hi, p1.hi, p2.hi, p3.hi};
+      lo = u32x4{p0.lo, p1.lo, p2.lo, p3.lo};
+    }
+    u32x4* dst = tiles + static_cast<size_t>(sl) * 2 * per_plane + r * 4 + (c ^ swz16(r));
+    dst[0] = hi;
+    dst[per_plane] = lo;
+  }
+}
+
+template <int CT, bool TRAIN>
+__global__ __launch_bounds__(2 * kMsgThreads, 4) void tarmac_msg_fwd_h2_kernel(
+    const float* __restrict__ x, int ld_x, const float* __restrict__ h, int ld_h, int N, int H, const float* __restrict__ xb, int ld_xb,
+    int nxb, const float* __restrict__ hb, int ld_hb, int nhb, const u32x4* __restrict__ Wt, const float* __restrict__ winv,
+    const float* __restrict__ bias, int M, int K, const int32_t* __restrict__ talk_off, const int32_t* __restrict__ talk_src, float scale,
+    float* __restrict__ c_out, int ld_c, float* __restrict__ a_save, float* __restrict__ proj_out, int ld_p, float* __restrict__ x_copy,
+    int ld_xc, float* __restrict__ row_absmax) {
+  constexpr int kThreads = 2 * kMsgThreads;
+  constexpr int RP = 16 * CT;
+  constexpr int BCH = 2 * RP * 4;
+  constexpr int BPT = (2 * BCH + kThreads - 1) / kThreads;
+  static_assert(2 * BCH == BPT * kThreads, "every thread copies whole chunks of a stage: no clamped duplicates");
+  constexpr int LDP = RP + 1;
+  constexpr int kLoopBytes = 2 * 2 * BCH * 16, kTailBytes = kMsgWaves * (16 * LDP + kScratch) * 4;
+  __shared__ float sRowMax[kMsgWaves][2][16];
+  __shared__ __attribute__((aligned(16))) unsigned char smem_raw[kLoopBytes > kTailBytes ? kLoopBytes : kTailBytes];
+  u32x4(*sB)[2 * BCH] = reinterpret_cast<u32x4(*)[2 * BCH]>(smem_raw);
+
+  const int tid = threadIdx.x, lane = tid & 63;
+  const int wave = __builtin_amdgcn_readfirstlane(tid >> 6);
+  const int tile = wave & 3, half = wave >> 2;
+  const int j = lane & 15, g = lane >> 4;
+  const int row0 = blockIdx.x * kMsgRows + tile * 16;
+  const int row = row0 + j, rowc = min(row, N - 1);
+  const int nsx = H / 32;
+  const float* __restrict__ ar = (half ? h + static_cast<size_t>(rowc) * ld_h : x + static_cast<size_t>(rowc) * ld_x) + 4 * g;
+
+  f32x4 acc[CT];
+#pragma unroll
+  for (int ct = 0; ct < CT; ++ct) acc[ct] = f32x4{0.f, 0.f, 0.f, 0.f};
+
+  const char* __restrict__ wbase = reinterpret_cast<const char*>(Wt);
+  unsigned wo[BPT];
+#pragma unroll
+  for (int i = 0; i < BPT; ++i) {
+    const int q = tid + kThreads * i;
+    wo[i] = 16u * static_cast<unsigned>(q < BCH ? q : nsx * BCH + (q - BCH));
+  }
+  int lt = 0;
+  u32x4 rb[BPT];
+  auto load_b = [&]() {
+#pragma unroll
+    for (int i = 0; i < BPT; ++i) rb[i] = *reinterpret_cast<const u32x4*>(wbase + wo[i]);
+    if (lt + 1 < nsx) {
+      ++lt;
+      wbase += BCH * 16;
+    }
+  };
+  auto store_b = [&](int buf) {
+#pragma unroll
+    for (int i = 0; i < BPT; ++i) sB[buf][tid + kThreads * i] = rb[i];
+  };
+  float4 a0_lo, a0_hi, a1_lo, a1_hi;
+#define UAVGNN_MSG_LOAD_A(LO, HI, S)                              \
+  {                                                               \
+    const float* p_ = ar + 32 * min((S), nsx - 1);                \
+    LO = *reinterpret_cast<const float4*>(p_);                    \
+    HI = *reinterpret_cast<const float4*>(p_ + 16);               \
+  }
+  const int toff = half == 0 ? talk_off[min(row0 + min(lane, 16), N)] : 0;
+  float bnd = 0.f;
+  {
+    const float* bp = half ? hb + static_cast<size_t>(rowc) * ld_hb : xb + static_cast<size_t>(rowc) * ld_xb;
+    const int nb = half ? nhb : nxb;
+    bool bad = false;
+    for (int p = g; p < nb; p += 4) {
+      const float v = bp[p];
+      bad |= !(fabsf(v) <= kFltMax);
+      bnd = fmaxf(bnd, v);
+    }
+    if (bad) bnd = INFINITY;
+  }
+  load_b();
+  __builtin_amdgcn_sched_barrier(0);
+  UAVGNN_MSG_LOAD_A(a0_lo, a0_hi, 0)
+  UAVGNN_MSG_LOAD_A(a1_lo, a1_hi, 1)
+  __builtin_amdgcn_sched_barrier(0);
+  const int e_lo = __shfl(toff, 0);
+  const int E = __shfl(toff, 16) - e_lo;
+  const bool ok = E <= kEMax && E >= 0;
+  bnd = fmaxf(bnd, __shfl_xor(bnd, 16));
+  bnd = fmaxf(bnd, __shfl_xor(bnd, 32));
+  if (g == 0) sRowMax[tile][half][j] = bnd;
+  const int se = scale_exp(bnd);
+  const float rs = bnd <= kFltMax ? pow2f(se) : NAN;
+  const float rinv = pow2f(-se);
+  store_b(0);
+  load_b();
+  int fsrc[4];
+#pragma unroll
+  for (int i = 0; i < 4; ++i) fsrc[i] = (half == 0 && ok && lane + kWave * i < E) ? talk_src[e_lo + lane + kWave * i] : 0;
+  lds_barrier();
+
+#define UAVGNN_MSG_TERM(FA, PB)                                                                                      \
+  acc[cp] = mfma16(FA, as_frag(sb[(PB) * RP * 4 + (cp * 16 + j) * 4 + (g ^ swz16(j))]), acc[cp]);                    \
+  acc[cp + 1] = mfma16(FA, as_frag(sb[(PB) * RP * 4 + ((cp + 1) * 16 + j) * 4 + (g ^ swz16(j))]), acc[cp + 1]);
+#define UAVGNN_MSG_STEP(LO, HI, T)                                                                   \
+  if ((T) < nsx) {                                                                                   \
+    const int t_ = (T);                                                                              \
+    const Split2 s0 = split_pair(LO.x * rs, LO.y * rs), s1 = split_pair(LO.z * rs, LO.w * rs),       \
+                 s2 = split_pair(HI.x * rs, HI.y * rs), s3 = split_pair(HI.z * rs, HI.w * rs);       \
+    if (TRAIN && half == 0 && x_copy != nullptr && row < N) {           \
+      float* d = x_copy + static_cast<size_t>(row) * ld_xc + 32 * t_ + 4 * g;                        \
+      *reinterpret_cast<float4*>(d) = LO;                                                            \
+      *reinterpret_cast<float4*>(d + 16) = HI;                                                       \
+    }                                                                                                \
+    UAVGNN_MSG_LOAD_A(LO, HI, t_ + 2)                                                                \
+    const f16x8 fhi = as_frag(u32x4{s0.hi, s1.hi, s2.hi, s3.hi}), flo = as_frag(u32x4{s0.lo, s1.lo, s2.lo, s3.lo}); \
+    const u32x4* sb = sB[t_ & 1] + half * BCH;                                                       \
+    _Pragma("unroll") for (int cp = 0; cp < CT; cp += 2) {                                           \
+      UAVGNN_MSG_TERM(fhi, 1) UAVGNN_MSG_TERM(flo, 0) UAVGNN_MSG_TERM(fhi, 0)                        \
+    }                                                                                                \
+    store_b((t_ + 1) & 1);                    \
+    load_b();                                                                                        \
+    lds_barrier();                                                                                   \
+  }
+  for (int t = 0; t < nsx; t += 2) {
+    UAVGNN_MSG_STEP(a0_lo, a0_hi, t)
+    UAVGNN_MSG_STEP(a1_lo, a1_hi, t + 1)
+  }
+#undef UAVGNN_MSG_STEP
+#undef UAVGNN_MSG_TERM
+#undef UAVGNN_MSG_LOAD_A
+
+  float* __restrict__ P = reinterpret_cast<float*>(smem_raw) + tile * (16 * LDP + kScratch);
+  const int ncol = M + 2 * K;
+  float ri[4];
+#pragma unroll
+  for (int i = 0; i < 4; ++i) ri[i] = __shfl(rinv, 4 * g + i);
+  const float* __restrict__ wi = winv + half * RP;
+  if (half == 0) {
+#pragma unroll
+    for (int ct = 0; ct < CT; ++ct) {
+      const int col = ct * 16 + j;
+      const float b = col < ncol ? bias[col] : 0.f, ci = wi[col];
+#pragma unroll
+      for (int i = 0; i < 4; ++i) P[(4 * g + i) * LDP + col] = acc[ct][i] * ci * ri[i] + b;
+    }
+  }
+  lds_barrier();
+  if (half == 1) {
+#pragma unroll
+    for (int ct = 0; ct < CT; ++ct) {
+      const int col = ct * 16 + j;
+      const float ci = wi[col];
+#pragma unroll
+      for (int i = 0; i < 4; ++i) P[(4 * g + i) * LDP + col] += acc[ct][i] * ci * ri[i];
+    }
+  }
+  lds_barrier();
+  pair_tail<LDP, TRAIN, true>(P, half, lane, row0, N, M, K, ok, toff, e_lo, E, fsrc, scale, c_out, ld_c, a_save, proj_out, ld_p, row_absmax,
+                              &sRowMax[tile][0][0]);
+}
+
+int rows_padded_h2(int M, int K) { return 16 * ((M + 2 * K + 15) / 16 <= 4 ? 4 : 6); }
+
+}
+}
+
+using namespace uavgnn;
+
+extern "C" int uavgnn_tarmac_msg_rowmax_supported(int H, int M, int K, int n_ag);
+
+extern "C" int uavgnn_tarmac_msg_h2_supported(int H, int M, int K, int n_ag) { return uavgnn_tarmac_msg_rowmax_supported(H, M, K, n_ag); }
+
+extern "C" long long uavgnn_tarmac_msg_weight_bytes_h2(int H, int M, int K) {
+  if (H <= 0 || M <= 0 || K <= 0 || (M + 2 * K + 15) / 16 > 6) return 0;
+  const long long RP = rows_padded_h2(M, K);
+  return static_cast<long long>(2 * H / 32) * 2 * RP * 64 + 2 * RP * 4;
+}
+
+extern "C" int uavgnn_tarmac_msg_prepare_h2(const float* Wp, int ld, int H, int M, int K, void* tiles, uavgnn_stream_t stream) {
+  if (!Wp || !tiles || H <= 0 || M <= 0 || K <= 0 || ld < 2 * H) return UAVGNN_EINVAL;
+  if ((H % 32) || (ld & 3) || (reinterpret_cast<uintptr_t>(Wp) & 15) || (reinterpret_cast<uintptr_t>(tiles) & 15) ||
+      (M + 2 * K + 15) / 16 > 6)
+    return UAVGNN_EUNSUPPORTED;
+  const int R = M + 2 * K, RP = rows_padded_h2(M, K);
+  u32x4* t = static_cast<u32x4*>(tiles);
+  float* winv = reinterpret_cast<float*>(t + static_cast<size_t>(2 * H / 32) * 2 * RP * 4);
+  hipLaunchKernelGGL(tarmac_msg_prepare_h2_kernel, dim3(RP), dim3(256), 0, static_cast<hipStream_t>(stream), Wp, ld, R, RP, H, t, winv);
+  return launch_status();
+}
+
+extern "C" int uavgnn_tarmac_msg_fwd_h2(const float* x, int ld_x, const float* h, int ld_h, int N, int H, int n_ag, const float* x_bound,
+                                        int ld_xb, int n_xb, const float* h_bound, int ld_hb, int n_hb, const void* tiles,
+                                        const float* bias, int M, int K, const int32_t* talk_off, const int32_t* talk_src, float scale,
+                                        float* c_out, int ld_c, float* a_save, float* proj_out, int ld_p, float* x_copy, int ld_xc,
+                                        float* row_absmax, uavgnn_stream_t stream) {
+  if (N < 0 || !x || !h || !tiles || !bias || !talk_off || !c_out || !row_absmax || !x_bound || !h_bound || ld_x < H || ld_h < H ||
+      ld_c < M || n_xb < 1 || n_hb < 1 || ld_xb < n_xb || ld_hb < n_hb)
+    return UAVGNN_EINVAL;
+  if (proj_out && ld_p < M + 2 * K) return UAVGNN_EINVAL;
+  if (x_copy && ld_xc < H) return UAVGNN_EINVAL;
+  if (!uavgnn_tarmac_msg_h2_supported(H, M, K, n_ag) || (N % n_ag) || (ld_x & 3) || (ld_h & 3) || (x_copy && (ld_xc & 3)) ||
+      ((reinterpret_cast<uintptr_t>(x) | reinterpret_cast<uintptr_t>(h) | reinterpret_cast<uintptr_t>(tiles) |
+        reinterpret_cast<uintptr_t>(x_copy)) & 15))
+    return UAVGNN_EUNSUPPORTED;
+  if (N == 0) return 0;
+  const int ct = (M + 2 * K + 15) / 16, RP = rows_padded_h2(M, K);
+  const bool train = a_save != nullptr || proj_out != nullptr || x_copy != nullptr;
+  const dim3 grid((N + kMsgRows - 1) / kMsgRows), block(2 * kMsgThreads);
+  hipStream_t st = static_cast<hipStream_t>(stream);
+  const u32x4* Wt = static_cast<const u32x4*>(tiles);
+  const float* winv = reinterpret_cast<const float*>(Wt + static_cast<size_t>(2 * H / 32) * 2 * RP * 4);
+#define UAVGNN_MSG_H2(CT_, TR_)                                                                                                       \
+  hipLaunchKernelGGL((tarmac_msg_fwd_h2_kernel<CT_, TR_>), grid, block, 0, st, x, ld_x, h, ld_h, N, H, x_bound, ld_xb, n_xb, h_bound, \
+                     ld_hb, n_hb, Wt, winv, bias, M, K, talk_off, talk_src, scale, c_out, ld_c, a_save, proj_out, ld_p, x_copy, ld_xc,  \
+                     row_absmax)
+  if (ct <= 4) {
+    if (train) UAVGNN_MSG_H2(4, true);
+    else UAVGNN_MSG_H2(4, false);
+  } else {
+    if (train) UAVGNN_MSG_H2(6, true);
+    else UAVGNN_MSG_H2(6, false);
+  }
+#undef UAVGNN_MSG_H2
+  return launch_status();
+}
diff --git a/uav_bs_ctrl_amd/csrc/tarmac_msg_pair.h b/uav_bs_ctrl_amd/csrc/tarmac_msg_pair.h
--- /dev/null
+++ b/uav_bs_ctrl_amd/csrc/tarmac_msg_pair.h
@@ -0,0 +1,153 @@
+#pragma once
+#include <math.h>
+
+#include "common.h"
+
+namespace uavgnn {
+namespace msg {
+
+constexpr int kMsgWaves = 4;
+constexpr int kMsgRows = 16 * kMsgWaves;
+constexpr int kMsgThreads = kWave * kMsgWaves;
+constexpr int kNA = 16, kEMax = kNA * kNA;
+constexpr int kScratch = (kNA + 4) + 5 * kEMax;
+
+__device__ __forceinline__ void lds_barrier() {
+  __builtin_amdgcn_fence(__ATOMIC_RELEASE, "workgroup", "local");
+  __builtin_amdgcn_s_barrier();
+  __builtin_amdgcn_fence(__ATOMIC_ACQUIRE, "workgroup", "local");
+}
+
+__device__ __forceinline__ void msg_scatter(float* __restrict__ Mx, int nmax, const float* __restrict__ VAL,
+                                            const int* __restrict__ SRC, const int* __restrict__ DST,
+                                            const int* __restrict__ OFF, int E, int lane) {
+  for (int e = lane; e < E; e += kWave) {
+    const int d = DST[e], sidx = SRC[e];
+    const int j0 = OFF[d], j1 = OFF[d + 1];
+    bool first = true;
+    for (int jx = j0; jx < e; ++jx) first = first && (SRC[jx] != sidx);
+    if (first) {
+      float acc = VAL[e];
+      for (int jx = e + 1; jx < j1; ++jx)
+        if (SRC[jx] == sidx) acc += VAL[jx];
+      Mx[d * nmax + sidx] = acc;
+    }
+  }
+}
+
+template <int LDP, bool TRAIN, bool RM>
+__device__ __forceinline__ void pair_tail(float* __restrict__ P, int half, int lane, int row0, int N, int M, int K, bool ok, int toff,
+                                          int e_lo, int E, const int (&fsrc)[4], float scale, float* __restrict__ c_out, int ld_c,
+                                          float* __restrict__ a_save, float* __restrict__ proj_out, int ld_p,
+                                          float* __restrict__ row_absmax, const float* rm_pair) {
+  constexpr int NA = kNA, EMAX = kEMax;
+  const int j = lane & 15, g = lane >> 4, row = row0 + j;
+  const int ncol = M + 2 * K;
+  int* __restrict__ OFF = reinterpret_cast<int*>(P + 16 * LDP);
+  float* __restrict__ SC = reinterpret_cast<float*>(OFF + NA + 4);
+  float* __restrict__ AD = SC + EMAX;
+  int* __restrict__ SRC = reinterpret_cast<int*>(AD + EMAX);
+  int* __restrict__ DST = SRC + EMAX;
+  float* __restrict__ AV = reinterpret_cast<float*>(DST + EMAX);
+  if (half == 1) {
+    if (TRAIN && proj_out != nullptr) {
+      for (int r = 0; r < 16; ++r) {
+        if (row0 + r >= N) break;
+        float* d = proj_out + static_cast<size_t>(row0 + r) * ld_p;
+        for (int col = lane; col < ncol; col += kWave) d[col] = P[r * LDP + col];
+      }
+    }
+    lds_barrier();
+    return;
+  }
+  bool poison = !ok;
+  if (ok) {
+    for (int i = lane; i < EMAX; i += kWave) AD[i] = 0.f;
+    if (lane <= 16) OFF[lane] = toff - e_lo;
+    wave_sync_lds();
+    bool bad = false;
+#pragma unroll
+    for (int i = 0; i < 4; ++i) {
+      const int e = lane + kWave * i;
+      if (e < E) {
+        const int u = fsrc[i] - row0;
+        bad |= (u < 0) | (u >= 16);
+        SRC[e] = u < 0 ? 0 : (u >= 16 ? 15 : u);
+        int d = 0;
+#pragma unroll
+        for (int jj = 1; jj < 16; ++jj) d += e >= OFF[jj];
+        DST[e] = d;
+      }
+    }
+    poison = __any(bad);
+    wave_sync_lds();
+    if (!poison) {
+      for (int e = lane; e < E; e += kWave) {
+        const float* __restrict__ sr = P + SRC[e] * LDP + M;
+        const float* __restrict__ qr = P + DST[e] * LDP + M + K;
+        float a = 0.f;
+#pragma unroll 4
+        for (int k = 0; k < K; ++k) a = fmaf(sr[k], qr[k], a);
+        SC[e] = a * scale;
+      }
+      wave_sync_lds();
+      for (int e = lane; e < E; e += kWave) {
+        const int d = DST[e];
+        const int j0 = OFF[d], j1 = OFF[d + 1];
+        float m = -INFINITY;
+#pragma unroll 2
+        for (int jj = j0; jj < j1; ++jj) m = fmaxf(m, SC[jj]);
+        float den = 0.f;
+#pragma unroll 2
+        for (int jj = j0; jj < j1; ++jj) den += expf(SC[jj] - m);
+        const float a = expf(SC[e] - m) / den;
+        if (TRAIN && a_save != nullptr) a_save[e_lo + e] = a;
+        AV[e] = a;
+      }
+      wave_sync_lds();
+      msg_scatter(AD, NA, AV, SRC, DST, OFF, E, lane);
+      wave_sync_lds();
+    }
+  }
+  lds_barrier();
+  if (poison) {
+    for (int i = 0; i < 16; ++i)
+      for (int ch = lane; ch < M; ch += kWave) P[i * LDP + ch] = NAN;
+  } else {
+    for (int c0 = 0; c0 < M; c0 += kWave) {
+      const int ch = c0 + lane, chc = ch < M ? ch : M - 1;
+      float v[NA];
+#pragma unroll
+      for (int t = 0; t < NA; ++t) v[t] = P[t * LDP + chc];
+#pragma unroll 4
+      for (int r = 0; r < NA; ++r) {
+        float a = 0.f;
+#pragma unroll
+        for (int t = 0; t < NA; t += 4) {
+          const float4 q = *reinterpret_cast<const float4*>(AD + r * NA + t);
+          a = fmaf(q.x, v[t], a);
+          a = fmaf(q.y, v[t + 1], a);
+          a = fmaf(q.z, v[t + 2], a);
+          a = fmaf(q.w, v[t + 3], a);
+        }
+        if (ch < M) P[r * LDP + ch] = a;
+      }
+    }
+  }
+  wave_sync_lds();
+  for (int r = 0; r < 16; ++r) {
+    if (row0 + r >= N) break;
+    float* d = c_out + static_cast<size_t>(row0 + r) * ld_c;
+    for (int ch = lane; ch < M; ch += kWave) d[ch] = P[r * LDP + ch];
+  }
+  if (RM) {
+    float cm = 0.f;
+    for (int ch = g; ch < M; ch += 4) cm = fmaxf(cm, fabsf(P[j * LDP + ch]));
+    cm = fmaxf(cm, __shfl_xor(cm, 16));
+    cm = fmaxf(cm, __shfl_xor(cm, 32));
+    if (g == 0 && row < N) row_absmax[row] = fmaxf(cm, fmaxf(rm_pair[j], rm_pair[16 + j]));
+  }
+}
+
+}
+}
diff --git a/uav_bs_ctrl_amd/ops.py b/uav_bs_ctrl_amd/ops.py
--- a/uav_bs_ctrl_amd/ops.py
+++ b/uav_bs_ctrl_amd/ops.py
@@ -1,6 +1,8 @@
 from __future__ import annotations
 
 import os
+import weakref
+
 import torch as th
 
 from . import _lib as L
@@ -186,6 +188,48 @@
     return None if t.is_inference() else t._version
 
 
+_ROW_BOUNDS = {}
+
+
+class _RowBound:
+    __slots__ = ("ref", "offset", "rows", "cols", "version", "parts")
+
+
+def _leave_row_bound(out, parts):
+    if out.is_inference() or out.dim() != 2 or not out.is_contiguous():
+        return
+    key = out.untyped_storage().data_ptr()
+
+    def gone(r, key=key):
+        rec = _ROW_BOUNDS.get(key)
+        if rec is not None and rec.ref is r:
+            del _ROW_BOUNDS[key]
+
+    rec = _RowBound()
+    rec.ref, rec.offset, rec.rows, rec.cols = weakref.ref(out, gone), out.storage_offset(), out.shape[0], out.shape[1]
+    rec.version, rec.parts = out._version, parts
+    _ROW_BOUNDS[key] = rec
+
+
+def _row_bound_of(t):
+    if t.is_inference() or t.dim() != 2:
+        return None
+    key = t.untyped_storage().data_ptr()
+    rec = _ROW_BOUNDS.get(key)
+    if rec is None:
+        return None
+    base = rec.ref()
+    if base is None or base.untyped_storage().data_ptr() != key or base._version != rec.version or t._version != rec.version:
+        return None
+    off = t.storage_offset() - rec.offset
+    if t.shape[1] != rec.cols or t.stride(1) != 1 or t.stride(0) != rec.cols or off < 0 or off % rec.cols:
+        return None
+    r0 = off // rec.cols
+    if r0 + t.shape[0] > rec.rows:
+        return None
+    return rec.parts[r0:r0 + t.shape[0]]
+
+
 def _talk_transpose_if_needed(g, *tensors):
     if th.is_grad_enabled() and any(t is not None and t.requires_grad for t in tensors):
         return g.talk_transpose()
@@ -384,7 +428,7 @@
                 and 4 * N * max(ld_max, H) < 2 ** 32)
 
 
-def _gru_cell_launch(inp, h, W_ih, b_ih, W_hh, b_hh, save, inp2=None, h2_out=None, rowmax=None):
+def _gru_cell_launch(inp, h, W_ih, b_ih, W_hh, b_hh, save, inp2=None, h2_out=None, rowmax=None, hmax=None):
     N, H = h.shape
     h2 = th.empty_like(h) if h2_out is None else h2_out
     pre = th.empty((N, 4 * H), dtype=th.float32, device=h.device) if save else None
@@ -397,9 +441,12 @@
                                     lambda p: L.check(lib.uavgnn_gru_split_weights_h2(W_ih.data_ptr(), K_in, W_hh.data_ptr(), H,
                                                                                       p.data_ptr(), L.stream()),
                                                       "uavgnn_gru_split_weights_h2"), keep=(W_ih, W_hh))
-            rc = lib.uavgnn_gru_cell_fwd_h2(inp.data_ptr(), inp.stride(0), K1, L.ptr(inp2), 0 if inp2 is None else inp2.stride(0), K2,
-                                            h.data_ptr(), N, H, rowmax.data_ptr(), planes.data_ptr(), b_ih.data_ptr(), b_hh.data_ptr(),
-                                            h2.data_ptr(), L.ptr(pre), L.stream())
+            args = (inp.data_ptr(), inp.stride(0), K1, L.ptr(inp2), 0 if inp2 is None else inp2.stride(0), K2, h.data_ptr(), N, H,
+                    rowmax.data_ptr(), planes.data_ptr(), b_ih.data_ptr(), b_hh.data_ptr(), h2.data_ptr(), L.ptr(pre))
+            if hmax is not None:
+                rc = lib.uavgnn_gru_cell_fwd_h2_hmax(*args, hmax.data_ptr(), L.stream())
+            else:
+                rc = lib.uavgnn_gru_cell_fwd_h2(*args, L.stream())
         L.check(rc, "uavgnn_gru_cell_fwd_h2")
         return h2, pre
     if inp2 is not None or (GRU_X3 and L.lib().uavgnn_gru_cell_x3_supported(inp.shape[1], H)
@@ -632,7 +679,7 @@
 
 
 def gemm_h2(a, W, rowmax, transpose_w=False, bias=None, out=None, accumulate=False, relu=False, a2=None, W2=None, rowmax2=None,
-            rowmax2_out=None):
+            rowmax2_out=None, ymax_out=None):
     lib = L.lib()
     M, K1 = a.shape
     if a2 is not None:
@@ -659,9 +706,14 @@
     with KERNEL_TIMER.span("gemm_h2", (M, n_out, K)):
         planes = _cached_planes(key, lib.uavgnn_split_h2_bytes(n_out, K), a.device, build, keep=keep)
         fn, rm2 = (lib.uavgnn_gemm_nt_h2, rowmax2) if rowmax2_out is None else (lib.uavgnn_gemm_nt_h2_rm2, rowmax2_out)
-        rc = fn(a.data_ptr(), a.stride(0), K1, L.ptr(a2), 0 if a2 is None else a2.stride(0), M, K, rowmax.data_ptr(),
+        args = (a.data_ptr(), a.stride(0), K1, L.ptr(a2), 0 if a2 is None else a2.stride(0), M, K, rowmax.data_ptr(),
                 L.ptr(rm2), planes.data_ptr(), n_out, L.ptr(bias), out.data_ptr(), out.stride(0),
-                (1 if accumulate else 0) | (2 if relu else 0) | (GEMM_X3_FLAGS & 4), L.stream())
+                (1 if accumulate else 0) | (2 if relu else 0) | (GEMM_X3_FLAGS & 4))
+        if ymax_out is not None:
+            assert rowmax2_out is None
+            rc = lib.uavgnn_gemm_nt_h2_ymax(*args, ymax_out.data_ptr(), L.stream())
+        else:
+            rc = fn(*args, L.stream())
     L.check(rc, "uavgnn_gemm_nt_h2")
     return out
 
@@ -787,6 +839,8 @@
 
 class _LinearReLU(th.autograd.Function):
 
+    last_ymax = None
+
     @staticmethod
     def forward(ctx, x, W, b, rm_a=None, rm_b=None, train=True):
         ctx.x_rowmax = None
@@ -794,7 +848,9 @@
         n_out = W.shape[0]
         rm = None if rm_a is None else (rm_a, rm_b)
         if (rm is not None and b is not None and b.is_contiguous() and W.stride(1) == 1 and gemm_h2_supported(x, n_out, W.shape[1])):
-            y = gemm_h2(x, W, rm[0], False, bias=b, relu=True, rowmax2=rm[1])
+            ymax = th.empty((x.shape[0], n_out // 128), dtype=th.float32, device=x.device) if (MSG_H2 and n_out % 128 == 0) else None
+            y = gemm_h2(x, W, rm[0], False, bias=b, relu=True, rowmax2=rm[1], ymax_out=ymax)
+            _LinearReLU.last_ymax = None if ymax is None else (y.data_ptr(), ymax)
             if ctx.needs_input_grad[1] and train:
                 ctx.x_rowmax = th.maximum(rm[0], rm[1])
             ctx.save_for_backward(x, W, y)
@@ -837,7 +893,12 @@
 def linear_relu(x, W, b):
     rm = getattr(x, "_uavgnn_rowmax", None)
     if rm is not None and rm[2] == _version_of(x):
-        return _LinearReLU.apply(x, W, b, rm[0], rm[1], th.is_grad_enabled())
+        _LinearReLU.last_ymax = None
+        y = _LinearReLU.apply(x, W, b, rm[0], rm[1], th.is_grad_enabled())
+        ym, _LinearReLU.last_ymax = _LinearReLU.last_ymax, None
+        if ym is not None and ym[0] == y.data_ptr():
+            _leave_row_bound(y, ym[1])
+        return y
     return _LinearReLU.apply(x, W, b)
 
 
@@ -1139,9 +1200,10 @@
 
 
 MSG_FUSED = os.environ.get("UAVGNN_MSG_FUSED", "1") != "0"
-
-
-def _tarmac_msg_plan(x, h, Wp, bp, M, K, env, N, H):
+MSG_H2 = os.environ.get("UAVGNN_MSG_H2", "1") != "0"
+
+
+def _tarmac_msg_plan(x, h, Wp, bp, M, K, env, N, H, h2=False):
     if not MSG_FUSED or env is None or N == 0:
         return None
     _, B, n_ag = env
@@ -1151,6 +1213,12 @@
             or x.data_ptr() % 16 or h.data_ptr() % 16 or x.dtype != th.float32 or Wp.dtype != th.float32):
         return None
     lib = L.lib()
+    if h2:
+        tiles = _cached_planes(("msgw_h2", Wp.data_ptr(), Wp._version, H, M, K), lib.uavgnn_tarmac_msg_weight_bytes_h2(H, M, K), x.device,
+                               lambda buf: L.check(lib.uavgnn_tarmac_msg_prepare_h2(Wp.data_ptr(), Wp.stride(0), H, M, K, buf.data_ptr(),
+                                                                                   L.stream()), "uavgnn_tarmac_msg_prepare_h2"),
+                               keep=(Wp,))
+        return tiles, n_ag
     tiles = _cached_planes(("msgw", Wp.data_ptr(), Wp._version, H, M, K), lib.uavgnn_tarmac_msg_weight_bytes(H, M, K), x.device,
                            lambda buf: L.check(lib.uavgnn_tarmac_msg_prepare(Wp.data_ptr(), Wp.stride(0), H, M, K, buf.data_ptr(),
                                                                             L.stream()), "uavgnn_tarmac_msg_prepare"),
@@ -1159,8 +1227,17 @@
 
 
 def _launch_tarmac_msg(msg, x, h, bp, M, K, talk_off, talk_src, N, H, c_ptr, ld_c, a_save, proj, ld_p, x_copy, ld_xc, planes=None,
-                       rowmax=None):
+                       rowmax=None, bounds=None):
     tiles, n_ag = msg
+    if bounds is not None:
+        xb, hb = bounds
+        with KERNEL_TIMER.span("tarmac_msg_fwd", (N, H, M, K, int(proj is not None), int(x_copy is not None))):
+            rc = L.lib().uavgnn_tarmac_msg_fwd_h2(x.data_ptr(), x.stride(0), h.data_ptr(), h.stride(0), N, H, n_ag, xb.data_ptr(),
+                                                  xb.stride(0), xb.shape[1], hb.data_ptr(), hb.stride(0), hb.shape[1], tiles.data_ptr(),
+                                                  bp.data_ptr(), M, K, L.ptr(talk_off), L.ptr(talk_src), 1.0 / K, c_ptr, ld_c, a_save,
+                                                  proj, ld_p, x_copy, ld_xc, rowmax.data_ptr(), L.stream())
+        L.check(rc, "uavgnn_tarmac_msg_fwd_h2")
+        return
     if rowmax is not None:
         with KERNEL_TIMER.span("tarmac_msg_fwd", (N, H, M, K, int(proj is not None), int(x_copy is not None))):
             rc = L.lib().uavgnn_tarmac_msg_fwd_rowmax(x.data_ptr(), x.stride(0), h.data_ptr(), h.stride(0), N, H, n_ag, tiles.data_ptr(),
@@ -1191,13 +1268,24 @@
 
 class _TarmacStep(th.autograd.Function):
 
+    last_hmax = None
+
     @staticmethod
     def forward(ctx, x, h, Wp, bp, W_ih, b_ih, W_hh, b_hh, W_out, b_out, M, K, talk_off, talk_src, t_off, t_dst, t_pos,
                 split, env=None, dx_out=None, train=True):
         L.require_gpu(x, h, Wp, W_ih, talk_off)
         N, H = x.shape
         x, h = L.f32c(x), L.f32c(h)
-        msg = _tarmac_msg_plan(x, h, Wp, bp, M, K, env, N, H)
+        aligned = all(t.is_contiguous() and t.data_ptr() % 16 == 0 for t in (W_ih, W_hh))
+        want_rm = bool(env is not None and aligned and GRU_FUSED and gru_cell_h2_supported(H + M, H, N, max(x.stride(0), H + M))
+                       and H % 32 == 0 and M % 32 == 0 and L.lib().uavgnn_tarmac_msg_rowmax_supported(H, M, K, env[2]))
+        bounds = None
+        if want_rm and MSG_H2 and L.lib().uavgnn_tarmac_msg_h2_supported(H, M, K, env[2]):
+            xb = _row_bound_of(x)
+            hb = _row_bound_of(h) if xb is not None else None
+            if hb is not None:
+                bounds = (xb, hb)
+        msg = _tarmac_msg_plan(x, h, Wp, bp, M, K, env, N, H, h2=bounds is not None)
         if msg is not None:
             proj = None
         elif gemm_x3_supported(x, Wp.shape[0], H) and gemm_x3_supported(h, Wp.shape[0], H) and bp.is_contiguous():
@@ -1210,11 +1298,13 @@
         a_save = th.empty(max(E, 1), dtype=th.float32, device=x.device)
         ld = M + 2 * K
         ctx.seq = ctx.seq_t = None
-        aligned = all(t.is_contiguous() and t.data_ptr() % 16 == 0 for t in (W_ih, W_hh))
-        rowmax = None
-        if (msg is not None and aligned and GRU_FUSED and gru_cell_h2_supported(H + M, H, N, max(x.stride(0), H + M))
-                and H % 32 == 0 and M % 32 == 0 and L.lib().uavgnn_tarmac_msg_rowmax_supported(H, M, K, msg[1])):
+        rowmax = hmax = None
+        if msg is not None and want_rm:
             rowmax = th.empty(N, dtype=th.float32, device=x.device)
+            if MSG_H2 and H % 64 == 0 and L.lib().uavgnn_tarmac_msg_h2_supported(H, M, K, msg[1]):
+                hmax = th.empty((N, H // 64), dtype=th.float32, device=x.device)
+        else:
+            bounds = None
         c_only = None
         if not train and aligned and h.shape[0] >= GRU_FUSED_MIN_ROWS and GRU_FUSED:
             c_only = th.empty((N, M), dtype=th.float32, device=x.device)
@@ -1223,11 +1313,11 @@
         if c_only is not None:
             if msg is not None:
                 _launch_tarmac_msg(msg, x, h, bp, M, K, talk_off, talk_src, N, H, c_only.data_ptr(), M, None, None, 0, None, 0,
-                                   rowmax=rowmax)
+                                   rowmax=rowmax, bounds=bounds)
             else:
                 _launch_talk_fwd(env, proj.data_ptr() + 4 * M, ld, proj.data_ptr() + 4 * (M + K), ld, proj.data_ptr(), ld, K, M,
                                  talk_off, talk_src, N, 1.0 / K, c_only.data_ptr(), M, a_save.data_ptr(), None, 0, 0)
-            h2, _ = _gru_cell_launch(x, h, W_ih, b_ih, W_hh, b_hh, save=False, inp2=c_only, rowmax=rowmax)
+            h2, _ = _gru_cell_launch(x, h, W_ih, b_ih, W_hh, b_hh, save=False, inp2=c_only, rowmax=rowmax, hmax=hmax)
             inp, fused = c_only, True
             gi = gh = h2
         else:
@@ -1252,7 +1342,7 @@
             if msg is not None:
                 proj = th.empty((N, ld), dtype=th.float32, device=x.device)
                 _launch_tarmac_msg(msg, x, h, bp, M, K, talk_off, talk_src, N, H, inp.data_ptr() + 4 * H, H + M, a_save.data_ptr(),
-                                   proj.data_ptr(), ld, inp.data_ptr(), H + M, rowmax=rowmax)
+                                   proj.data_ptr(), ld, inp.data_ptr(), H + M, rowmax=rowmax, bounds=bounds)
             else:
                 _launch_talk_fwd(env, proj.data_ptr() + 4 * M, ld, proj.data_ptr() + 4 * (M + K), ld, proj.data_ptr(), ld, K, M,
                                  talk_off, talk_src, N, 1.0 / K, inp.data_ptr() + 4 * H, H + M, a_save.data_ptr(), x.data_ptr(),
@@ -1260,7 +1350,8 @@
             fused = gru_cell_supported(inp, h) and aligned
             if fused:
                 h2, pre = _gru_cell_launch(inp, h, W_ih, b_ih, W_hh, b_hh, save=bool(train),
-                                           h2_out=None if seq is None else seq.slot("h", seq_t + 1, H, extra=1), rowmax=rowmax)
+                                           h2_out=None if seq is None else seq.slot("h", seq_t + 1, H, extra=1), rowmax=rowmax,
+                                           hmax=hmax)
                 if seq is not None and pre is not None:
                     ctx.seq, ctx.seq_t = seq, seq_t
                 gi = gh = pre if pre is not None else h2
@@ -1271,6 +1362,7 @@
                 with KERNEL_TIMER.span("gru_gates_fwd"):
                     rc = L.lib().uavgnn_gru_gates_fwd(gi.data_ptr(), gh.data_ptr(), h.data_ptr(), N, H, h2.data_ptr(), L.stream())
                 L.check(rc, "uavgnn_gru_gates_fwd")
+        _TarmacStep.last_hmax = (h2.data_ptr(), hmax) if (hmax is not None and fused) else None
         q = head_fwd(h2, W_out, b_out)
         if proj is None:
             proj = h2
@@ -1445,8 +1537,13 @@
 
     train = th.is_grad_enabled() and any(t.requires_grad for t in (x, h, Wp, bp, cell.weight_ih, cell.bias_ih,
                                                                    cell.weight_hh, cell.bias_hh, f_out.weight, f_out.bias))
-    return _TarmacStep.apply(x, h, Wp, bp, cell.weight_ih, cell.bias_ih, cell.weight_hh, cell.bias_hh, f_out.weight,
-                             f_out.bias, M, K, off, src, t_off, t_dst, t_pos, split, env, dx_out, train)
+    _TarmacStep.last_hmax = None
+    q, h2 = _TarmacStep.apply(x, h, Wp, bp, cell.weight_ih, cell.bias_ih, cell.weight_hh, cell.bias_hh, f_out.weight,
+                              f_out.bias, M, K, off, src, t_off, t_dst, t_pos, split, env, dx_out, train)
+    hm, _TarmacStep.last_hmax = _TarmacStep.last_hmax, None
+    if hm is not None and hm[0] == h2.data_ptr():
+        _leave_row_bound(h2, hm[1])
+    return q, h2
 
 
 class _DiscComm(th.autograd.Function):
```

Measured after the change: 2.619 million. -1.1%, worse.
